# atomicarchitects/equiformer

Hardware: NVIDIA H100
Metric: edges/sec fwd+bwd, QM9 Lmax=2 batch (higher is better)
Workload: dtype f32

## Files before the change

### equiformer_b200/_lib.py

```python
from __future__ import annotations

import ctypes
import os
import shutil
import subprocess
import threading
from ctypes import POINTER, c_char_p, c_float, c_int32, c_int64, c_void_p
from pathlib import Path

PKG_DIR = Path(__file__).resolve().parent
CSRC_DIR = PKG_DIR / "csrc"
INCLUDE_DIR = PKG_DIR.parent / "include"
LIB_PATH = PKG_DIR / "libeqf_b200.so"
SOURCES = ("eqf_abi.cu", "eqf_dtp.cu", "eqf_dtp_vec.cu", "eqf_dtp_v3.cu", "eqf_attn.cu", "eqf_pointwise.cu", "eqf_gemm_tf32x3.cu", "eqf_graph.cu",
           "eqf_fused.cu", "eqf_edge.cu", "eqf_gemm_small.cu")

EQF_COLSUM_COUNTERS = 16384
EQF_MAX_BLOCKS = 8
EQF_MAX_HEADS = 16

NVCC_FLAGS = [
    "-gencode", "arch=compute_90a,code=sm_90a",
    "-lineinfo", "-O3", "-std=c++17", "--shared", "-Xcompiler", "-fPIC",
]


class EqfPathDesc(ctypes.Structure):
    _fields_ = [
        ("l1", c_int32), ("l2", c_int32), ("l3", c_int32), ("mul", c_int32),
        ("in1_block", c_int32), ("in2_off", c_int32), ("out_group", c_int32),
        ("out_chan_off", c_int32), ("w_off", c_int32), ("cg_off", c_int32),
    ]


class EqfEdgeOperands(ctypes.Structure):
    _fields_ = [
        ("x", c_void_p * EQF_MAX_BLOCKS),
        ("x2", c_void_p * EQF_MAX_BLOCKS),
        ("src", c_void_p),
        ("dst", c_void_p),
        ("y", c_void_p),
        ("w", c_void_p),
        ("w_shared", c_int32),
        ("g", c_void_p * EQF_MAX_BLOCKS),
        ("w_offset", c_void_p),
    ]


class EqfGateLayout(ctypes.Structure):
    _fields_ = [
        ("n_gated", c_int32),
        ("d", c_int32 * EQF_MAX_BLOCKS),
        ("C", c_int32 * EQF_MAX_BLOCKS),
        ("n_alpha", c_int32), ("n_scalars", c_int32), ("n_heads", c_int32),
        ("c_silu", c_float), ("c_sigmoid", c_float), ("c_slr", c_float), ("slr_slope", c_float),
    ]


class EqfNormLayout(ctypes.Structure):
    _fields_ = [
        ("n_entries", c_int32),
        ("mul", c_int32 * EQF_MAX_BLOCKS),
        ("d", c_int32 * EQF_MAX_BLOCKS),
        ("is_scalar", c_int32 * EQF_MAX_BLOCKS),
        ("eps", c_float),
    ]


class EqfHeadLayout(ctypes.Structure):
    _fields_ = [
        ("n_groups", c_int32),
        ("d", c_int32 * EQF_MAX_BLOCKS),
        ("C", c_int32 * EQF_MAX_BLOCKS),
        ("n_heads", c_int32),
    ]


EQF_GROUP_MAX = 8


class EqfGemmProblem(ctypes.Structure):
    _fields_ = [
        ("A", c_void_p), ("B", c_void_p), ("C", c_void_p),
        ("M", c_int64), ("N", c_int64), ("K", c_int64), ("lda", c_int64), ("ldb", c_int64), ("ldc", c_int64),
        ("mode", c_int32), ("accumulate", c_int32), ("alpha", c_float), ("pad", c_int32),
    ]


PtrArray = c_void_p * EQF_MAX_BLOCKS

SIGNATURES = {
    "eqf_version": (c_int32, []),
    "eqf_last_error": (c_char_p, []),
    "eqf_device_sm_count": (c_int32, []),
    "eqf_plan_create": (c_int32, [POINTER(EqfPathDesc), c_int32, POINTER(c_int32), POINTER(c_int32), c_int32,
                                  POINTER(c_int32), POINTER(c_int32), c_int32, c_int32, c_int32,
                                  POINTER(c_float), c_int32, POINTER(c_void_p)]),
    "eqf_plan_destroy": (None, [c_void_p]),
    "eqf_plan_info": (c_int32, [c_void_p, POINTER(c_int32), c_int32]),
    "eqf_plan_partial_rows": (c_int32, [c_void_p, c_int64]),
    "eqf_dtp_forward": (c_int32, [c_void_p, POINTER(EqfEdgeOperands), c_int64, POINTER(c_void_p), c_void_p]),
    "eqf_dtp_grad_x": (c_int32, [c_void_p, POINTER(EqfEdgeOperands), c_int64, POINTER(c_void_p), c_void_p]),
    "eqf_dtp_grad_w": (c_int32, [c_void_p, POINTER(EqfEdgeOperands), c_int64, c_void_p, c_void_p]),
    "eqf_dtp_grad_y": (c_int32, [c_void_p, POINTER(EqfEdgeOperands), c_int64, c_void_p, c_void_p]),
    "eqf_dtp_grad_xw": (c_int32, [c_void_p, POINTER(EqfEdgeOperands), c_int64, POINTER(c_void_p), c_void_p, c_void_p]),
    "eqf_seg_softmax": (c_int32, [c_void_p, c_void_p, c_int64, c_int32, c_void_p, c_void_p]),
    "eqf_seg_softmax_bwd": (c_int32, [c_void_p, c_void_p, c_void_p, c_void_p, c_int64, c_int32, c_void_p, c_void_p]),
    "eqf_attn_aggregate": (c_int32, [POINTER(EqfHeadLayout), c_void_p, POINTER(c_void_p), c_void_p, c_void_p, c_int64,
                                     POINTER(c_void_p), c_void_p]),
    "eqf_attn_softmax_aggregate": (c_int32, [POINTER(EqfHeadLayout), c_void_p, c_void_p, POINTER(c_void_p), c_void_p,
                                             c_int64, POINTER(c_void_p), c_void_p, c_void_p]),
    "eqf_attn_edge_dot": (c_int32, [POINTER(EqfHeadLayout), POINTER(c_void_p), POINTER(c_void_p), c_void_p, c_int64,
                                    c_void_p, c_void_p]),
    "eqf_attn_edge_scale": (c_int32, [POINTER(EqfHeadLayout), c_void_p, c_void_p, POINTER(c_void_p), c_void_p, c_int64,
                                      POINTER(c_void_p), c_void_p]),
    "eqf_pointwise_rows": (c_int32, [c_int64]),
    "eqf_ln_silu_fwd": (c_int32, [c_void_p, c_void_p, c_void_p, c_void_p, c_float, c_int64, c_int32, c_void_p, c_void_p,
                                  c_void_p, c_void_p]),
    "eqf_ln_silu_bwd": (c_int32, [c_void_p, c_void_p, c_void_p, c_void_p, c_void_p, c_void_p, c_void_p, c_int64, c_int32,
                                  c_void_p, c_void_p, c_void_p]),
    "eqf_gemm_tf32x3": (c_int32, [c_void_p, c_void_p, c_void_p, c_int64, c_int64, c_int64, c_int64, c_int64, c_int64, c_int32,
                                  c_void_p, c_void_p]),
    "eqf_gemm_tf32x3_wgrad_slices": (c_int64, [c_int64, c_int64, c_int64]),
    "eqf_gemm_tf32x3_wgrad": (c_int32, [c_void_p, c_void_p, c_void_p, c_int64, c_int64, c_int64, c_int64, c_int64, c_void_p]),
    "eqf_gemm_tf32x3_wgrad_accumulate": (c_int32, [c_void_p, c_void_p, c_void_p, c_int64, c_int64, c_int64, c_int64, c_int64,
                                                   c_void_p]),
    "eqf_dtp_linear_supported": (c_int32, [c_void_p, c_int32]),
    "eqf_fused_set_timeline": (None, [c_void_p]),
    "eqf_dtp_group_forward": (c_int32, [c_void_p, POINTER(EqfEdgeOperands), c_int64, c_int32, c_void_p, c_void_p]),
    "eqf_dtp_linear_fwd": (c_int32, [c_void_p, POINTER(EqfEdgeOperands), c_int64, c_int32, c_void_p, c_int64, c_int64, c_void_p,
                                     c_int64, c_void_p, c_void_p]),
    "eqf_radius_graph_count": (c_int32, [c_void_p, c_void_p, c_int64, c_float, c_int32, c_int64, c_void_p, c_void_p]),
    "eqf_radius_graph_fill": (c_int32, [c_void_p, c_void_p, c_int64, c_float, c_int32, c_int64, c_void_p, c_void_p, c_void_p,
                                        c_void_p]),
    "eqf_radius_graph_pbc_count": (c_int32, [c_void_p, c_void_p, c_void_p, c_void_p, c_int64, c_float, c_int32, c_int32, c_int32,
                                             c_void_p, c_void_p]),
    "eqf_radius_graph_pbc_fill": (c_int32, [c_void_p, c_void_p, c_void_p, c_void_p, c_int64, c_float, c_int32, c_int32, c_int32,
                                            c_void_p, c_void_p, c_void_p, c_void_p, c_void_p, c_void_p]),
    "eqf_edge_geom_fwd": (c_int32, [c_void_p, c_void_p, c_void_p, c_void_p, c_void_p, c_void_p, c_int64, c_int32, c_void_p,
                                    c_void_p, c_void_p, c_void_p]),
    "eqf_edge_geom_bwd": (c_int32, [c_void_p, c_void_p, c_void_p, c_int64, c_int32, c_void_p, c_void_p, c_void_p, c_void_p]),
    "eqf_expnorm_fwd": (c_int32, [c_void_p, c_void_p, c_void_p, c_float, c_float, c_int64, c_int32, c_void_p, c_void_p]),
    "eqf_expnorm_bwd": (c_int32, [c_void_p, c_void_p, c_void_p, c_float, c_float, c_int64, c_int32, c_void_p, c_void_p, c_void_p]),
    "eqf_rbf_fwd": (c_int32, [c_void_p, c_void_p, c_void_p, c_void_p, c_void_p, c_float, c_int64, c_void_p, c_void_p]),
    "eqf_rbf_bwd": (c_int32, [c_void_p, c_void_p, c_void_p, c_void_p, c_void_p, c_float, c_void_p, c_int64, c_void_p, c_void_p,
                              c_void_p]),
    "eqf_colsum_scratch_floats": (c_int64, [c_int64, c_int64]),
    "eqf_colsum": (c_int32, [c_void_p, c_int64, c_int64, c_int64, c_void_p, c_void_p, c_void_p, c_void_p]),
    "eqf_gemm_grouped": (c_int32, [ctypes.POINTER(EqfGemmProblem), c_int32, c_void_p]),
    "eqf_eln_rows": (c_int32, [POINTER(EqfNormLayout), c_int64]),
    "eqf_eln_fwd": (c_int32, [POINTER(EqfNormLayout), c_void_p, c_void_p, c_void_p, c_int64, c_void_p, c_void_p, c_void_p]),
    "eqf_eln_bwd": (c_int32, [POINTER(EqfNormLayout), c_void_p, c_void_p, c_void_p, c_void_p, c_int64, c_void_p, c_void_p,
                              c_void_p]),
    "eqf_eln_fwd_planar": (c_int32, [POINTER(EqfNormLayout), c_void_p, c_void_p, c_void_p, c_int64, c_void_p, c_void_p, c_void_p]),
    "eqf_eln_bwd_planar": (c_int32, [POINTER(EqfNormLayout), c_void_p, c_void_p, c_void_p, c_void_p, c_int64, c_void_p, c_void_p,
                                     c_void_p]),
    "eqf_gate_logits_fwd": (c_int32, [POINTER(EqfGateLayout), c_void_p, c_void_p, POINTER(c_void_p), c_void_p, c_int64,
                                      c_void_p, c_void_p, POINTER(c_void_p), c_void_p]),
    "eqf_gate_logits_bwd": (c_int32, [POINTER(EqfGateLayout), c_void_p, c_void_p, POINTER(c_void_p), c_void_p, c_void_p,
                                      c_void_p, POINTER(c_void_p), c_int64, c_void_p, POINTER(c_void_p), c_void_p,
                                      c_void_p]),
}


class EqfError(RuntimeError):
    pass


_lock = threading.Lock()
_lib = None


def sources():
    gen = sorted((CSRC_DIR / "gen").glob("dtp_gen_*.cu")) if (CSRC_DIR / "gen").exists() else []
    return [CSRC_DIR / s for s in SOURCES if (CSRC_DIR / s).exists()] + gen


def generate_sources():
    from . import codegen
    return codegen.write_all()


def needs_build() -> bool:
    if not LIB_PATH.exists():
        return True
    mtime = LIB_PATH.stat().st_mtime
    deps = sources() + list(CSRC_DIR.glob("*.cuh")) + [INCLUDE_DIR / "eqf_b200.h"]
    return any(p.stat().st_mtime > mtime for p in deps)


def build(force: bool = False, verbose: bool = False) -> Path:
    generate_sources()
    if not force and not needs_build():
        return LIB_PATH
    nvcc = shutil.which("nvcc") or "/usr/local/cuda/bin/nvcc"
    if not os.path.exists(nvcc):
        raise EqfError("nvcc not found: cannot build libeqf_b200.so")
    from concurrent.futures import ThreadPoolExecutor
    obj_dir = PKG_DIR / "build" / ("obj%d" % os.getpid())
    obj_dir.mkdir(parents=True, exist_ok=True)
    compile_flags = [f for f in NVCC_FLAGS if f != "--shared"]

    def compile_one(src: Path):
        obj = obj_dir / (src.stem + ".o")
        cmd = [nvcc, *compile_flags, "-I", str(INCLUDE_DIR), "-c", "-o", str(obj), str(src)]
        if verbose:
            cmd.insert(1, "-Xptxas=-v")
        return obj, subprocess.run(cmd, capture_output=True, text=True)

    try:
        with ThreadPoolExecutor(max_workers=min(8, os.cpu_count() or 1)) as pool:
            results = list(pool.map(compile_one, sources()))
        for _obj, proc in results:
            if proc.returncode != 0:
                raise EqfError("nvcc failed:\n" + proc.stdout + proc.stderr)
            if verbose:
                print(proc.stderr)
        tmp = LIB_PATH.with_suffix(".so.tmp%d" % os.getpid())
        link = subprocess.run([nvcc, "--shared", "-Xcompiler", "-fPIC", "-gencode", "arch=compute_90a,code=sm_90a",
                               "-o", str(tmp), *[str(o) for o, _ in results]], capture_output=True, text=True)
        if link.returncode != 0:
            raise EqfError("nvcc link failed:\n" + link.stdout + link.stderr)
        os.replace(tmp, LIB_PATH)
    finally:
        shutil.rmtree(obj_dir, ignore_errors=True)
    return LIB_PATH


def load():
    global _lib
    if _lib is not None:
        return _lib
    with _lock:
        if _lib is not None:
            return _lib
        if not LIB_PATH.exists():
            raise EqfError(
                f"{LIB_PATH} is missing: run `python -c 'import __graft_entry__ as g; g.build()'` "
                "(the sm_90a kernels are the only implementation of the edge path)")
        lib = ctypes.CDLL(str(LIB_PATH))
        for name, (restype, argtypes) in SIGNATURES.items():
            try:
                fn = getattr(lib, name)
            except AttributeError as exc:
                raise EqfError(f"libeqf_b200.so does not export {name}; rebuild it") from exc
            fn.restype = restype
            fn.argtypes = argtypes
        _lib = lib
    return _lib


def check(rc: int, what: str) -> None:
    if rc != 0:
        msg = load().eqf_last_error()
        raise EqfError(f"{what} failed (code {rc}): {msg.decode() if msg else '?'}")
```

### equiformer_b200/csrc/eqf_common.cuh

```cuda
#pragma once
#include <cuda_runtime.h>
#include <stdint.h>
#include <string>
#include <vector>

#include "../../include/eqf_b200.h"

struct EqfPlan;

namespace eqf {

constexpr int kThreads = 256;
constexpr int kWarps = kThreads / 32;
constexpr int kMaxD = 7;

struct PathDev {
  int d1, d2, d3;
  int mul;
  int xb;
  int y_off;
  int og;
  int koff;
  int w_off;
  int cg_off;
  int m_off;
  int pad;
};
static_assert(sizeof(PathDev) == 48, "PathDev layout");

struct PlanHdr {
  int n_paths, n_in1, n_out, d_y, w_numel, m_size, cg_len;
  int n_wtasks;
  int n_xtasks;
  int blob_words;
  int off_paths, off_cg, off_mdesc, off_wtasks, off_xtasks, off_xbstart, off_xbpaths;
  int te;
  int vec_ok, n_vwtasks, n_vxtasks, off_vwtasks, off_vxtasks;
  int in1_lpe[EQF_MAX_BLOCKS], in1_epw[EQF_MAX_BLOCKS];
  int in1_lpe_shift[EQF_MAX_BLOCKS];
  int in1_off[EQF_MAX_BLOCKS];
  int d_in;
  int in1_d[EQF_MAX_BLOCKS], in1_mul[EQF_MAX_BLOCKS];
  int out_d[EQF_MAX_BLOCKS], out_mul[EQF_MAX_BLOCKS];
};

struct EdgeArgs {
  const float* x[EQF_MAX_BLOCKS];
  const float* x2[EQF_MAX_BLOCKS];
  const long long* src;
  const long long* dst;
  const float* y;
  const float* w;
  const float* w_off;
  int w_shared;
  const float* g[EQF_MAX_BLOCKS];
  float* out[EQF_MAX_BLOCKS];
  float* gx[EQF_MAX_BLOCKS];
  float* gw;
  float* gy;
  long long E;
};

void set_error(const std::string& msg);
int check_cuda(cudaError_t err, const char* what);
int ensure_device(const EqfPlan* plan);
struct GeneratedKernels {
  unsigned long long signature;
  const char* tag;
  int (*forward)(const EqfPlan*, const EdgeArgs&, cudaStream_t);
  int (*backward)(const EqfPlan*, const EdgeArgs&, bool with_w, cudaStream_t);
  int (*grad_y)(const EqfPlan*, const EdgeArgs&, cudaStream_t);
  int (*partial_rows)(const EqfPlan*, long long);
};
int register_generated(const GeneratedKernels* k);
const GeneratedKernels* find_generated(unsigned long long signature);
int dtp_variant();
int launch_forward_vec(const EqfPlan* plan, const EdgeArgs& a, bool tma, cudaStream_t stream);
int launch_grad_x_vec(const EqfPlan* plan, const EdgeArgs& a, bool with_w, cudaStream_t stream);
int launch_forward_v3(const EqfPlan* plan, const EdgeArgs& a, cudaStream_t stream);
int launch_backward_v3(const EqfPlan* plan, const EdgeArgs& a, bool with_w, cudaStream_t stream);
int backward_v3_grid(const EqfPlan* plan, long long E);

}

struct EqfPlan {
  eqf::PlanHdr hdr;
  std::vector<uint32_t> blob;
  uint32_t* d_blob = nullptr;
  int device = -1;
  int sm_count = 132;
  size_t smem_bytes = 0;
  size_t smem_bytes_vec_fwd = 0;
  size_t smem_bytes_vec_bwd = 0;
  unsigned long long signature = 0;
  const eqf::GeneratedKernels* gen = nullptr;
};
```

### equiformer_b200/csrc/eqf_dtp.cu

```cuda
#include <mutex>
#include <unordered_map>

#include "eqf_common.cuh"

namespace eqf {

struct Smem {
  const PathDev* paths;
  const float* cg;
  const int* mdesc;
  const int2* wtasks;
  const int2* xtasks;
  const int* xbstart;
  const int* xbpaths;
  float* M;
  float* ysh;
  float* extra;
};

__device__ __forceinline__ Smem carve(const PlanHdr& h, const uint32_t* __restrict__ blob, uint32_t* smem) {
  for (int i = threadIdx.x; i < h.blob_words; i += blockDim.x) smem[i] = blob[i];
  Smem s;
  s.paths = reinterpret_cast<const PathDev*>(smem + h.off_paths);
  s.cg = reinterpret_cast<const float*>(smem + h.off_cg);
// ... 75 lines not shown
                                         long long e, int u) {
  float M[D1][D3];
  load_M<D1, D3>(Mp, M);
  if (u >= P.mul) return;
  float xi[D1];
  load_x<D1>(a, P.xb, P.mul, e, u, xi);
  const float wv = __ldg(a.w + (a.w_shared ? 0 : e * h.w_numel) + P.w_off + u);
  const int K = h.out_mul[P.og];
  float* o = a.out[P.og] + (e * D3) * K + P.koff + u;
#pragma unroll
  for (int k = 0; k < D3; ++k) {
    float acc = 0.f;
#pragma unroll
    for (int i = 0; i < D1; ++i) acc = fmaf(xi[i], M[i][k], acc);
    o[(long long)k * K] = wv * acc;
  }
}

__global__ void __launch_bounds__(kThreads) dtp_forward_kernel(PlanHdr h, const uint32_t* __restrict__ blob, EdgeArgs a) {
  extern __shared__ __align__(16) uint32_t smem_raw[];
  const Smem s = carve(h, blob, smem_raw);
  const int warp = threadIdx.x >> 5, lane = threadIdx.x & 31;
  const long long n_tiles = (a.E + h.te - 1) / h.te;
  for (long long tile = blockIdx.x; tile < n_tiles; tile += gridDim.x) {
    const long long e0 = tile * h.te;
    __syncthreads();
    stage_tile(h, s, a.y, e0, a.E);
    const int n_tasks = h.te * h.n_wtasks;
    for (int t = warp; t < n_tasks; t += kWarps) {
      const int te = t / h.n_wtasks;
      const long long e = e0 + te;
      if (e >= a.E) continue;
      const int2 wt = s.wtasks[t - te * h.n_wtasks];
      const PathDev& P = s.paths[wt.x];
      const float* Mp = s.M + te * h.m_size + P.m_off;
      const int u = wt.y + lane;
      EQF_DISPATCH_D(P.d1, D1, EQF_DISPATCH_D(P.d3, D3, (fwd_task<D1, D3>(h, a, P, Mp, e, u))));
    }
  }
}

template <int D1, int D3>
__device__ __forceinline__ float gw_value(const PlanHdr& h, const EdgeArgs& a, const PathDev& P, const float* Mp,
                                          long long e, int u) {
  float M[D1][D3];
  load_M<D1, D3>(Mp, M);
  if (u >= P.mul) return 0.f;
  float xi[D1];
  load_x<D1>(a, P.xb, P.mul, e, u, xi);
  const int K = h.out_mul[P.og];
  const float* gp = a.g[P.og] + (e * D3) * K + P.koff + u;
  float acc = 0.f;
#pragma unroll
  for (int k = 0; k < D3; ++k) {
    const float gk = __ldg(gp + (long long)k * K);
    float t = 0.f;
#pragma unroll
    for (int i = 0; i < D1; ++i) t = fmaf(xi[i], M[i][k], t);
    acc = fmaf(t, gk, acc);
  }
  return acc;
}

__global__ void __launch_bounds__(kThreads) dtp_grad_w_kernel(PlanHdr h, const uint32_t* __restrict__ blob, EdgeArgs a) {
  extern __shared__ __align__(16) uint32_t smem_raw[];
  const Smem s = carve(h, blob, smem_raw);
  float* wacc = s.extra;
  if (a.w_shared)
    for (int i = threadIdx.x; i < h.w_numel; i += blockDim.x) wacc[i] = 0.f;
  const int warp = threadIdx.x >> 5, lane = threadIdx.x & 31;
  const long long n_tiles = (a.E + h.te - 1) / h.te;
  for (long long tile = blockIdx.x; tile < n_tiles; tile += gridDim.x) {
    const long long e0 = tile * h.te;
    __syncthreads();
    stage_tile(h, s, a.y, e0, a.E);
    const int n_tasks = h.te * h.n_wtasks;
    for (int t = warp; t < n_tasks; t += kWarps) {
      const int te = t / h.n_wtasks;
      const long long e = e0 + te;
      if (e >= a.E) continue;
      const int2 wt = s.wtasks[t - te * h.n_wtasks];
      const PathDev& P = s.paths[wt.x];
      const float* Mp = s.M + te * h.m_size + P.m_off;
      const int u = wt.y + lane;
      float v = 0.f;
      EQF_DISPATCH_D(P.d1, D1, EQF_DISPATCH_D(P.d3, D3, (v = gw_value<D1, D3>(h, a, P, Mp, e, u))));
      if (u < P.mul) {
        if (a.w_shared) atomicAdd(wacc + P.w_off + u, v);
        else a.gw[e * h.w_numel + P.w_off + u] = v;
      }
    }
  }
  if (a.w_shared) {
    __syncthreads();
    for (int i = threadIdx.x; i < h.w_numel; i += blockDim.x) a.gw[(long long)blockIdx.x * h.w_numel + i] = wacc[i];
  }
}

template <int D1, int D3, bool WITH_W>
__device__ __forceinline__ void gx_path(const PlanHdr& h, const EdgeArgs& a, const PathDev& P, const float* Mp,
                                        long long e, int u, const float (&xi)[D1], float (&acc)[D1], float* wacc) {
  float M[D1][D3];
  load_M<D1, D3>(Mp, M);
  const int K = h.out_mul[P.og];
  const float* gp = a.g[P.og] + (e * D3) * K + P.koff + u;
  float gk[D3];
#pragma unroll
  for (int k = 0; k < D3; ++k) gk[k] = __ldg(gp + (long long)k * K);
  const float wv = __ldg(a.w + (a.w_shared ? 0 : e * h.w_numel) + P.w_off + u);
  float gwv = 0.f;
#pragma unroll
  for (int i = 0; i < D1; ++i) {
    float t = 0.f;
#pragma unroll
    for (int k = 0; k < D3; ++k) t = fmaf(gk[k], M[i][k], t);
    acc[i] = fmaf(wv, t, acc[i]);
    if (WITH_W) gwv = fmaf(xi[i], t, gwv);
  }
  if (WITH_W) {
    if (a.w_shared) atomicAdd(wacc + P.w_off + u, gwv);
    else a.gw[e * h.w_numel + P.w_off + u] = gwv;
  }
}

template <int D1, bool WITH_W>
__device__ __forceinline__ void gx_task(const PlanHdr& h, const EdgeArgs& a, const Smem& s, int te, long long e,
                                        int xb, int u, float* wacc) {
  const int mul = h.in1_mul[xb];
  if (u >= mul) return;
  float xi[D1];
  if (WITH_W) load_x<D1>(a, xb, mul, e, u, xi);
  float acc[D1];
#pragma unroll
  for (int i = 0; i < D1; ++i) acc[i] = 0.f;
  for (int q = s.xbstart[xb]; q < s.xbstart[xb + 1]; ++q) {
    const PathDev& P = s.paths[s.xbpaths[q]];
    const float* Mp = s.M + te * h.m_size + P.m_off;
    EQF_DISPATCH_D(P.d3, D3, (gx_path<D1, D3, WITH_W>(h, a, P, Mp, e, u, xi, acc, wacc)));
  }
  float* o = a.gx[xb] + (e * D1) * mul + u;
#pragma unroll
  for (int i = 0; i < D1; ++i) o[(long long)i * mul] = acc[i];
}

template <bool WITH_W>
__global__ void __launch_bounds__(kThreads) dtp_grad_x_kernel(PlanHdr h, const uint32_t* __restrict__ blob, EdgeArgs a) {
  extern __shared__ __align__(16) uint32_t smem_raw[];
  const Smem s = carve(h, blob, smem_raw);
  float* wacc = s.extra;
  if (WITH_W && a.w_shared)
    for (int i = threadIdx.x; i < h.w_numel; i += blockDim.x) wacc[i] = 0.f;
  const int warp = threadIdx.x >> 5, lane = threadIdx.x & 31;
  const long long n_tiles = (a.E + h.te - 1) / h.te;
  for (long long tile = blockIdx.x; tile < n_tiles; tile += gridDim.x) {
    const long long e0 = tile * h.te;
    __syncthreads();
    stage_tile(h, s, a.y, e0, a.E);
    const int n_tasks = h.te * h.n_xtasks;
    for (int t = warp; t < n_tasks; t += kWarps) {
      const int te = t / h.n_xtasks;
      const long long e = e0 + te;
      if (e >= a.E) continue;
      const int2 xt = s.xtasks[t - te * h.n_xtasks];
      const int u = xt.y + lane;
      EQF_DISPATCH_D(h.in1_d[xt.x], D1, (gx_task<D1, WITH_W>(h, a, s, te, e, xt.x, u, wacc)));
    }
  }
  if (WITH_W && a.w_shared) {
    __syncthreads();
    for (int i = threadIdx.x; i < h.w_numel; i += blockDim.x) a.gw[(long long)blockIdx.x * h.w_numel + i] = wacc[i];
  }
}

template <int D1, int D3>
__device__ __forceinline__ void gy_task(const PlanHdr& h, const EdgeArgs& a, const PathDev& P, float* Np,
                                        long long e, int u, int lane) {
  float xi[D1], gk[D3];
  float wv = 0.f;
#pragma unroll
  for (int i = 0; i < D1; ++i) xi[i] = 0.f;
#pragma unroll
  for (int k = 0; k < D3; ++k) gk[k] = 0.f;
  if (u < P.mul) {
    load_x<D1>(a, P.xb, P.mul, e, u, xi);
    const int K = h.out_mul[P.og];
    const float* gp = a.g[P.og] + (e * D3) * K + P.koff + u;
#pragma unroll
    for (int k = 0; k < D3; ++k) gk[k] = __ldg(gp + (long long)k * K);
    wv = __ldg(a.w + (a.w_shared ? 0 : e * h.w_numel) + P.w_off + u);
  }
#pragma unroll
  for (int i = 0; i < D1; ++i) {
    const float wx = wv * xi[i];
#pragma unroll
    for (int k = 0; k < D3; ++k) {
      const float r = warp_sum(wx * gk[k]);
      if (lane == 0) atomicAdd(Np + i * D3 + k, r);
    }
  }
}

__global__ void __launch_bounds__(kThreads) dtp_grad_y_kernel(PlanHdr h, const uint32_t* __restrict__ blob, EdgeArgs a) {
  extern __shared__ __align__(16) uint32_t smem_raw[];
  const Smem s = carve(h, blob, smem_raw);
  float* N = s.extra;
  const int warp = threadIdx.x >> 5, lane = threadIdx.x & 31;
  const long long n_tiles = (a.E + h.te - 1) / h.te;
  for (long long tile = blockIdx.x; tile < n_tiles; tile += gridDim.x) {
    const long long e0 = tile * h.te;
    __syncthreads();
    for (int i = threadIdx.x; i < h.te * h.m_size; i += blockDim.x) N[i] = 0.f;
    __syncthreads();
    const int n_tasks = h.te * h.n_wtasks;
    for (int t = warp; t < n_tasks; t += kWarps) {
      const int te = t / h.n_wtasks;
      const long long e = e0 + te;
      if (e >= a.E) continue;
      const int2 wt = s.wtasks[t - te * h.n_wtasks];
      const PathDev& P = s.paths[wt.x];
      float* Np = N + te * h.m_size + P.m_off;
      const int u = wt.y + lane;
      EQF_DISPATCH_D(P.d1, D1, EQF_DISPATCH_D(P.d3, D3, (gy_task<D1, D3>(h, a, P, Np, e, u, lane))));
    }
    __syncthreads();
    for (int idx = threadIdx.x; idx < h.te * h.d_y; idx += blockDim.x) {
      const int te = idx / h.d_y;
      const int jj = idx - te * h.d_y;
      const long long e = e0 + te;
      if (e >= a.E) continue;
      float acc = 0.f;
      for (int p = 0; p < h.n_paths; ++p) {
        const PathDev& P = s.paths[p];
        const int j = jj - P.y_off;
        if (j < 0 || j >= P.d2) continue;
        const float* c = s.cg + P.cg_off + j * P.d3;
        const float* Np = N + te * h.m_size + P.m_off;
        for (int i = 0; i < P.d1; ++i)
          for (int k = 0; k < P.d3; ++k) acc = fmaf(c[i * P.d2 * P.d3 + k], Np[i * P.d3 + k], acc);
      }
      a.gy[e * h.d_y + jj] = acc;
    }
  }
}

static int fill_args(const EqfPlan* plan, const EqfEdgeOperands* op, long long E, EdgeArgs& a, bool need_x,
                     bool need_g, bool need_w) {
  if (plan == nullptr || op == nullptr) { set_error("null plan/operands"); return EQF_ERR_INVALID; }
  if (E < 0) { set_error("negative edge count"); return EQF_ERR_INVALID; }
  const PlanHdr& h = plan->hdr;
  for (int b = 0; b < EQF_MAX_BLOCKS; ++b) {
    a.x[b] = op->x[b]; a.x2[b] = op->x2[b]; a.g[b] = op->g[b];
    a.out[b] = nullptr; a.gx[b] = nullptr;
  }
  a.src = reinterpret_cast<const long long*>(op->src);
  a.dst = reinterpret_cast<const long long*>(op->dst);
  a.y = op->y; a.w = op->w; a.w_off = op->w_offset; a.w_shared = op->w_shared; a.gw = nullptr; a.gy = nullptr; a.E = E;
  if (E == 0) return EQF_OK;
  if (a.w_off != nullptr && !(plan->gen != nullptr && dtp_variant() == 4)) {
    set_error("w_offset is only supported by the plan-specialised kernels");
    return EQF_ERR_UNSUPPORTED;
  }
  if (a.y == nullptr) { set_error("edge_attr (y) pointer is null"); return EQF_ERR_INVALID; }
  if (need_w && a.w == nullptr) { set_error("weight pointer is null"); return EQF_ERR_INVALID; }
  if (need_x) for (int b = 0; b < h.n_in1; ++b) {
    if (a.x[b] == nullptr) { set_error("in1 block pointer is null"); return EQF_ERR_INVALID; }
    if (a.x2[b] != nullptr && a.dst == nullptr) { set_error("x2 given without dst index"); return EQF_ERR_INVALID; }
  }
  if (need_g) for (int g = 0; g < h.n_out; ++g)
    if (a.g[g] == nullptr) { set_error("output-group pointer is null"); return EQF_ERR_INVALID; }
  return ensure_device(plan);
}

static int grid_for(const EqfPlan* plan, long long E) {
  const long long n_tiles = (E + plan->hdr.te - 1) / plan->hdr.te;
  const long long cap = (long long)plan->sm_count * 8;
  return (int)(n_tiles < cap ? (n_tiles > 0 ? n_tiles : 1) : cap);
}

template <typename K>
static int set_smem(K kernel, size_t bytes) {
  if (bytes <= 48 * 1024) return EQF_OK;
  static std::mutex mu;
  static std::unordered_map<const void*, size_t> configured;
  std::lock_guard<std::mutex> lock(mu);
  size_t& have = configured[reinterpret_cast<const void*>(kernel)];
  if (bytes > have) {
    int rc = check_cuda(cudaFuncSetAttribute(kernel, cudaFuncAttributeMaxDynamicSharedMemorySize, (int)bytes),
                        "cudaFuncSetAttribute(smem)");
    if (rc != EQF_OK) return rc;
    have = bytes;
  }
  return EQF_OK;
}

}

using namespace eqf;

extern "C" int eqf_plan_partial_rows(const EqfPlan* plan, int64_t n_edges) {
  if (plan == nullptr) return EQF_ERR_INVALID;
  int rows = grid_for(plan, n_edges);
  const int b = backward_v3_grid(plan, n_edges);
  if (b > rows) rows = b;
  if (plan->gen != nullptr) { const int c = plan->gen->partial_rows(plan, n_edges); if (c > rows) rows = c; }
  return rows;
}

extern "C" int eqf_dtp_forward(const EqfPlan* plan, const EqfEdgeOperands* op, int64_t n_edges,
                               float* const* out_groups, void* stream) {
  EdgeArgs a;
  int rc = fill_args(plan, op, n_edges, a, true, false, true);
  if (rc != EQF_OK || n_edges == 0) return rc;
  for (int g = 0; g < plan->hdr.n_out; ++g) {
    if (out_groups == nullptr || out_groups[g] == nullptr) { set_error("null output group"); return EQF_ERR_INVALID; }
    a.out[g] = out_groups[g];
  }
  if (plan->gen != nullptr && dtp_variant() == 4) return plan->gen->forward(plan, a, (cudaStream_t)stream);
  if (plan->hdr.vec_ok && dtp_variant() == 3) return launch_forward_v3(plan, a, (cudaStream_t)stream);
  if (plan->hdr.vec_ok && dtp_variant() > 0)
    return launch_forward_vec(plan, a, dtp_variant() == 2 && !a.w_shared, (cudaStream_t)stream);
  const size_t smem = plan->smem_bytes;
  if ((rc = set_smem(dtp_forward_kernel, smem)) != EQF_OK) return rc;
  dtp_forward_kernel<<<grid_for(plan, n_edges), kThreads, smem, (cudaStream_t)stream>>>(plan->hdr, plan->d_blob, a);
  return check_cuda(cudaGetLastError(), "dtp_forward_kernel launch");
}

extern "C" int eqf_dtp_grad_w(const EqfPlan* plan, const EqfEdgeOperands* op, int64_t n_edges, float* gw,
                              void* stream) {
  EdgeArgs a;
  int rc = fill_args(plan, op, n_edges, a, true, true, false);
  if (rc != EQF_OK || n_edges == 0) return rc;
  if (gw == nullptr) { set_error("null gw"); return EQF_ERR_INVALID; }
  a.gw = gw;
  const size_t smem = plan->smem_bytes;
  if ((rc = set_smem(dtp_grad_w_kernel, smem)) != EQF_OK) return rc;
  dtp_grad_w_kernel<<<grid_for(plan, n_edges), kThreads, smem, (cudaStream_t)stream>>>(plan->hdr, plan->d_blob, a);
  return check_cuda(cudaGetLastError(), "dtp_grad_w_kernel launch");
}

extern "C" int eqf_dtp_grad_x(const EqfPlan* plan, const EqfEdgeOperands* op, int64_t n_edges,
                              float* const* gx_blocks, void* stream) {
  EdgeArgs a;
  int rc = fill_args(plan, op, n_edges, a, false, true, true);
  if (rc != EQF_OK || n_edges == 0) return rc;
  for (int b = 0; b < plan->hdr.n_in1; ++b) {
    if (gx_blocks == nullptr || gx_blocks[b] == nullptr) { set_error("null gx block"); return EQF_ERR_INVALID; }
    a.gx[b] = gx_blocks[b];
  }
  if (plan->gen != nullptr && dtp_variant() == 4) return plan->gen->backward(plan, a, false, (cudaStream_t)stream);
  if (plan->hdr.vec_ok && dtp_variant() == 3) return launch_backward_v3(plan, a, false, (cudaStream_t)stream);
  if (plan->hdr.vec_ok && dtp_variant() > 0) return launch_grad_x_vec(plan, a, false, (cudaStream_t)stream);
  const size_t smem = plan->smem_bytes;
  if ((rc = set_smem(dtp_grad_x_kernel<false>, smem)) != EQF_OK) return rc;
  dtp_grad_x_kernel<false><<<grid_for(plan, n_edges), kThreads, smem, (cudaStream_t)stream>>>(plan->hdr, plan->d_blob, a);
  return check_cuda(cudaGetLastError(), "dtp_grad_x_kernel launch");
}

extern "C" int eqf_dtp_grad_xw(const EqfPlan* plan, const EqfEdgeOperands* op, int64_t n_edges,
                               float* const* gx_blocks, float* gw, void* stream) {
  EdgeArgs a;
  int rc = fill_args(plan, op, n_edges, a, true, true, true);
  if (rc != EQF_OK || n_edges == 0) return rc;
  if (gw == nullptr) { set_error("null gw"); return EQF_ERR_INVALID; }
  for (int b = 0; b < plan->hdr.n_in1; ++b) {
    if (gx_blocks == nullptr || gx_blocks[b] == nullptr) { set_error("null gx block"); return EQF_ERR_INVALID; }
    a.gx[b] = gx_blocks[b];
  }
  a.gw = gw;
  if (plan->gen != nullptr && dtp_variant() == 4) return plan->gen->backward(plan, a, true, (cudaStream_t)stream);
  if (plan->hdr.vec_ok && dtp_variant() == 3) return launch_backward_v3(plan, a, true, (cudaStream_t)stream);
  if (plan->hdr.vec_ok && dtp_variant() > 0) return launch_grad_x_vec(plan, a, true, (cudaStream_t)stream);
  const size_t smem = plan->smem_bytes;
  if ((rc = set_smem(dtp_grad_x_kernel<true>, smem)) != EQF_OK) return rc;
  dtp_grad_x_kernel<true><<<grid_for(plan, n_edges), kThreads, smem, (cudaStream_t)stream>>>(plan->hdr, plan->d_blob, a);
  return check_cuda(cudaGetLastError(), "dtp_grad_xw_kernel launch");
}

extern "C" int eqf_dtp_grad_y(const EqfPlan* plan, const EqfEdgeOperands* op, int64_t n_edges, float* gy,
                              void* stream) {
  EdgeArgs a;
  int rc = fill_args(plan, op, n_edges, a, true, true, true);
  if (rc != EQF_OK || n_edges == 0) return rc;
  if (gy == nullptr) { set_error("null gy"); return EQF_ERR_INVALID; }
  a.gy = gy;
  if (plan->gen != nullptr && dtp_variant() == 4) return plan->gen->grad_y(plan, a, (cudaStream_t)stream);
  const size_t smem = plan->smem_bytes;
  if ((rc = set_smem(dtp_grad_y_kernel, smem)) != EQF_OK) return rc;
  dtp_grad_y_kernel<<<grid_for(plan, n_edges), kThreads, smem, (cudaStream_t)stream>>>(plan->hdr, plan->d_blob, a);
  return check_cuda(cudaGetLastError(), "dtp_grad_y_kernel launch");
}
```

### equiformer_b200/csrc/eqf_tc.cuh

```cuda
#pragma once
#include <cuda.h>
#include <cuda_runtime.h>

#include <cstdint>
#include <string>

#include "eqf_common.cuh"

namespace eqf {
namespace tc {

__device__ __forceinline__ uint32_t smem_u32(const void* p) { return (uint32_t)__cvta_generic_to_shared(p); }

__device__ __forceinline__ void mbar_init(uint64_t* bar, uint32_t count) {
  asm volatile("mbarrier.init.shared::cta.b64 [%0], %1;" ::"r"(smem_u32(bar)), "r"(count));
}
__device__ __forceinline__ void mbar_arrive(uint64_t* bar) {
  asm volatile("mbarrier.arrive.shared::cta.b64 _, [%0];" ::"r"(smem_u32(bar)) : "memory");
}
__device__ __forceinline__ void mbar_expect_tx(uint64_t* bar, uint32_t bytes) {
  asm volatile("mbarrier.arrive.expect_tx.shared::cta.b64 _, [%0], %1;" ::"r"(smem_u32(bar)), "r"(bytes) : "memory");
}
__device__ __forceinline__ void mbar_wait(uint64_t* bar, uint32_t parity) {
  uint32_t done;
  do {
    asm volatile("{\n\t.reg .pred p;\n\tmbarrier.try_wait.parity.shared::cta.b64 p, [%1], %2;\n\tselp.u32 %0, 1, 0, p;\n\t}"
                 : "=r"(done) : "r"(smem_u32(bar)), "r"(parity) : "memory");
  } while (!done);
}
__device__ __forceinline__ void mbar_wait_hint(uint64_t* bar, uint32_t parity) {
  asm volatile(
      "{\n\t.reg .pred p;\n\t"
      "WAIT_%=:\n\t"
      "mbarrier.try_wait.parity.shared::cta.b64 p, [%0], %1, %2;\n\t"
      "@p bra DONE_%=;\n\t"
      "bra WAIT_%=;\n\t"
      "DONE_%=:\n\t}"
      ::"r"(smem_u32(bar)), "r"(parity), "r"(0x989680u) : "memory");
}
__device__ __forceinline__ void tma_load_2d(void* dst, const CUtensorMap* map, int c0, int c1, uint64_t* bar) {
  asm volatile("cp.async.bulk.tensor.2d.shared::cluster.global.mbarrier::complete_tx::bytes [%0], [%1, {%2, %3}], [%4];"
               ::"r"(smem_u32(dst)), "l"(reinterpret_cast<uint64_t>(map)), "r"(c0), "r"(c1), "r"(smem_u32(bar)) : "memory");
}
__device__ __forceinline__ void prefetch_map(const CUtensorMap* map) {
  asm volatile("prefetch.tensormap [%0];" ::"l"(reinterpret_cast<uint64_t>(map)) : "memory");
}
__device__ __forceinline__ void fence_async_smem() { asm volatile("fence.proxy.async.shared::cta;" ::: "memory"); }

__device__ __forceinline__ float tf32_rn(float x) {
  uint32_t r;
  asm("cvt.rna.tf32.f32 %0, %1;" : "=r"(r) : "f"(x));
  return __uint_as_float(r);
}
__device__ __forceinline__ float tf32_rn_fast(float x) {
  return __uint_as_float((__float_as_uint(x) + 0x1000u) & 0xffffe000u);
}

__device__ __forceinline__ float lds32(uint32_t addr) {
  float v;
  asm volatile("ld.shared.f32 %0, [%1];" : "=f"(v) : "r"(addr));
  return v;
}
__device__ __forceinline__ float4 lds128(uint32_t addr) {
  float4 v;
  asm volatile("ld.shared.v4.f32 {%0, %1, %2, %3}, [%4];" : "=f"(v.x), "=f"(v.y), "=f"(v.z), "=f"(v.w) : "r"(addr));
  return v;
}
__device__ __forceinline__ void sts128(uint32_t addr, const float4& v) {
  asm volatile("st.shared.v4.f32 [%0], {%1, %2, %3, %4};" ::"r"(addr), "f"(v.x), "f"(v.y), "f"(v.z), "f"(v.w) : "memory");
}

template <int N> __device__ __forceinline__ void reg_alloc() { asm volatile("setmaxnreg.inc.sync.aligned.u32 %0;" ::"n"(N)); }
template <int N> __device__ __forceinline__ void reg_dealloc() { asm volatile("setmaxnreg.dec.sync.aligned.u32 %0;" ::"n"(N)); }

__device__ __forceinline__ void named_barrier(int id, int threads) {
  asm volatile("bar.sync %0, %1;" ::"r"(id), "r"(threads) : "memory");
}

__device__ __forceinline__ uint64_t smem_desc_sw128(uint32_t addr) {
  return (uint64_t)((addr >> 4) & 0x3FFF) | (1ull << 16) | (64ull << 32) | (1ull << 62);
}
__device__ __forceinline__ void wgmma_fence() { asm volatile("wgmma.fence.sync.aligned;" ::: "memory"); }
__device__ __forceinline__ void wgmma_commit() { asm volatile("wgmma.commit_group.sync.aligned;" ::: "memory"); }
template <int N> __device__ __forceinline__ void wgmma_wait() { asm volatile("wgmma.wait_group.sync.aligned %0;" ::"n"(N) : "memory"); }

__device__ __forceinline__ void wgmma_rs_n32(float* d, const uint32_t* a, uint64_t b_desc) {
  asm volatile(
      "{\n\t.reg .pred p;\n\tsetp.ne.b32 p, 1, 0;\n\t"
      "wgmma.mma_async.sync.aligned.m64n32k8.f32.tf32.tf32 "
      "{%0, %1, %2, %3, %4, %5, %6, %7, %8, %9, %10, %11, %12, %13, %14, %15}, "
      "{%16, %17, %18, %19}, %20, p, 1, 1;\n\t}"
      : "+f"(d[0]), "+f"(d[1]), "+f"(d[2]), "+f"(d[3]), "+f"(d[4]), "+f"(d[5]), "+f"(d[6]), "+f"(d[7]),
        "+f"(d[8]), "+f"(d[9]), "+f"(d[10]), "+f"(d[11]), "+f"(d[12]), "+f"(d[13]), "+f"(d[14]), "+f"(d[15])
      : "r"(a[0]), "r"(a[1]), "r"(a[2]), "r"(a[3]), "l"(b_desc));
}
__device__ __forceinline__ void wgmma_rs_n64(float* d, const uint32_t* a, uint64_t b_desc) {
  asm volatile(
      "{\n\t.reg .pred p;\n\tsetp.ne.b32 p, 1, 0;\n\t"
      "wgmma.mma_async.sync.aligned.m64n64k8.f32.tf32.tf32 "
      "{%0, %1, %2, %3, %4, %5, %6, %7, %8, %9, %10, %11, %12, %13, %14, %15, "
      "%16, %17, %18, %19, %20, %21, %22, %23, %24, %25, %26, %27, %28, %29, %30, %31}, "
      "{%32, %33, %34, %35}, %36, p, 1, 1;\n\t}"
      : "+f"(d[0]), "+f"(d[1]), "+f"(d[2]), "+f"(d[3]), "+f"(d[4]), "+f"(d[5]), "+f"(d[6]), "+f"(d[7]),
        "+f"(d[8]), "+f"(d[9]), "+f"(d[10]), "+f"(d[11]), "+f"(d[12]), "+f"(d[13]), "+f"(d[14]), "+f"(d[15]),
        "+f"(d[16]), "+f"(d[17]), "+f"(d[18]), "+f"(d[19]), "+f"(d[20]), "+f"(d[21]), "+f"(d[22]), "+f"(d[23]),
        "+f"(d[24]), "+f"(d[25]), "+f"(d[26]), "+f"(d[27]), "+f"(d[28]), "+f"(d[29]), "+f"(d[30]), "+f"(d[31])
      : "r"(a[0]), "r"(a[1]), "r"(a[2]), "r"(a[3]), "l"(b_desc));
}

constexpr int kKTile = 32;

template <int N4>
__device__ __forceinline__ void load_a_split(uint32_t tile, int row0, int lane, uint32_t (&hi)[N4], uint32_t (&lo)[N4],
                                             int kb0 = 0) {
  static_assert(N4 % 4 == 0 && N4 <= 4 * (kKTile / 8), "whole 8-deep k-steps of one k-tile");
  const int g = row0 + (lane >> 2), t = lane & 3;
#pragma unroll
  for (int kb = 0; kb < N4 / 4; ++kb) {
#pragma unroll
    for (int q = 0; q < 4; ++q) {
      const int r = g + ((q & 1) ? 8 : 0);
      const int c = (kb0 + kb) * 8 + t + ((q & 2) ? 4 : 0);
      const float x = lds32(tile + (uint32_t)r * 128u + (uint32_t)((((c >> 2) ^ (r & 7)) << 4) + (c & 3) * 4));
      const float h = tf32_rn_fast(x);
      hi[kb * 4 + q] = __float_as_uint(h);
      lo[kb * 4 + q] = __float_as_uint(tf32_rn_fast(x - h));
    }
  }
}

template <int BN, int N4>
__device__ __forceinline__ void mma_ktile_3xtf32(float* acc, const uint32_t (&hi)[N4], const uint32_t (&lo)[N4], uint32_t b_hi,
                                                 uint32_t b_lo, int kb0 = 0) {
  static_assert(BN % 32 == 0 && BN >= 32 && BN <= 256, "BN must be a multiple of 32 up to 256");
  wgmma_fence();
#pragma unroll
  for (int kb = 0; kb < N4 / 4; ++kb) {
    const uint64_t adv = (uint64_t)(((kb0 + kb) * 32) >> 4);
#pragma unroll
    for (int j = 0; j < BN / 64; ++j) {
      const uint64_t dh = smem_desc_sw128(b_hi + (uint32_t)j * 8192u) + adv, dl = smem_desc_sw128(b_lo + (uint32_t)j * 8192u) + adv;
      wgmma_rs_n64(acc + 32 * j, &lo[kb * 4], dh);
      wgmma_rs_n64(acc + 32 * j, &hi[kb * 4], dl);
      wgmma_rs_n64(acc + 32 * j, &hi[kb * 4], dh);
    }
    if constexpr (BN % 64 == 32) {
      constexpr int j = BN / 64;
      const uint64_t dh = smem_desc_sw128(b_hi + (uint32_t)j * 8192u) + adv, dl = smem_desc_sw128(b_lo + (uint32_t)j * 8192u) + adv;
      wgmma_rs_n32(acc + 32 * j, &lo[kb * 4], dh);
      wgmma_rs_n32(acc + 32 * j, &hi[kb * 4], dl);
      wgmma_rs_n32(acc + 32 * j, &hi[kb * 4], dh);
    }
  }
  wgmma_commit();
}

__device__ __forceinline__ int acc_row(int i, int lane) { return (lane >> 2) + ((i >> 1) & 1) * 8; }
__device__ __forceinline__ int acc_col(int i, int lane) { return 8 * ((i & 31) >> 2) + 2 * (lane & 3) + (i & 1) + 64 * (i >> 5); }

template <int BN>
__device__ __forceinline__ void store_acc(const float* acc, float* C, long long ldc, long long row0, long long M, int col0, int N,
                                          int lane, bool add) {
#pragma unroll
  for (int i = 0; i < BN / 2; i += 2) {
    const long long r = row0 + acc_row(i, lane);
    const int c = col0 + acc_col(i, lane);
    if (r >= M || c >= N) continue;
    float* p = C + r * ldc + c;
    if (add) {
      atomicAdd(p, acc[i]);
      if (c + 1 < N) atomicAdd(p + 1, acc[i + 1]);
    } else if (c + 1 < N) {
      *reinterpret_cast<float2*>(p) = make_float2(acc[i], acc[i + 1]);
    } else {
      *p = acc[i];
    }
  }
}

typedef CUresult (*EncodeTiled)(CUtensorMap*, CUtensorMapDataType, cuuint32_t, void*, const cuuint64_t*, const cuuint64_t*,
                                const cuuint32_t*, const cuuint32_t*, CUtensorMapInterleave, CUtensorMapSwizzle,
                                CUtensorMapL2promotion, CUtensorMapFloatOOBfill);

static inline EncodeTiled encode_fn() {
  static EncodeTiled fn = [] {
    void* f = nullptr;
    cudaDriverEntryPointQueryResult q;
    if (cudaGetDriverEntryPoint("cuTensorMapEncodeTiled", &f, cudaEnableDefault, &q) != cudaSuccess) f = nullptr;
    return reinterpret_cast<EncodeTiled>(f);
  }();
  return fn;
}

enum class MapKind { kSwizzled, kLinear };

static inline int make_map_2d(CUtensorMap* map, const float* base, long long rows, long long cols, long long ld, int box_rows,
                              int box_cols, MapKind kind = MapKind::kSwizzled) {
  EncodeTiled enc = encode_fn();
  if (enc == nullptr) { set_error("cuTensorMapEncodeTiled is not available from the driver"); return EQF_ERR_CUDA; }
  cuuint64_t dims[2] = {(cuuint64_t)cols, (cuuint64_t)rows};
  cuuint64_t strides[1] = {(cuuint64_t)ld * sizeof(float)};
  cuuint32_t box[2] = {(cuuint32_t)box_cols, (cuuint32_t)box_rows};
  cuuint32_t estr[2] = {1, 1};
  const CUtensorMapSwizzle sw = kind == MapKind::kLinear ? CU_TENSOR_MAP_SWIZZLE_NONE : CU_TENSOR_MAP_SWIZZLE_128B;
  CUresult r = enc(map, CU_TENSOR_MAP_DATA_TYPE_FLOAT32, 2, const_cast<float*>(base), dims, strides, box, estr,
                   CU_TENSOR_MAP_INTERLEAVE_NONE, sw, CU_TENSOR_MAP_L2_PROMOTION_L2_128B, CU_TENSOR_MAP_FLOAT_OOB_FILL_NONE);
  if (r != CUDA_SUCCESS) { set_error("cuTensorMapEncodeTiled failed (code " + std::to_string((int)r) + ")"); return EQF_ERR_CUDA; }
  return EQF_OK;
}

static inline int device_sms() {
  int sms = 132, dev = 0;
  cudaGetDevice(&dev);
  cudaDeviceGetAttribute(&sms, cudaDevAttrMultiProcessorCount, dev);
  return sms;
}

}
}
```

### equiformer_b200/nets/graph_attention_transformer.py

```python
from __future__ import annotations

import math
from typing import List, Sequence

import torch

from .. import o3, ops
from ..graph import radius_graph, scatter_sum
from ..o3 import Irreps
from .drop import EquivariantDropout, GraphDropPath
from .fast_activation import Activation, Gate
from .gaussian_rbf import GaussianRadialBasisLayer
from .layer_norm import EquivariantLayerNormV2
from .radial_func import RadialProfile, clear_hoisted, hoist_first_layers
from .registry import register_model
from .tensor_product_rescale import (FullyConnectedTensorProductRescale,
                                     FullyConnectedTensorProductRescaleSwishGate, LinearRS, TensorProductRescale,
                                     irreps2gate, sort_irreps_even_first)

_RESCALE = True
_USE_BIAS = True

_MAX_ATOM_TYPE = 5
_AVG_NUM_NODES = 18.03065905448718
_AVG_DEGREE = 15.57930850982666


def get_norm_layer(norm_type):
    if norm_type == "layer":
        return EquivariantLayerNormV2
    if norm_type is None:
        return None
    if norm_type in ("graph", "instance", "fast_layer"):
        raise NotImplementedError(f"norm '{norm_type}' is not used by any shipped Equiformer config (out of scope)")
    raise ValueError(f"Norm type {norm_type} not supported.")


class SmoothLeakyReLU(torch.nn.Module):

    def __init__(self, negative_slope: float = 0.2):
        super().__init__()
        self.alpha = negative_slope

    def forward(self, x):
        return 0.5 * (1 + self.alpha) * x + 0.5 * (1 - self.alpha) * x * (2 * torch.sigmoid(x) - 1)

    def extra_repr(self) -> str:
        return f"negative_slope={self.alpha}"


def get_mul_0(irreps) -> int:
    return sum(mul for mul, ir in Irreps(irreps) if ir.l == 0 and ir.p == 1)


def DepthwiseTensorProduct(irreps_node_input, irreps_edge_attr, irreps_node_output, internal_weights=False, bias=True):
    irreps_node_input, irreps_edge_attr = Irreps(irreps_node_input), Irreps(irreps_edge_attr)
    irreps_node_output = Irreps(irreps_node_output)
    entries, raw = [], []
    scalar = o3.Irrep(0, 1)
    for i, (mul, ir_in) in enumerate(irreps_node_input):
        for j, (_, ir_edge) in enumerate(irreps_edge_attr):
            for ir_out in ir_in * ir_edge:
                if ir_out in irreps_node_output or ir_out == scalar:
                    raw.append((i, j, len(entries), "uvu", True))
                    entries.append((mul, ir_out))
    irreps_output, perm, _ = sort_irreps_even_first(Irreps(entries))
    instructions = [(i1, i2, perm[io], mode, train) for i1, i2, io, mode, train in raw]
    return TensorProductRescale(irreps_node_input, irreps_edge_attr, irreps_output, instructions,
                                internal_weights=internal_weights, shared_weights=internal_weights,
                                bias=bias, rescale=_RESCALE)


class SeparableFCTP(torch.nn.Module):

    def __init__(self, irreps_node_input, irreps_edge_attr, irreps_node_output, fc_neurons,
                 use_activation=False, norm_layer="graph", internal_weights=False):
        super().__init__()
        self.irreps_node_input = Irreps(irreps_node_input)
        self.irreps_edge_attr = Irreps(irreps_edge_attr)
        self.irreps_node_output = Irreps(irreps_node_output)
        norm = get_norm_layer(norm_layer)
        self.dtp = DepthwiseTensorProduct(self.irreps_node_input, self.irreps_edge_attr, self.irreps_node_output,
                                          bias=False, internal_weights=internal_weights)
        self.dtp_rad = None
        if fc_neurons is not None:
            self.dtp_rad = RadialProfile(fc_neurons + [self.dtp.tp.weight_numel])
            with torch.no_grad():
                for sl, k in self.dtp.slices_sqrt_k.values():
                    self.dtp_rad.net[-1].weight.data[sl, :] *= k
                    self.dtp_rad.offset.data[sl] *= k
        irreps_lin_output = self.irreps_node_output
        irreps_scalars, irreps_gates, irreps_gated = irreps2gate(self.irreps_node_output)
        if use_activation:
            irreps_lin_output = (irreps_scalars + irreps_gates + irreps_gated).simplify()
        self.lin = LinearRS(self.dtp.irreps_out.simplify(), irreps_lin_output)
        self.norm = norm(self.lin.irreps_out) if norm_layer is not None else None
        self.gate = None
        if use_activation:
            if irreps_gated.num_irreps == 0:
                self.gate = Activation(self.irreps_node_output, acts=[torch.nn.SiLU()])
            else:
                self.gate = Gate(irreps_scalars, [torch.nn.SiLU() for _ in irreps_scalars],
                                 irreps_gates, [torch.sigmoid for _ in irreps_gates], irreps_gated)

    def forward(self, node_input, edge_attr, edge_scalars, batch=None, **kwargs):
        weight = None
        if self.dtp_rad is not None and edge_scalars is not None:
            weight = self.dtp_rad(edge_scalars)
        out = self.lin(self.dtp(node_input, edge_attr, weight))
        if self.norm is not None:
            out = self.norm(out, batch=batch)
        if self.gate is not None:
            out = self.gate(out)
        return out

    def planar(self, xs: Sequence[torch.Tensor], edge_attr, edge_scalars):
        if self.norm is not None:
            raise NotImplementedError("planar SeparableFCTP with a norm layer is unused by the reference")
        weight = self.dtp_rad(edge_scalars) if (self.dtp_rad is not None and edge_scalars is not None) else None
        out = self.lin.planar(self.dtp.planar(xs, edge_attr, weight))
        if self.gate is not None:
            out = self.gate.planar(out) if isinstance(self.gate, Gate) else [self.gate(o) for o in out]
        return out


class Vec2AttnHeads(torch.nn.Module):

    def __init__(self, irreps_head, num_heads):
        super().__init__()
        self.num_heads = num_heads
        self.irreps_head = Irreps(irreps_head)
        self.irreps_mid_in = Irreps([(mul * num_heads, ir) for mul, ir in self.irreps_head])
        self.mid_in_indices = [(s.start, s.stop) for s in self.irreps_mid_in.slices()]

    def forward(self, x):
        n = x.shape[0]
        return torch.cat([x.narrow(1, a, b - a).reshape(n, self.num_heads, -1) for a, b in self.mid_in_indices], dim=2)

    def __repr__(self) -> str:
        return f"{self.__class__.__name__}(irreps_head={self.irreps_head}, num_heads={self.num_heads})"


class AttnHeads2Vec(torch.nn.Module):

    def __init__(self, irreps_head):
        super().__init__()
        self.irreps_head = Irreps(irreps_head)
        self.head_indices = [(s.start, s.stop) for s in self.irreps_head.slices()]

    def forward(self, x):
        n = x.shape[0]
        return torch.cat([x.narrow(2, a, b - a).reshape(n, -1) for a, b in self.head_indices], dim=1)

    def __repr__(self) -> str:
        return f"{self.__class__.__name__}(irreps_head={self.irreps_head})"


_GRAPH_CACHE = {}


def _graph_for(edge_src, edge_dst, n_nodes, kwargs) -> ops.Graph:
    g = kwargs.get("graph")
    if isinstance(g, ops.Graph) and g.n_nodes == n_nodes:
        return g
    key = (edge_src.data_ptr(), edge_dst.data_ptr(), edge_dst.numel(), n_nodes, edge_dst._version, edge_src._version)
    hit = _GRAPH_CACHE.get("last")
    if hit is not None and hit[0] == key:
        return hit[1]
    g = ops.Graph(edge_src, edge_dst, n_nodes)
    _GRAPH_CACHE["last"] = (key, g, edge_src, edge_dst)
    return g


def _is_sorted_simplified(irreps: Irreps) -> bool:
    keys = [(ir.l, -ir.p) for _, ir in irreps]
    return keys == sorted(keys) and len(set(keys)) == len(keys)


def _entries_from_groups(groups: Sequence[torch.Tensor], plan) -> List[torch.Tensor]:
    return [groups[plan.group_of_entry[io]].narrow(2, plan.chan_off_of_entry[io], mul)
            for io, (mul, _ir) in enumerate(plan.irreps_out)]


def _reblock(blocks: Sequence[torch.Tensor], irreps_from: Irreps, irreps_to: Irreps) -> List[torch.Tensor]:
    if list(irreps_from) == list(irreps_to):
        return list(blocks)
    if irreps_from.dim != irreps_to.dim:
        raise ValueError(f"cannot reinterpret {irreps_from} as {irreps_to}")
    return ops.to_planar(ops.from_planar(blocks), irreps_to)


def _group_weight_matrices(lin, n_groups: int):
    try:
        ins = [(i.i_in1, i.i_in2, i.i_out) for i in lin.tp.instructions]
        if ins != [(g, 0, g) for g in range(n_groups)] or len(lin.irreps_out) != n_groups:
            return None
        blocks = lin.tp.linear_weight_blocks()
        if any(c != 1.0 for *_i, _W, c in blocks):
            return None
        return [W.reshape(W.shape[0], W.shape[2]) for _i1, _i2, _io, W, _c in blocks]
    except (AttributeError, NotImplementedError):
        return None


def _fused_linear_possible(lin, dtp) -> bool:
    return _group_weight_matrices(lin, len(dtp.tp.plan.out_groups)) is not None


class GraphAttention(torch.nn.Module):

    def __init__(self, irreps_node_input, irreps_node_attr, irreps_edge_attr, irreps_node_output, fc_neurons,
                 irreps_head, num_heads, irreps_pre_attn=None, rescale_degree=False, nonlinear_message=False,
                 alpha_drop=0.1, proj_drop=0.1):
        super().__init__()
        self.irreps_node_input = Irreps(irreps_node_input)
        self.irreps_node_attr = Irreps(irreps_node_attr)
        self.irreps_edge_attr = Irreps(irreps_edge_attr)
        self.irreps_node_output = Irreps(irreps_node_output)
        self.irreps_pre_attn = self.irreps_node_input if irreps_pre_attn is None else Irreps(irreps_pre_attn)
        self.irreps_head = Irreps(irreps_head)
        self.num_heads = num_heads
        self.rescale_degree = rescale_degree
        self.nonlinear_message = nonlinear_message

        self.merge_src = LinearRS(self.irreps_node_input, self.irreps_pre_attn, bias=True)
        self.merge_dst = LinearRS(self.irreps_node_input, self.irreps_pre_attn, bias=False)

        irreps_attn_heads = self.irreps_head * num_heads
        irreps_attn_heads, _, _ = sort_irreps_even_first(irreps_attn_heads)
        irreps_attn_heads = irreps_attn_heads.simplify()
        mul_alpha = get_mul_0(irreps_attn_heads)
        mul_alpha_head = mul_alpha // num_heads
        irreps_alpha = Irreps(f"{mul_alpha}x0e")
        irreps_attn_all = (irreps_alpha + irreps_attn_heads).simplify()
        self.irreps_attn_heads = irreps_attn_heads

        self.sep_act = None
        if self.nonlinear_message:
            self.sep_act = SeparableFCTP(self.irreps_pre_attn, self.irreps_edge_attr, self.irreps_pre_attn, fc_neurons,
                                         use_activation=True, norm_layer=None, internal_weights=False)
            self.sep_alpha = LinearRS(self.sep_act.dtp.irreps_out, irreps_alpha)
            self.sep_value = SeparableFCTP(self.irreps_pre_attn, self.irreps_edge_attr, irreps_attn_heads,
                                           fc_neurons=None, use_activation=False, norm_layer=None,
                                           internal_weights=True)
            self.vec2heads_alpha = Vec2AttnHeads(Irreps(f"{mul_alpha_head}x0e"), num_heads)
            self.vec2heads_value = Vec2AttnHeads(self.irreps_head, num_heads)
        else:
            self.sep = SeparableFCTP(self.irreps_pre_attn, self.irreps_edge_attr, irreps_attn_all, fc_neurons,
                                     use_activation=False, norm_layer=None)
            self.vec2heads = Vec2AttnHeads((Irreps(f"{mul_alpha_head}x0e") + self.irreps_head).simplify(), num_heads)

        self.alpha_act = Activation(Irreps(f"{mul_alpha_head}x0e"), [SmoothLeakyReLU(0.2)])
        self.heads2vec = AttnHeads2Vec(self.irreps_head)
        self.mul_alpha_head = mul_alpha_head
        self.alpha_dot = torch.nn.Parameter(torch.randn(1, num_heads, mul_alpha_head))
        bound = math.sqrt(6.0 / (num_heads + mul_alpha_head))
        with torch.no_grad():
            self.alpha_dot.uniform_(-bound, bound)
        self.alpha_dropout = torch.nn.Dropout(alpha_drop) if alpha_drop != 0.0 else None
        self.proj = LinearRS(irreps_attn_heads, self.irreps_node_output)
        self.proj_drop = EquivariantDropout(self.irreps_node_input, drop_prob=proj_drop) if proj_drop != 0.0 else None

        self._alpha_single_gemm = False
        if self.nonlinear_message:
            plan_out = self.sep_act.dtp.irreps_out
            n0 = sum(1 for _, ir in plan_out if ir.is_scalar())
            ins = [(i.i_in1, i.i_in2, i.i_out) for i in self.sep_alpha.tp.instructions]
            if (n0 > 0 and all(ir.is_scalar() for _, ir in plan_out[:n0]) and ins == [(i, 0, 0) for i in range(n0)]
                    and all(c == 1.0 for *_i, _W, c in self.sep_alpha.tp.linear_weight_blocks())):
                self._alpha_single_gemm = True

        self._gate_layout = None
        if self.nonlinear_message and self._alpha_single_gemm and isinstance(self.sep_act.gate, Gate):
            gate, lin = self.sep_act.gate, self.sep_act.lin
            ins = [(i.i_in1, i.i_out) for i in lin.tp.instructions]
            n_out = len(lin.irreps_out)
            canonical = (len(gate.irreps_scalars) == 1 and ins == [(i, i) for i in range(n_out)]
                         and lin.irreps_out[0].ir.is_scalar()
                         and lin.irreps_out[0].mul == gate.irreps_scalars.dim + gate.irreps_gates.dim
                         and [m for m, _ in lin.irreps_out[1:]] == [m for m, _ in gate.irreps_gated]
                         and len(lin.bias) == 1 and len(self.sep_alpha.bias) == 1 and mul_alpha_head <= 32
                         and all(c == 1.0 for *_i, _W, c in lin.tp.linear_weight_blocks())
                         and all(c == 1.0 for *_i, _W, c in self.sep_alpha.tp.linear_weight_blocks()))
            if canonical:
                self._gate_layout = ops.GateLayout(
                    mul_alpha, gate.irreps_scalars.dim, num_heads, [ir.dim for _, ir in gate.irreps_gated],
                    [m for m, _ in gate.irreps_gated], gate.act_scalars.acts[0].cst, gate.act_gates.acts[0].cst,
                    self.alpha_act.acts[0].cst, 0.2)

        if not _is_sorted_simplified(self.irreps_head):
            raise NotImplementedError("irreps_head must be sorted (l ascending, even first) with one entry per irrep")
        self._head_layout = ops.HeadLayout([ir.dim for _, ir in irreps_attn_heads],
                                           [mul for mul, _ in irreps_attn_heads], num_heads)
        self._fuse_act = (self._gate_layout is not None and _fused_linear_possible(self.sep_act.lin, self.sep_act.dtp))
        self._fuse_value = (self.nonlinear_message and _fused_linear_possible(self.sep_value.lin, self.sep_value.dtp))

    @property
    def supports_planar(self) -> bool:
        return self.proj_drop is None or not self.training or getattr(self.proj_drop, "drop_prob", 1.0) == 0.0

    def forward(self, node_input, node_attr, edge_src, edge_dst, edge_attr, edge_scalars, batch, **kwargs):
        xs = ops.to_planar(node_input, self.irreps_node_input)
        node = self.forward_planar(xs, node_attr, edge_src, edge_dst, edge_attr, edge_scalars, batch, **kwargs)
        node_output = ops.from_planar(node)
        if self.proj_drop is not None:
            node_output = self.proj_drop(node_output)
        return node_output

    def forward_planar(self, xs, node_attr, edge_src, edge_dst, edge_attr, edge_scalars, batch, **kwargs):
        n_nodes = xs[0].shape[0]
        graph = _graph_for(edge_src, edge_dst, n_nodes, kwargs)
        edge_attr = graph.sort_edges(edge_attr).contiguous()
        edge_scalars = graph.sort_edges(edge_scalars)
        E, H, A = graph.n_edges, self.num_heads, self.mul_alpha_head

        m_src = self.merge_src.planar(xs)
        m_dst = self.merge_dst.planar(xs)

        if self.nonlinear_message:
            sa = self.sep_act
            weight = sa.dtp_rad(edge_scalars, add_offset=False)
            plan1 = sa.dtp.tp.plan
            fuse1 = self._fuse_act and ops.dtp_linear_ok(plan1, edge_attr, weight)
            f = None
            if not fuse1:
                f = sa.dtp.tp.planar_depthwise_gathered(graph, m_src, m_dst, edge_attr, weight,
                                                        sa.dtp_rad.offset)
            logits = None
            if self._gate_layout is not None and (fuse1 or ops.fused_ok(f[0])):
                lay = self._gate_layout
                blocks = {io: (W, c) for _i1, _i2, io, W, c in sa.lin.tp.linear_weight_blocks()}
                k0 = plan1.out_groups[0][2]
                w_cat = torch.cat([self.sep_alpha.tp.weight.view(k0, -1), blocks[0][0].reshape(k0, -1)], dim=1)
                bias = torch.cat([self.sep_alpha.bias[0], sa.lin.bias[0]])
                if fuse1:
                    Ws = [w_cat] + [blocks[g][0].reshape(blocks[g][0].shape[0], -1) for g in range(1, len(plan1.out_groups))]
                    outs = ops.dtp_linear(plan1, graph, m_src, m_dst, edge_attr, weight, sa.dtp_rad.offset, Ws)
                    t0, gated = outs[0].reshape(E, -1), outs[1:]
                else:
                    t0 = ops.matmul_f32(f[0].reshape(E, k0), w_cat)
                    gated = [ops.matmul_f32(f[g].reshape(E * f[g].shape[1], f[g].shape[2]), blocks[g][0].reshape(f[g].shape[2], -1))
                             .view(E, f[g].shape[1], -1) for g in range(1, len(f))]
                logits, v0, *vs = ops.GateLogits.apply(lay, t0, bias, self.alpha_dot.view(H, A), *gated)
                value = _reblock([v0.view(E, 1, -1), *vs], sa.gate.irreps_out, self.sep_value.irreps_node_input)
                value = self._value_linear(value, edge_attr)
                alpha = None
            elif self._alpha_single_gemm:
                k0 = f[0].shape[2]
                w_alpha = self.sep_alpha.tp.weight.view(k0, -1)
                alpha = ops.matmul_f32(f[0].reshape(E, k0), w_alpha)
                if len(self.sep_alpha.bias) > 0:
                    alpha = alpha + self.sep_alpha.bias[0]
            else:
                alpha = self.sep_alpha.planar(_entries_from_groups(f, sa.dtp.tp.plan))[0]
            if logits is None:
                value = sa.lin.planar(f)
                value = sa.gate.planar(value) if isinstance(sa.gate, Gate) else [sa.gate(v) for v in value]
                value = _reblock(value, sa.gate.irreps_out, self.sep_value.irreps_node_input)
                value = self._value_linear(value, edge_attr)
                alpha = alpha.reshape(E, H, A)
        else:
            weight = self.sep.dtp_rad(edge_scalars, add_offset=False)
            logits = None
            out = self.sep.lin.planar(self.sep.dtp.tp.planar_depthwise_gathered(
                graph, m_src, m_dst, edge_attr, weight, self.sep.dtp_rad.offset))
            first = out[0]
            if first.shape[1] != 1:
                raise NotImplementedError("attention logits need a leading 0e entry")
            per_head = first.reshape(E, H, -1)
            alpha = per_head.narrow(2, 0, A)
            rest = per_head.shape[2] - A
            value = ([per_head.narrow(2, A, rest).reshape(E, 1, H * rest)] if rest > 0 else []) + list(out[1:])

        z = logits if logits is not None else (self.alpha_act(alpha) * self.alpha_dot).sum(dim=-1)
        no_drop = self.alpha_dropout is None or not self.training or self.alpha_dropout.p == 0.0
        if ops.softmax_aggregate_ok(self._head_layout, z):
            vs = [v.contiguous() for v in value]
            if no_drop:
                node = list(ops.SoftmaxAggregate.apply(self._head_layout, graph, z.contiguous(), *vs))
            else:
                keep = torch.nn.functional.dropout(torch.ones_like(z), self.alpha_dropout.p, True)
                node = list(ops.MaskedSoftmaxAggregate.apply(self._head_layout, graph, z.contiguous(), keep, *vs))
        else:
            attn = ops.segment_softmax(z.contiguous(), graph)
            if self.alpha_dropout is not None:
                attn = self.alpha_dropout(attn)
            node = ops.attention_aggregate(self._head_layout, graph, attn.contiguous(), [v.contiguous() for v in value])

        if self.rescale_degree:
            degree = (graph.row_ptr[1:] - graph.row_ptr[:-1]).to(node[0].dtype).view(-1, 1, 1)
            node = [t * degree for t in node]
        return self.proj.planar(node)

    def _value_linear(self, value, edge_attr):
        sv = self.sep_value
        plan2 = sv.dtp.tp.plan
        w2 = sv.dtp.tp.weight
        if self._fuse_value and ops.dtp_linear_ok(plan2, edge_attr, w2):
            Ws = _group_weight_matrices(sv.lin, len(plan2.out_groups))
            return sv.lin._planar_bias(ops.dtp_linear(plan2, None, [v.contiguous() for v in value], None, edge_attr, w2,
                                                      None, Ws))
        return sv.lin.planar(sv.dtp.planar(value, edge_attr, None))

    def extra_repr(self) -> str:
        return f"rescale_degree={self.rescale_degree}, "


class FeedForwardNetwork(torch.nn.Module):

    def __init__(self, irreps_node_input, irreps_node_attr, irreps_node_output, irreps_mlp_mid=None, proj_drop=0.1):
        super().__init__()
        self.irreps_node_input = Irreps(irreps_node_input)
        self.irreps_node_attr = Irreps(irreps_node_attr)
        self.irreps_mlp_mid = Irreps(irreps_mlp_mid) if irreps_mlp_mid is not None else self.irreps_node_input
        self.irreps_node_output = Irreps(irreps_node_output)
        self.fctp_1 = FullyConnectedTensorProductRescaleSwishGate(
            self.irreps_node_input, self.irreps_node_attr, self.irreps_mlp_mid, bias=True, rescale=_RESCALE)
        self.fctp_2 = FullyConnectedTensorProductRescale(
            self.irreps_mlp_mid, self.irreps_node_attr, self.irreps_node_output, bias=True, rescale=_RESCALE)
        self.proj_drop = EquivariantDropout(self.irreps_node_output, drop_prob=proj_drop) if proj_drop != 0.0 else None
        self._gate_layout = None
        gate, f1 = self.fctp_1.gate, self.fctp_1
        ins = [(i.i_in1, i.i_out) for i in f1.tp.instructions]
        if (isinstance(gate, Gate) and ins == [(i, i) for i in range(len(f1.irreps_out))] and len(f1.bias) == 1
                and self.irreps_node_attr.dim == 1):
            lay = ops.gate_only_layout(gate, f1.irreps_out)
            self._gate_layout = lay if (lay is not None and f1.bias[0].numel() == lay.width) else None

    @property
    def supports_planar(self) -> bool:
        return self.proj_drop is None or not self.training or getattr(self.proj_drop, "drop_prob", 1.0) == 0.0

    def forward(self, node_input, node_attr, **kwargs):
        node_output = ops.from_planar(self.forward_planar(ops.to_planar(node_input, self.irreps_node_input), node_attr))
        if self.proj_drop is not None:
            node_output = self.proj_drop(node_output)
        return node_output

    def forward_planar(self, xs, node_attr, **kwargs):
        y = None if (getattr(node_attr, "_eqf_all_ones", False) and self.irreps_node_attr.dim == 1) else node_attr
        gate = self.fctp_1.gate
        if self._gate_layout is not None and y is None and ops.fused_ok(xs[0]):
            pre = self.fctp_1.tp.planar_linear(xs, None, None)
            N = pre[0].shape[0]
            h = ops.gate_fused(self._gate_layout, pre[0].reshape(N, -1), self.fctp_1.bias[0], pre[1:])
            h = _reblock([h[0].view(N, 1, -1), *h[1:]], gate.irreps_out, self.fctp_2.irreps_in1)
        else:
            h = self.fctp_1.planar(xs, y)
            if isinstance(gate, Gate):
                h = _reblock(gate.planar(h), gate.irreps_out, self.fctp_2.irreps_in1)
            else:
                h = [gate(t) for t in h]
        return self.fctp_2.planar(h, y)


class TransBlock(torch.nn.Module):

    def __init__(self, irreps_node_input, irreps_node_attr, irreps_edge_attr, irreps_node_output, fc_neurons,
                 irreps_head, num_heads, irreps_pre_attn=None, rescale_degree=False, nonlinear_message=False,
                 alpha_drop=0.1, proj_drop=0.1, drop_path_rate=0.0, irreps_mlp_mid=None, norm_layer="layer"):
        super().__init__()
        self.irreps_node_input = Irreps(irreps_node_input)
        self.irreps_node_attr = Irreps(irreps_node_attr)
        self.irreps_edge_attr = Irreps(irreps_edge_attr)
        self.irreps_node_output = Irreps(irreps_node_output)
        self.irreps_pre_attn = self.irreps_node_input if irreps_pre_attn is None else Irreps(irreps_pre_attn)
        self.irreps_head = Irreps(irreps_head)
        self.num_heads = num_heads
        self.rescale_degree = rescale_degree
        self.nonlinear_message = nonlinear_message
        self.irreps_mlp_mid = Irreps(irreps_mlp_mid) if irreps_mlp_mid is not None else self.irreps_node_input

        self.norm_1 = get_norm_layer(norm_layer)(self.irreps_node_input)
        setattr(self, self._attn_name, self._make_attention(fc_neurons, alpha_drop, proj_drop))
        self.drop_path = GraphDropPath(drop_path_rate) if drop_path_rate > 0.0 else None
        self.norm_2 = get_norm_layer(norm_layer)(self.irreps_node_input)
        self.ffn = FeedForwardNetwork(irreps_node_input=self.irreps_node_input, irreps_node_attr=self.irreps_node_attr,
                                      irreps_node_output=self.irreps_node_output, irreps_mlp_mid=self.irreps_mlp_mid,
                                      proj_drop=proj_drop)
        self.ffn_shortcut = None
        if self.irreps_node_input != self.irreps_node_output:
            self.ffn_shortcut = FullyConnectedTensorProductRescale(
                self.irreps_node_input, self.irreps_node_attr, self.irreps_node_output, bias=True, rescale=_RESCALE)

    _attn_name = "ga"

    def _make_attention(self, fc_neurons, alpha_drop, proj_drop):
        return GraphAttention(irreps_node_input=self.irreps_node_input, irreps_node_attr=self.irreps_node_attr,
                              irreps_edge_attr=self.irreps_edge_attr, irreps_node_output=self.irreps_node_input,
                              fc_neurons=fc_neurons, irreps_head=self.irreps_head, num_heads=self.num_heads,
                              irreps_pre_attn=self.irreps_pre_attn, rescale_degree=self.rescale_degree,
                              nonlinear_message=self.nonlinear_message, alpha_drop=alpha_drop, proj_drop=proj_drop)

    @property
    def attention(self):
        return getattr(self, self._attn_name)

    def forward(self, node_input, node_attr, edge_src, edge_dst, edge_attr, edge_scalars, batch, **kwargs):
        features = self.norm_1(node_input, batch=batch)
        features = self.attention(node_input=features, node_attr=node_attr, edge_src=edge_src, edge_dst=edge_dst,
                                  edge_attr=edge_attr, edge_scalars=edge_scalars, batch=batch, **kwargs)
        n_graphs = kwargs.get("n_graphs")
        if self.drop_path is not None:
            features = self._drop_path(features, batch, n_graphs)
        node_output = node_input + features

        features = self.ffn(self.norm_2(node_output, batch=batch), node_attr)
        if self.ffn_shortcut is not None:
            node_output = self.ffn_shortcut(node_output, node_attr)
        if self.drop_path is not None:
            features = self._drop_path(features, batch, n_graphs)
        return node_output + features

    def _drop_path(self, features, batch, n_graphs):
        return self.drop_path(features, batch) if n_graphs is None else self.drop_path(features, batch, n_graphs=n_graphs)

    @property
    def supports_planar(self) -> bool:
        return (getattr(self.norm_1, "supports_planar", False) and getattr(self.norm_2, "supports_planar", False)
                and self.ffn_shortcut is None
                and (self.drop_path is None or not self.training or type(self.drop_path) is GraphDropPath)
                and self.attention.supports_planar and self.ffn.supports_planar
                and self.irreps_node_input == self.irreps_node_output)

    def forward_planar(self, xs, node_attr, edge_src, edge_dst, edge_attr, edge_scalars, batch, **kwargs):
        f = self.attention.forward_planar(self.norm_1.planar(xs), node_attr, edge_src, edge_dst, edge_attr, edge_scalars,
                                          batch, **kwargs)
        xs = self._residual(xs, f, batch, kwargs.get("n_graphs"))
        f = self.ffn.forward_planar(self.norm_2.planar(xs), node_attr)
        return self._residual(xs, f, batch, kwargs.get("n_graphs"))

    def _residual(self, xs, f, batch, n_graphs):
        if self.drop_path is None or not self.training:
            return [a + b for a, b in zip(xs, f)]
        s = self.drop_path.node_scale(f[0], batch, n_graphs)
        return [torch.addcmul(a, b, s) for a, b in zip(xs, f)]


class NodeEmbeddingNetwork(torch.nn.Module):
    def __init__(self, irreps_node_embedding, max_atom_type=_MAX_ATOM_TYPE, bias=True):
        super().__init__()
        self.max_atom_type = max_atom_type
        self.irreps_node_embedding = Irreps(irreps_node_embedding)
        self.atom_type_lin = LinearRS(Irreps(f"{self.max_atom_type}x0e"), self.irreps_node_embedding, bias=bias)
        self.atom_type_lin.tp.weight.data.mul_(self.max_atom_type ** 0.5)

    def forward(self, node_atom):
        classes = torch.arange(self.max_atom_type, device=node_atom.device)
        onehot = (node_atom.unsqueeze(-1) == classes).to(self.atom_type_lin.tp.weight.dtype)
        return self.atom_type_lin(onehot), onehot, onehot


class ScaledScatter(torch.nn.Module):
    def __init__(self, avg_aggregate_num):
        super().__init__()
        self.avg_aggregate_num = avg_aggregate_num + 0.0

    def forward(self, x, index, **kwargs):
        return scatter_sum(x, index, **kwargs).div(self.avg_aggregate_num ** 0.5)

    def extra_repr(self) -> str:
        return f"avg_aggregate_num={self.avg_aggregate_num}"


class EdgeDegreeEmbeddingNetwork(torch.nn.Module):

    def __init__(self, irreps_node_embedding, irreps_edge_attr, fc_neurons, avg_aggregate_num):
        super().__init__()
        irreps_node_embedding = Irreps(irreps_node_embedding)
        self.exp = LinearRS(Irreps("1x0e"), irreps_node_embedding, bias=_USE_BIAS, rescale=_RESCALE)
        self.dw = DepthwiseTensorProduct(irreps_node_embedding, irreps_edge_attr, irreps_node_embedding,
                                         internal_weights=False, bias=False)
        self.rad = RadialProfile(fc_neurons + [self.dw.tp.weight_numel])
        with torch.no_grad():
            for sl, k in self.dw.slices_sqrt_k.values():
                self.rad.net[-1].weight.data[sl, :] *= k
                self.rad.offset.data[sl] *= k
        self.proj = LinearRS(self.dw.irreps_out.simplify(), irreps_node_embedding)
        self.scale_scatter = ScaledScatter(avg_aggregate_num)
        self._sum_layout = ops.HeadLayout([ir.dim for _, ir in self.proj.irreps_out],
                                          [mul for mul, _ in self.proj.irreps_out], 1)
        self._fuse_proj = _fused_linear_possible(self.proj, self.dw)

    def forward(self, node_input, edge_attr, edge_scalars, edge_src, edge_dst, batch, **kwargs):
        n_nodes = node_input.shape[0]
        graph = _graph_for(edge_src, edge_dst, n_nodes, kwargs)
        edge_attr = graph.sort_edges(edge_attr).contiguous()
        edge_scalars = graph.sort_edges(edge_scalars)
        ones = torch.ones((n_nodes, 1, 1), dtype=node_input.dtype, device=node_input.device)
        node_feats = self.exp.planar([ones])
        weight = self.rad(edge_scalars, add_offset=False)
        plan = self.dw.tp.plan
        if self._fuse_proj and ops.dtp_linear_ok(plan, edge_attr, weight):
            Ws = _group_weight_matrices(self.proj, len(plan.out_groups))
            edge_feats = self.proj._planar_bias(ops.dtp_linear(plan, graph, node_feats, None, edge_attr, weight,
                                                               self.rad.offset, Ws))
        else:
            edge_feats = self.dw.tp.planar_depthwise_gathered(graph, node_feats, None, edge_attr, weight, self.rad.offset)
            edge_feats = self.proj.planar(edge_feats)
        summed = ops.attention_aggregate(self._sum_layout, graph, None, [t.contiguous() for t in edge_feats])
        return ops.from_planar(summed).div(self.scale_scatter.avg_aggregate_num ** 0.5)


class GraphAttentionTransformer(torch.nn.Module):

    def __init__(self, irreps_in="5x0e", irreps_node_embedding="128x0e+64x1e+32x2e", num_layers=6,
                 irreps_node_attr="1x0e", irreps_sh="1x0e+1x1e+1x2e", max_radius=5.0, number_of_basis=128,
                 basis_type="gaussian", fc_neurons=[64, 64], irreps_feature="512x0e",
                 irreps_head="32x0e+16x1o+8x2e", num_heads=4, irreps_pre_attn=None, rescale_degree=False,
                 nonlinear_message=False, irreps_mlp_mid="128x0e+64x1e+32x2e", norm_layer="layer",
                 alpha_drop=0.2, proj_drop=0.0, out_drop=0.0, drop_path_rate=0.0,
                 mean=None, std=None, scale=None, atomref=None):
        super().__init__()
        self.max_radius = max_radius
        self.number_of_basis = number_of_basis
        self.alpha_drop, self.proj_drop, self.out_drop = alpha_drop, proj_drop, out_drop
        self.drop_path_rate = drop_path_rate
        self.norm_layer = norm_layer
        self.task_mean, self.task_std, self.scale = mean, std, scale
        self.register_buffer("atomref", atomref)

        self.irreps_node_attr = Irreps(irreps_node_attr)
        self.irreps_node_input = Irreps(irreps_in)
        self.irreps_node_embedding = Irreps(irreps_node_embedding)
        self.lmax = self.irreps_node_embedding.lmax
        self.irreps_feature = Irreps(irreps_feature)
        self.num_layers = num_layers
        self.irreps_edge_attr = Irreps(irreps_sh) if irreps_sh is not None else Irreps.spherical_harmonics(self.lmax)
        self.fc_neurons = [self.number_of_basis] + list(fc_neurons)
        self.irreps_head = Irreps(irreps_head)
        self.num_heads = num_heads
        self.irreps_pre_attn = irreps_pre_attn
        self.rescale_degree = rescale_degree
        self.nonlinear_message = nonlinear_message
        self.irreps_mlp_mid = Irreps(irreps_mlp_mid)

        self.atom_embed = NodeEmbeddingNetwork(self.irreps_node_embedding, _MAX_ATOM_TYPE)
        self.basis_type = basis_type
        if basis_type == "gaussian":
            self.rbf = GaussianRadialBasisLayer(self.number_of_basis, cutoff=self.max_radius)
        elif basis_type == "bessel":
            raise NotImplementedError("Bessel basis comes from ocpmodels (absent dependency; out of scope, SURVEY.md 2#5)")
        else:
            raise ValueError(basis_type)
        self.edge_deg_embed = EdgeDegreeEmbeddingNetwork(self.irreps_node_embedding, self.irreps_edge_attr,
                                                         self.fc_neurons, _AVG_DEGREE)
        self.blocks = torch.nn.ModuleList()
        self.build_blocks()
        self.norm = get_norm_layer(self.norm_layer)(self.irreps_feature)
        self.out_dropout = EquivariantDropout(self.irreps_feature, self.out_drop) if self.out_drop != 0.0 else None
        self.head = torch.nn.Sequential(
            LinearRS(self.irreps_feature, self.irreps_feature, rescale=_RESCALE),
            Activation(self.irreps_feature, acts=[torch.nn.SiLU()]),
            LinearRS(self.irreps_feature, Irreps("1x0e"), rescale=_RESCALE))
        self.scale_scatter = ScaledScatter(_AVG_NUM_NODES)
        self.register_buffer("_atom_remap", torch.tensor([-1, 0, -1, -1, -1, -1, 1, 2, 3, 4]), persistent=False)
        self.apply(self._init_weights)

    _block_cls = TransBlock

    def build_blocks(self):
        for i in range(self.num_layers):
            out = self.irreps_node_embedding if i != self.num_layers - 1 else self.irreps_feature
            self.blocks.append(self._block_cls(
                irreps_node_input=self.irreps_node_embedding, irreps_node_attr=self.irreps_node_attr,
                irreps_edge_attr=self.irreps_edge_attr, irreps_node_output=out, fc_neurons=self.fc_neurons,
                irreps_head=self.irreps_head, num_heads=self.num_heads, irreps_pre_attn=self.irreps_pre_attn,
                rescale_degree=self.rescale_degree, nonlinear_message=self.nonlinear_message,
                alpha_drop=self.alpha_drop, proj_drop=self.proj_drop, drop_path_rate=self.drop_path_rate,
                irreps_mlp_mid=self.irreps_mlp_mid, norm_layer=self.norm_layer))

    def _init_weights(self, m):
        if isinstance(m, torch.nn.Linear):
            if m.bias is not None:
                torch.nn.init.constant_(m.bias, 0)
        elif isinstance(m, torch.nn.LayerNorm):
            torch.nn.init.constant_(m.bias, 0)
            torch.nn.init.constant_(m.weight, 1.0)

    @torch.jit.ignore
    def no_weight_decay(self):
        skip = set()
        names = {n for n, _ in self.named_parameters()}
        for mod_name, mod in self.named_modules():
            if isinstance(mod, (torch.nn.Linear, torch.nn.LayerNorm, EquivariantLayerNormV2, GaussianRadialBasisLayer)):
                for p_name, _ in mod.named_parameters():
                    if isinstance(mod, torch.nn.Linear) and "weight" in p_name:
                        continue
                    full = f"{mod_name}.{p_name}"
                    assert full in names
                    skip.add(full)
        return skip

    def forward(self, f_in, pos, batch, node_atom, **kwargs) -> torch.Tensor:
        edge_src, edge_dst = radius_graph(pos, r=self.max_radius, batch=batch, max_num_neighbors=1000)
        return self.forward_edges(pos, batch, node_atom, edge_src, edge_dst, n_graphs=kwargs.get("n_graphs"),
                                  edges_sorted=True)

    def forward_edges(self, pos, batch, node_atom, edge_src, edge_dst, graph=None, n_graphs=None,
                      edges_sorted: bool = False, edge_vec=None) -> torch.Tensor:
        if edge_vec is not None and not (edges_sorted or graph is not None):
            raise ValueError("edge_vec needs a destination-sorted edge list (edges_sorted=True or a graph)")
        if graph is None:
            graph = ops.Graph(edge_src, edge_dst, pos.shape[0], check_sorted=not edges_sorted)
            if graph.perm is not None:
                edge_src, edge_dst = graph.src, graph.dst
                graph.perm = None
        edge_vec, edge_length, edge_sh = edge_features(self.irreps_edge_attr, pos, graph, edge_vec)
        atom_embedding, _attr, _onehot = self.atom_embed(self._atom_remap[node_atom])
        edge_length_embedding = self.rbf(edge_length)
        served = hoist_radial(self, edge_length_embedding)
        try:
            edge_degree_embedding = self.edge_deg_embed(atom_embedding, edge_sh, edge_length_embedding, edge_src, edge_dst,
                                                        batch, graph=graph)
            node_features = atom_embedding + edge_degree_embedding
            node_attr = torch.ones_like(node_features.narrow(1, 0, 1))
            node_attr._eqf_all_ones = True
            node_features = _run_blocks(self.blocks, node_features, self.irreps_node_embedding, node_attr, edge_src, edge_dst,
                                        edge_sh, edge_length_embedding, batch, graph, n_graphs)
        finally:
            clear_hoisted(served)
        node_features = self.norm(node_features, batch=batch)
        if self.out_dropout is not None:
            node_features = self.out_dropout(node_features)
        outputs = self.head(node_features)
        outputs = self.scale_scatter(outputs, batch, dim=0, dim_size=n_graphs)
        if self.scale is not None:
            outputs = self.scale * outputs
        return outputs


def edge_features(irreps_edge_attr, pos, graph, edge_vec=None):
    ls = [ir.l for mul, ir in irreps_edge_attr for _ in range(mul)]
    if (edge_vec is None and ls == list(range(len(ls))) and 1 <= len(ls) <= 4 and pos.is_cuda and pos.dtype == torch.float32
            and graph.perm is None and graph.n_edges > 0):
        return ops.edge_geometry(pos, graph, len(ls) - 1)
    if edge_vec is None:
        edge_vec = pos.index_select(0, graph.src) - pos.index_select(0, graph.dst)
    edge_sh = o3.spherical_harmonics(l=irreps_edge_attr, x=edge_vec, normalize=True, normalization="component")
    return edge_vec, edge_vec.norm(dim=1), edge_sh


def hoist_radial(model, edge_scalars):
    mods = model.__dict__.get("_rad_modules")
    if mods is None:
        mods = [m for m in model.modules() if isinstance(m, RadialProfile)]
        model.__dict__["_rad_modules"] = mods
    return hoist_first_layers(mods, edge_scalars)


def _run_blocks(blocks, node_features, irreps, node_attr, edge_src, edge_dst, edge_sh, edge_scalars, batch, graph,
                n_graphs=None):
    planar = None
    for blk in blocks:
        kw = dict(node_attr=node_attr, edge_src=edge_src, edge_dst=edge_dst, edge_attr=edge_sh, edge_scalars=edge_scalars,
                  batch=batch, graph=graph, n_graphs=n_graphs)
        if getattr(blk, "supports_planar", False) and ops.fused_ok(node_features if planar is None else planar[0]):
            if planar is None:
                planar = ops.to_planar(node_features, Irreps(irreps))
            planar = blk.forward_planar(planar, **kw)
        else:
            if planar is not None:
                node_features, planar = ops.from_planar(planar), None
            node_features = blk(node_input=node_features, **kw)
    return ops.from_planar(planar) if planar is not None else node_features


def _qm9(irreps_in, radius, num_basis, atomref, task_mean, task_std, **over):
    cfg = dict(irreps_in=irreps_in, irreps_node_embedding="128x0e+64x1e+32x2e", num_layers=6,
               irreps_node_attr="1x0e", irreps_sh="1x0e+1x1e+1x2e", max_radius=radius, number_of_basis=num_basis,
               fc_neurons=[64, 64], irreps_feature="512x0e", irreps_head="32x0e+16x1e+8x2e", num_heads=4,
               irreps_pre_attn=None, rescale_degree=False, nonlinear_message=False,
               irreps_mlp_mid="384x0e+192x1e+96x2e", norm_layer="layer", alpha_drop=0.2, proj_drop=0.0,
               out_drop=0.0, drop_path_rate=0.0, mean=task_mean, std=task_std, scale=None, atomref=atomref)
    cfg.update(over)
    return GraphAttentionTransformer(**cfg)


@register_model
def graph_attention_transformer_l2(irreps_in, radius, num_basis=128, atomref=None, task_mean=None, task_std=None, **kwargs):
    return _qm9(irreps_in, radius, num_basis, atomref, task_mean, task_std)


@register_model
def graph_attention_transformer_nonlinear_l2(irreps_in, radius, num_basis=128, atomref=None, task_mean=None,
                                             task_std=None, **kwargs):
    return _qm9(irreps_in, radius, num_basis, atomref, task_mean, task_std, nonlinear_message=True)


@register_model
def graph_attention_transformer_nonlinear_l2_e3(irreps_in, radius, num_basis=128, atomref=None, task_mean=None,
                                                task_std=None, **kwargs):
    return _qm9(irreps_in, radius, num_basis, atomref, task_mean, task_std, nonlinear_message=True,
                irreps_node_embedding="128x0e+32x0o+32x1e+32x1o+16x2e+16x2o", irreps_sh="1x0e+1x1o+1x2e",
                irreps_head="32x0e+8x0o+8x1e+8x1o+4x2e+4x2o", irreps_mlp_mid="384x0e+96x0o+96x1e+96x1o+48x2e+48x2o")


@register_model
def graph_attention_transformer_nonlinear_bessel_l2(irreps_in, radius, num_basis=128, atomref=None, task_mean=None,
                                                    task_std=None, **kwargs):
    return _qm9(irreps_in, radius, num_basis, atomref, task_mean, task_std, nonlinear_message=True, basis_type="bessel")


@register_model
def graph_attention_transformer_nonlinear_bessel_l2_drop01(irreps_in, radius, num_basis=128, atomref=None,
                                                           task_mean=None, task_std=None, **kwargs):
    return _qm9(irreps_in, radius, num_basis, atomref, task_mean, task_std, nonlinear_message=True,
                basis_type="bessel", alpha_drop=0.1)


@register_model
def graph_attention_transformer_nonlinear_bessel_l2_drop00(irreps_in, radius, num_basis=128, atomref=None,
                                                           task_mean=None, task_std=None, **kwargs):
    return _qm9(irreps_in, radius, num_basis, atomref, task_mean, task_std, nonlinear_message=True,
                basis_type="bessel", alpha_drop=0.0)
```

### equiformer_b200/ops.py

```python
from __future__ import annotations

import contextlib
import ctypes
import os
from typing import List, Optional, Sequence, Tuple

import torch

from . import _lib
from .plan import DtpPlan



def _require_cuda(t: torch.Tensor, name: str) -> torch.Tensor:
    if not t.is_cuda:
        raise _lib.EqfError(
            f"{name} lives on {t.device}: the equiformer_b200 edge kernels are CUDA-only (sm_90a); "
            "there is no CPU fallback on the product path")
    if t.dtype != torch.float32:
        raise _lib.EqfError(f"{name} must be float32 (the reference trains in fp32), got {t.dtype}")
    return t.contiguous()


def _require_index(t: torch.Tensor, name: str) -> torch.Tensor:
    if not t.is_cuda:
        raise _lib.EqfError(f"{name} lives on {t.device}: CUDA index tensor required")
    if t.dtype != torch.int64:
        t = t.to(torch.int64)
    return t.contiguous()


def _stream() -> ctypes.c_void_p:
    return ctypes.c_void_p(torch.cuda.current_stream().cuda_stream)


def _ptr_array(ts: Sequence[torch.Tensor]):
    arr = (ctypes.c_void_p * _lib.EQF_MAX_BLOCKS)()
    for i, t in enumerate(ts):
        arr[i] = t.data_ptr()
    return arr


def _operands(plan: DtpPlan, xs, y, w, gs, w_shared: bool, gather=None, w_offset=None) -> _lib.EqfEdgeOperands:
    op = _lib.EqfEdgeOperands()
    if w_offset is not None:
        w_offset = _require_cuda(w_offset, "w_offset")
        if w_shared or tuple(w_offset.shape) != (plan.weight_numel,):
            raise ValueError("w_offset must be [weight_numel] and needs per-edge weights")
        op.w_offset = w_offset.data_ptr()
    if xs is not None:
        for i, t in enumerate(xs):
            op.x[i] = t.data_ptr()
    if gather is not None:
        src, dst, x2s = gather
        op.src = src.data_ptr()
        if x2s is not None:
            op.dst = dst.data_ptr()
            for i, t in enumerate(x2s):
                op.x2[i] = t.data_ptr()
    if gs is not None:
        for i, t in enumerate(gs):
            op.g[i] = t.data_ptr()
    op.y = y.data_ptr()
    op.w = w.data_ptr() if w is not None else None
    op.w_shared = 1 if w_shared else 0
    return op


def _check_blocks(plan: DtpPlan, xs, E: int, what: str):
    if len(xs) != len(plan.in1_blocks):
        raise ValueError(f"{what}: expected {len(plan.in1_blocks)} in1 blocks, got {len(xs)}")
    out = []
    for t, (l, mul) in zip(xs, plan.in1_blocks):
        t = _require_cuda(t, what)
        if tuple(t.shape) != (E, 2 * l + 1, mul):
            raise ValueError(f"{what}: block shape {tuple(t.shape)} != {(E, 2 * l + 1, mul)}")
        out.append(t)
    return out


def _check_groups(plan: DtpPlan, gs, E: int, what: str):
    if len(gs) != len(plan.out_groups):
        raise ValueError(f"{what}: expected {len(plan.out_groups)} output groups, got {len(gs)}")
    out = []
    for t, (l, _p, mul) in zip(gs, plan.out_groups):
        t = _require_cuda(t, what)
        if tuple(t.shape) != (E, 2 * l + 1, mul):
            raise ValueError(f"{what}: group shape {tuple(t.shape)} != {(E, 2 * l + 1, mul)}")
        out.append(t)
    return out


def _check_yw(plan: DtpPlan, y, w, E: Optional[int] = None):
    y = _require_cuda(y, "edge_attr")
    if y.dim() != 2 or y.shape[1] != plan.d_y:
        raise ValueError(f"edge_attr must be [E, {plan.d_y}], got {tuple(y.shape)}")
    E = y.shape[0]
    shared = None
    if w is not None:
        w = _require_cuda(w, "weight")
        if w.dim() == 1:
            shared = True
            if w.shape[0] != plan.weight_numel:
                raise ValueError(f"shared weight must be [{plan.weight_numel}], got {tuple(w.shape)}")
        else:
            shared = False
            if tuple(w.shape) != (E, plan.weight_numel):
                raise ValueError(f"per-edge weight must be [{E}, {plan.weight_numel}], got {tuple(w.shape)}")
    return y, w, E, shared




class KernelProfile:

    def __init__(self, time_events: bool = True, presleep_cycles: int = 0):
        self.time_events = time_events
        self.presleep_cycles = presleep_cycles
        self.launches = 0
        self.records = []

    def summary(self):
        out = {}
        for name, nbytes, s, e, flops in self.records:
            ms = s.elapsed_time(e)
            d = out.setdefault(name, {"launches": 0, "ms": 0.0, "bytes": 0, "flops": 0})
            d["launches"] += 1
            d["ms"] += ms
            d["bytes"] += nbytes
            d["flops"] += flops
        return out


PROFILE: Optional[KernelProfile] = None


@contextlib.contextmanager
def _kernel(name: str, nbytes: int, flops: int = 0):
    prof = PROFILE
    if prof is None:
        yield
        return
    prof.launches += 1
    if not prof.time_events:
        yield
        return
    s = torch.cuda.Event(enable_timing=True)
    e = torch.cuda.Event(enable_timing=True)
    if prof.presleep_cycles:
        torch.cuda._sleep(prof.presleep_cycles)
    s.record()
    yield
    e.record()
    prof.records.append((name, nbytes, s, e, flops))


def _dtp_bytes(plan: DtpPlan, E: int, shared: bool, kind: str) -> int:
    d_in, d_out, w = plan.irreps_in1.dim, plan.irreps_out.dim, (0 if shared else plan.weight_numel)
    per_edge = {"forward": d_in + plan.d_y + w + d_out,
                "grad_x": d_out + plan.d_y + w + d_in,
                "grad_w": d_out + plan.d_y + d_in + w,
                "grad_y": d_out + d_in + w + 2 * plan.d_y,
                "grad_xw": d_out + d_in + plan.d_y + w + d_in + w}[kind]
    return 4 * per_edge * E


def _attn_bytes(lay: "HeadLayout", rows_edge: int, rows_node: int, kind: str) -> int:
    dv = sum(d * c for d, c in zip(lay.ds, lay.Cs))
    h = lay.n_heads
    per = {"aggregate": rows_edge * (dv + h) + rows_node * dv,
           "edge_dot": rows_edge * (2 * dv + h),
           "edge_scale": rows_edge * (2 * dv + h)}[kind]
    return 4 * per




def _check_gather(plan: DtpPlan, xs, gather, E: int, what: str):
    if gather is None:
        return _check_blocks(plan, xs, E, what), None
    src, dst, x2s = gather
    n_rows = xs[0].shape[0]
    xs = _check_blocks(plan, xs, n_rows, what)
    src = _require_index(src, "edge_src")
    if src.numel() != E:
        raise ValueError(f"{what}: gather index has {src.numel()} entries for {E} edges")
    if x2s is not None:
        x2s = _check_blocks(plan, x2s, x2s[0].shape[0], what)
        dst = _require_index(dst, "edge_dst")
    return xs, (src, dst, x2s)


def dtp_forward_raw(plan: DtpPlan, xs, y, w, gather=None, w_offset=None) -> List[torch.Tensor]:
    y, w, E, shared = _check_yw(plan, y, w)
    xs, gather = _check_gather(plan, xs, gather, E, "dtp_forward x")
    outs = [torch.empty((E, 2 * l + 1, mul), device=y.device, dtype=torch.float32) for l, _p, mul in plan.out_groups]
    op = _operands(plan, xs, y, w, None, shared, gather, w_offset)
    with torch.cuda.device(y.device), _kernel("dtp_forward", _dtp_bytes(plan, E, shared, "forward")):
        rc = _lib.load().eqf_dtp_forward(plan.handle, ctypes.byref(op), E, _ptr_array(outs), _stream())
    _lib.check(rc, "eqf_dtp_forward")
    return outs


def dtp_grad_x_raw(plan: DtpPlan, gs, y, w) -> List[torch.Tensor]:
    y, w, E, shared = _check_yw(plan, y, w)
    gs = _check_groups(plan, gs, E, "dtp_grad_x g")
    gxs = [torch.empty((E, 2 * l + 1, mul), device=y.device, dtype=torch.float32) for l, mul in plan.in1_blocks]
    op = _operands(plan, None, y, w, gs, shared)
    with torch.cuda.device(y.device), _kernel("dtp_grad_x", _dtp_bytes(plan, E, shared, "grad_x")):
        rc = _lib.load().eqf_dtp_grad_x(plan.handle, ctypes.byref(op), E, _ptr_array(gxs), _stream())
    _lib.check(rc, "eqf_dtp_grad_x")
    return gxs


def _gw_buffer(plan: DtpPlan, E: int, shared: bool, device) -> torch.Tensor:
    if shared:
        rows = _lib.load().eqf_plan_partial_rows(plan.handle, E)
        return torch.zeros((max(rows, 1), plan.weight_numel), device=device, dtype=torch.float32)
    return torch.empty((E, plan.weight_numel), device=device, dtype=torch.float32)


def dtp_grad_w_raw(plan: DtpPlan, xs, y, gs, shared: bool) -> torch.Tensor:
    y, _, E, _ = _check_yw(plan, y, None)
    xs = _check_blocks(plan, xs, E, "dtp_grad_w x")
    gs = _check_groups(plan, gs, E, "dtp_grad_w g")
    if E == 0:
        return torch.zeros((plan.weight_numel,) if shared else (0, plan.weight_numel), device=y.device)
    gw = _gw_buffer(plan, E, shared, y.device)
    op = _operands(plan, xs, y, None, gs, shared)
    with torch.cuda.device(y.device), _kernel("dtp_grad_w", _dtp_bytes(plan, E, shared, "grad_w")):
        rc = _lib.load().eqf_dtp_grad_w(plan.handle, ctypes.byref(op), E, ctypes.c_void_p(gw.data_ptr()), _stream())
    _lib.check(rc, "eqf_dtp_grad_w")
    return _colsum(gw) if shared else gw


def dtp_grad_y_raw(plan: DtpPlan, xs, w, gs, y_like) -> torch.Tensor:
    y, w, E, shared = _check_yw(plan, y_like, w)
    xs = _check_blocks(plan, xs, E, "dtp_grad_y x")
    gs = _check_groups(plan, gs, E, "dtp_grad_y g")
    gy = torch.empty((E, plan.d_y), device=y.device, dtype=torch.float32)
    op = _operands(plan, xs, y, w, gs, shared)
    with torch.cuda.device(y.device), _kernel("dtp_grad_y", _dtp_bytes(plan, E, shared, "grad_y")):
        rc = _lib.load().eqf_dtp_grad_y(plan.handle, ctypes.byref(op), E, ctypes.c_void_p(gy.data_ptr()), _stream())
    _lib.check(rc, "eqf_dtp_grad_y")
    return gy


def dtp_grad_xw_raw(plan: DtpPlan, xs, y, w, gs, gather=None, w_offset=None) -> Tuple[List[torch.Tensor], torch.Tensor]:
    y, w, E, shared = _check_yw(plan, y, w)
    xs, gather = _check_gather(plan, xs, gather, E, "dtp_grad_xw x")
    gs = _check_groups(plan, gs, E, "dtp_grad_xw g")
    gxs = [torch.empty((E, 2 * l + 1, mul), device=y.device, dtype=torch.float32) for l, mul in plan.in1_blocks]
    if E == 0:
        return gxs, torch.zeros_like(w)
    gw = _gw_buffer(plan, E, shared, y.device)
    op = _operands(plan, xs, y, w, gs, shared, gather, w_offset)
    with torch.cuda.device(y.device), _kernel("dtp_grad_xw", _dtp_bytes(plan, E, shared, "grad_xw")):
        rc = _lib.load().eqf_dtp_grad_xw(plan.handle, ctypes.byref(op), E, _ptr_array(gxs),
                                         ctypes.c_void_p(gw.data_ptr()), _stream())
    _lib.check(rc, "eqf_dtp_grad_xw")
    return gxs, (_colsum(gw) if shared else gw)




def _fill(gs, likes):
    return [g if g is not None else torch.zeros_like(t) for g, t in zip(gs, likes)]


class DtpOut(torch.autograd.Function):

    @staticmethod
    def forward(ctx, plan: DtpPlan, y, w, *xs):
        ctx.plan = plan
        outs = dtp_forward_raw(plan, xs, y, w)
        ctx.save_for_backward(y, w, *xs)
        return tuple(outs)

    @staticmethod
    def backward(ctx, *gs):
        plan = ctx.plan
        y, w, *xs = ctx.saved_tensors
        nb = len(xs)
        E = y.shape[0]
        gs = [g if g is not None else torch.zeros((E, 2 * l + 1, m), device=y.device)
              for g, (l, _p, m) in zip(gs, plan.out_groups)]
        need_y, need_w = ctx.needs_input_grad[1], ctx.needs_input_grad[2]
        need_x = any(ctx.needs_input_grad[3:3 + nb])
        gy = gw = None
        gxs = [None] * nb
        if torch.is_grad_enabled():
            if need_x:
                gxs = list(DtpGradX.apply(plan, y, w, *gs))
            if need_w:
                gw = DtpGradW.apply(plan, y, w.dim() == 1, *xs, *gs)
            if need_y:
                gy = DtpGradY.apply(plan, y, w, *xs, *gs)
        else:
            gs = [g.contiguous() for g in gs]
            if need_x and need_w:
                gxs, gw = dtp_grad_xw_raw(plan, xs, y, w, gs)
            elif need_x:
                gxs = dtp_grad_x_raw(plan, gs, y, w)
            elif need_w:
                gw = dtp_grad_w_raw(plan, xs, y, gs, w.dim() == 1)
            if need_y:
                gy = dtp_grad_y_raw(plan, xs, w, gs, y)
        return (None, gy, gw, *gxs)


class DtpGradX(torch.autograd.Function):

    @staticmethod
    def forward(ctx, plan: DtpPlan, y, w, *gs):
        ctx.plan = plan
        outs = dtp_grad_x_raw(plan, gs, y, w)
        ctx.save_for_backward(y, w, *gs)
        return tuple(outs)

    @staticmethod
    def backward(ctx, *cxs):
        plan = ctx.plan
        y, w, *gs = ctx.saved_tensors
        E = y.shape[0]
        cxs = [c if c is not None else torch.zeros((E, 2 * l + 1, m), device=y.device)
               for c, (l, m) in zip(cxs, plan.in1_blocks)]
        need_y, need_w = ctx.needs_input_grad[1], ctx.needs_input_grad[2]
        need_g = any(ctx.needs_input_grad[3:])
        gy = gw = None
        ggs = [None] * len(gs)
        if need_g:
            ggs = list(DtpOut.apply(plan, y, w, *cxs))
        if need_w:
            gw = DtpGradW.apply(plan, y, w.dim() == 1, *cxs, *gs)
        if need_y:
            gy = DtpGradY.apply(plan, y, w, *cxs, *gs)
        return (None, gy, gw, *ggs)


class DtpGradW(torch.autograd.Function):

    @staticmethod
    def forward(ctx, plan: DtpPlan, y, shared: bool, *xg):
        nb = len(plan.in1_blocks)
        xs, gs = xg[:nb], xg[nb:]
        ctx.plan, ctx.shared = plan, shared
        out = dtp_grad_w_raw(plan, xs, y, gs, shared)
        ctx.save_for_backward(y, *xg)
        return out

    @staticmethod
    def backward(ctx, cw):
        plan = ctx.plan
        y, *xg = ctx.saved_tensors
        nb = len(plan.in1_blocks)
        xs, gs = xg[:nb], xg[nb:]
        need_y = ctx.needs_input_grad[1]
        need_x = any(ctx.needs_input_grad[3:3 + nb])
        need_g = any(ctx.needs_input_grad[3 + nb:])
        cw = cw.contiguous()
        gy = None
        gxs = [None] * nb
        ggs = [None] * len(gs)
        if need_x:
            gxs = list(DtpGradX.apply(plan, y, cw, *gs))
        if need_g:
            ggs = list(DtpOut.apply(plan, y, cw, *xs))
        if need_y:
            gy = DtpGradY.apply(plan, y, cw, *xs, *gs)
        return (None, gy, None, *gxs, *ggs)


class DtpGradY(torch.autograd.Function):

    @staticmethod
    def forward(ctx, plan: DtpPlan, y_like, w, *xg):
        nb = len(plan.in1_blocks)
        xs, gs = xg[:nb], xg[nb:]
        ctx.plan = plan
        out = dtp_grad_y_raw(plan, xs, w, gs, y_like)
        ctx.save_for_backward(w, *xg)
        return out

    @staticmethod
    def backward(ctx, cy):
        plan = ctx.plan
        w, *xg = ctx.saved_tensors
        nb = len(plan.in1_blocks)
        xs, gs = xg[:nb], xg[nb:]
        need_w = ctx.needs_input_grad[2]
        need_x = any(ctx.needs_input_grad[3:3 + nb])
        need_g = any(ctx.needs_input_grad[3 + nb:])
        cy = cy.contiguous()
        gw = None
        gxs = [None] * nb
        ggs = [None] * len(gs)
        if need_x:
            gxs = list(DtpGradX.apply(plan, cy, w, *gs))
        if need_g:
            ggs = list(DtpOut.apply(plan, cy, w, *xs))
        if need_w:
            gw = DtpGradW.apply(plan, cy, w.dim() == 1, *xs, *gs)
        return (None, None, gw, *gxs, *ggs)


class DtpOutGathered(torch.autograd.Function):

    @staticmethod
    def forward(ctx, plan: DtpPlan, graph: "Graph", n_b: int, y, w, *AB):
        nb = len(plan.in1_blocks)
        As, Bs = AB[:nb], (AB[nb:] if n_b else None)
        ctx.plan, ctx.graph, ctx.n_b = plan, graph, n_b
        outs = dtp_forward_raw(plan, As, y, w, gather=(graph.src, graph.dst, Bs))
        ctx.save_for_backward(y, w, *AB)
        return tuple(outs)

    @staticmethod
    def backward(ctx, *gs):
        plan, graph, n_b = ctx.plan, ctx.graph, ctx.n_b
        y, w, *AB = ctx.saved_tensors
        nb = len(plan.in1_blocks)
        As, Bs = AB[:nb], (AB[nb:] if n_b else None)
        E = y.shape[0]
        gs = [g if g is not None else torch.zeros((E, 2 * l + 1, m), device=y.device)
              for g, (l, _p, m) in zip(gs, plan.out_groups)]
        need_y, need_w = ctx.needs_input_grad[3], ctx.needs_input_grad[4]
        need_x = any(ctx.needs_input_grad[5:])
        if torch.is_grad_enabled():
            xs = [a.index_select(0, graph.src) for a in As]
            if Bs is not None:
                xs = [x + b.index_select(0, graph.dst) for x, b in zip(xs, Bs)]
            gy = DtpGradY.apply(plan, y, w, *xs, *gs) if need_y else None
            gw = DtpGradW.apply(plan, y, w.dim() == 1, *xs, *gs) if need_w else None
            gA = [None] * nb
            gB = [None] * nb
            if need_x:
                gxs = DtpGradX.apply(plan, y, w, *gs)
                gA = [torch.zeros_like(a).index_add(0, graph.src, g) for a, g in zip(As, gxs)]
                if Bs is not None:
                    gB = [torch.zeros_like(b).index_add(0, graph.dst, g) for b, g in zip(Bs, gxs)]
            return (None, None, None, gy, gw, *gA, *(gB if Bs is not None else []))
        gs = [g.contiguous() for g in gs]
        gather = (graph.src, graph.dst, Bs)
        gy = gw = None
        gA = [None] * nb
        gB = [None] * nb
        if need_x or need_w:
            gxs, gw_full = dtp_grad_xw_raw(plan, As, y, w, gs, gather=gather)
            gw = gw_full if need_w else None
            if need_x:
                lay = HeadLayout([2 * l + 1 for l, _ in plan.in1_blocks], [m for _, m in plan.in1_blocks], 1)
                gA = attn_aggregate_raw(lay, None, gxs, graph, by_src=True)
                if Bs is not None:
                    gB = attn_aggregate_raw(lay, None, gxs, graph)
        if need_y:
            xs = [a.index_select(0, graph.src) for a in As]
            if Bs is not None:
                xs = [x + b.index_select(0, graph.dst) for x, b in zip(xs, Bs)]
            gy = dtp_grad_y_raw(plan, xs, w, gs, y)
        return (None, None, None, gy, gw, *gA, *(gB if Bs is not None else []))


class DtpOutGatheredOffset(torch.autograd.Function):

    @staticmethod
    def forward(ctx, plan: DtpPlan, graph: "Graph", n_b: int, y, w, offset, *AB):
        nb = len(plan.in1_blocks)
        As, Bs = AB[:nb], (AB[nb:] if n_b else None)
        ctx.plan, ctx.graph, ctx.n_b = plan, graph, n_b
        outs = dtp_forward_raw(plan, As, y, w, gather=(graph.src, graph.dst, Bs), w_offset=offset)
        ctx.save_for_backward(y, w, offset, *AB)
        return tuple(outs)

    @staticmethod
    def backward(ctx, *gs):
        plan, graph, n_b = ctx.plan, ctx.graph, ctx.n_b
        y, w, offset, *AB = ctx.saved_tensors
        nb = len(plan.in1_blocks)
        As, Bs = AB[:nb], (AB[nb:] if n_b else None)
        E = y.shape[0]
        gs = [g if g is not None else torch.zeros((E, 2 * l + 1, m), device=y.device)
              for g, (l, _p, m) in zip(gs, plan.out_groups)]
        need_y, need_w, need_off = ctx.needs_input_grad[3:6]
        need_x = any(ctx.needs_input_grad[6:])
        if torch.is_grad_enabled() or need_y:
            fn = lambda yy, ww, oo, *ab: DtpOutGathered.apply(plan, graph, n_b, yy, ww + oo, *ab)
            grads = _higher_order_grads(fn, (y, w, offset, *AB), gs)
            return (None, None, None, *grads)
        gs = [g.contiguous() for g in gs]
        gw = goff = None
        gA = [None] * nb
        gB = [None] * nb
        if need_x or need_w or need_off:
            gxs, gw = dtp_grad_xw_raw(plan, As, y, w, gs, gather=(graph.src, graph.dst, Bs), w_offset=offset)
            if need_off:
                goff = colsum_raw(gw)
            if need_x:
                lay = HeadLayout([2 * l + 1 for l, _ in plan.in1_blocks], [m for _, m in plan.in1_blocks], 1)
                gA = attn_aggregate_raw(lay, None, gxs, graph, by_src=True)
                if Bs is not None:
                    gB = attn_aggregate_raw(lay, None, gxs, graph)
        return (None, None, None, None, gw if need_w else None, goff, *gA, *(gB if Bs is not None else []))


def depthwise_tensor_product_gathered(plan: DtpPlan, graph: "Graph", As, Bs, y, w, w_offset=None):
    AB = (*As, *(Bs if Bs is not None else ()))
    n_b = 0 if Bs is None else len(Bs)
    if w_offset is not None:
        if plan.generated and w.dim() == 2 and fused_ok(y):
            return list(DtpOutGatheredOffset.apply(plan, graph, n_b, y, w, w_offset, *AB))
        w = w + w_offset
    return list(DtpOutGathered.apply(plan, graph, n_b, y, w, *AB))



_FUSED_MODE = os.environ.get("EQF_FUSED", "auto")
_FUSED = _FUSED_MODE != "0"
_FUSED_MIN_EDGES = int(os.environ.get("EQF_FUSED_MIN_EDGES", "200000"))
_FUSED_SPLIT = {}


def dtp_linear_supported(plan: DtpPlan) -> bool:
    ok = getattr(plan, "_fused_ok", None)
    if ok is None:
        lib = _lib.load()
        ok = all(lib.eqf_dtp_linear_supported(plan.handle, g) == 1 for g in range(len(plan.out_groups)))
        plan._fused_ok = ok
    return ok


def dtp_linear_ok(plan: DtpPlan, y: torch.Tensor, w: torch.Tensor) -> bool:
    if not _FUSED or (_FUSED_MODE == "auto" and y.shape[0] < _FUSED_MIN_EDGES and not FUSED_ON_ANY_DEVICE):
        return False
    return (fused_ok(y) and not (torch.is_grad_enabled() and y.requires_grad)
            and y.shape[0] > 0 and dtp_linear_supported(plan))


def dtp_linear_fwd_raw(plan: DtpPlan, group: int, xs, y, w, Wt: torch.Tensor, gather=None, w_offset=None) -> torch.Tensor:
    y, w, E, shared = _check_yw(plan, y, w)
    xs, gather = _check_gather(plan, xs, gather, E, "dtp_linear x")
    l3, _p, K = plan.out_groups[group]
    Wt = _require_cuda(Wt, "dtp_linear weight")
    if Wt.dim() != 2 or Wt.shape[0] != K:
        raise ValueError(f"dtp_linear: weight must be [{K}, N], got {tuple(Wt.shape)}")
    N = Wt.shape[1]
    d3 = 2 * l3 + 1
    C = torch.empty((E, d3, N), device=y.device, dtype=torch.float32)
    need = 2 * N * K
    split = _FUSED_SPLIT.get(y.device)
    if split is None or split.numel() < need:
        split = torch.empty(max(need, 1 << 20), device=y.device, dtype=torch.float32)
        _FUSED_SPLIT[y.device] = split
    op = _operands(plan, xs, y, w, None, shared, gather, w_offset)
    d_in = sum((2 * l + 1) * m for l, m in plan.in1_blocks)
    nbytes = 4 * (E * (d_in + plan.d_y + (0 if shared else K) + d3 * N) + K * N)
    with torch.cuda.device(y.device), _kernel("dtp_linear_fwd", nbytes, 2 * E * d3 * K * N):
        rc = _lib.load().eqf_dtp_linear_fwd(plan.handle, ctypes.byref(op), E, group, Wt.data_ptr(), N, Wt.stride(0),
                                            C.data_ptr(), N, split.data_ptr(), _stream())
    _lib.check(rc, "eqf_dtp_linear_fwd")
    return C


_FUSED_MAX_N = int(os.environ.get("EQF_FUSED_MAX_N", "64"))


def dtp_group_forward_raw(plan: DtpPlan, group: int, xs, y, w, gather=None, w_offset=None) -> torch.Tensor:
    y, w, E, shared = _check_yw(plan, y, w)
    xs, gather = _check_gather(plan, xs, gather, E, "dtp_group_forward x")
    l3, _p, K = plan.out_groups[group]
    out = torch.empty((E, 2 * l3 + 1, K), device=y.device, dtype=torch.float32)
    op = _operands(plan, xs, y, w, None, shared, gather, w_offset)
    d_in = sum((2 * l + 1) * m for l, m in plan.in1_blocks)
    nbytes = 4 * E * (d_in + plan.d_y + (0 if shared else K) + (2 * l3 + 1) * K)
    with torch.cuda.device(y.device), _kernel("dtp_group_forward", nbytes):
        rc = _lib.load().eqf_dtp_group_forward(plan.handle, ctypes.byref(op), E, group, out.data_ptr(), _stream())
    _lib.check(rc, "eqf_dtp_group_forward")
    return out


def _dtp_linear_unfused(plan: DtpPlan, graph, n_b: int, y, w, offset, AB, Ws):
    nb = len(plan.in1_blocks)
    As, Bs = AB[:nb], (AB[nb:] if n_b else None)
    if graph is not None:
        f = depthwise_tensor_product_gathered(plan, graph, As, Bs, y, w, offset)
    else:
        f = depthwise_tensor_product(plan, As, y, w if offset is None else w + offset)
    E = y.shape[0]
    return [matmul_f32(fg.reshape(E * fg.shape[1], fg.shape[2]), W).view(E, fg.shape[1], -1) for fg, W in zip(f, Ws)]


class DtpLinear(torch.autograd.Function):

    @staticmethod
    def forward(ctx, plan: DtpPlan, graph, n_b: int, y, w, offset, *rest):
        nb, ng = len(plan.in1_blocks), len(plan.out_groups)
        n_ab = nb + (nb if n_b else 0)
        AB, Ws = rest[:n_ab], rest[n_ab:]
        if len(Ws) != ng:
            raise ValueError(f"DtpLinear: expected {ng} weight matrices, got {len(Ws)}")
        As, Bs = AB[:nb], (AB[nb:] if n_b else None)
        gather = (graph.src, graph.dst, Bs) if graph is not None else None
        outs = []
        for g in range(ng):
            if Ws[g].shape[1] <= _FUSED_MAX_N:
                outs.append(dtp_linear_fwd_raw(plan, g, As, y, w, Ws[g], gather=gather, w_offset=offset))
            else:
                fg = dtp_group_forward_raw(plan, g, As, y, w, gather=gather, w_offset=offset)
                E, d = fg.shape[0], fg.shape[1]
                outs.append(gemm_raw(0, fg.reshape(E * d, fg.shape[2]), Ws[g].contiguous()).view(E, d, -1))
        ctx.plan, ctx.graph, ctx.n_b, ctx.n_ab, ctx.has_off = plan, graph, n_b, n_ab, offset is not None
        ctx.save_for_backward(y, w, *([offset] if offset is not None else []), *rest)
        return tuple(outs)

    @staticmethod
    def backward(ctx, *dCs):
        plan, graph, n_b, n_ab = ctx.plan, ctx.graph, ctx.n_b, ctx.n_ab
        y, w, *saved = ctx.saved_tensors
        offset = saved.pop(0) if ctx.has_off else None
        AB, Ws = saved[:n_ab], saved[n_ab:]
        nb, ng = len(plan.in1_blocks), len(plan.out_groups)
        As, Bs = AB[:nb], (AB[nb:] if n_b else None)
        E = y.shape[0]
        dCs = [g if g is not None else torch.zeros((E, 2 * l + 1, W.shape[1]), device=y.device)
               for g, (l, _p, _k), W in zip(dCs, plan.out_groups, Ws)]
        need = ctx.needs_input_grad
        need_y, need_w, need_off = need[3], need[4], need[5]
        need_x = any(need[6:6 + n_ab])
        need_W = need[6 + n_ab:]
        if torch.is_grad_enabled() or need_y:
            fn = lambda yy, ww, oo, *r: tuple(_dtp_linear_unfused(plan, graph, n_b, yy, ww, oo, r[:n_ab], r[n_ab:]))
            grads = _higher_order_grads(fn, (y, w, offset, *AB, *Ws), dCs)
            return (None, None, None, *grads)
        gather = (graph.src, graph.dst, Bs) if graph is not None else None
        shared = w.dim() == 1
        f = dtp_forward_raw(plan, As, y, w, gather=gather, w_offset=offset)
        gWs, dfs = [], []
        for g in range(ng):
            d, K = f[g].shape[1], f[g].shape[2]
            dC2 = dCs[g].contiguous().reshape(E * d, -1)
            gWs.append(gemm_raw(2, f[g].reshape(E * d, K), dC2) if need_W[g] else None)
            dfs.append(gemm_raw(1, dC2, Ws[g]).view(E, d, K) if (need_x or need_w or need_off) else None)
        del f
        gw = goff = None
        gA = [None] * nb
        gB = [None] * nb
        if need_x or need_w or need_off:
            gxs, gw_full = dtp_grad_xw_raw(plan, As, y, w, dfs, gather=gather, w_offset=offset)
            gw = gw_full if need_w else None
            if need_off:
                goff = colsum_raw(gw_full)
            if need_x:
                if graph is None:
                    gA = gxs
                else:
                    lay = HeadLayout([2 * l + 1 for l, _ in plan.in1_blocks], [m for _, m in plan.in1_blocks], 1)
                    gA = attn_aggregate_raw(lay, None, gxs, graph, by_src=True)
                    if Bs is not None:
                        gB = attn_aggregate_raw(lay, None, gxs, graph)
        return (None, None, None, None, gw, goff, *gA, *(gB if Bs is not None else []), *gWs)


def dtp_linear(plan: DtpPlan, graph, As, Bs, y, w, w_offset, Ws):
    AB = (*As, *(Bs if Bs is not None else ()))
    n_b = 0 if Bs is None else len(Bs)
    return list(DtpLinear.apply(plan, graph, n_b, y, w, w_offset, *AB, *Ws))


def depthwise_tensor_product(plan: DtpPlan, xs: Sequence[torch.Tensor], y: torch.Tensor, w: torch.Tensor):
    return list(DtpOut.apply(plan, y, w, *xs))




class HeadLayout:

    def __init__(self, ds: Sequence[int], Cs: Sequence[int], n_heads: int):
        if len(ds) != len(Cs) or not ds:
            raise ValueError("bad head layout")
        if len(ds) > _lib.EQF_MAX_BLOCKS or n_heads > _lib.EQF_MAX_HEADS:
            raise NotImplementedError("head layout exceeds kernel limits")
        for c in Cs:
            if c % n_heads:
                raise ValueError("channels per group must be divisible by the number of heads")
        self.ds, self.Cs, self.n_heads = tuple(ds), tuple(Cs), int(n_heads)
        c = _lib.EqfHeadLayout()
        c.n_groups = len(ds)
        c.n_heads = n_heads
        for i, (d, C) in enumerate(zip(ds, Cs)):
            c.d[i], c.C[i] = d, C
        self.c = c

    def check(self, ts, rows: int, what: str):
        if len(ts) != len(self.ds):
            raise ValueError(f"{what}: expected {len(self.ds)} groups")
        out = []
        for t, d, C in zip(ts, self.ds, self.Cs):
            t = _require_cuda(t, what)
            if tuple(t.shape) != (rows, d, C):
                raise ValueError(f"{what}: group shape {tuple(t.shape)} != {(rows, d, C)}")
            out.append(t)
        return out


class Graph:

    def __init__(self, edge_src: torch.Tensor, edge_dst: torch.Tensor, n_nodes: int, check_sorted: bool = True):
        self.n_nodes = int(n_nodes)
        self.perm = None
        edge_src = _require_index(edge_src, "edge_src")
        edge_dst = _require_index(edge_dst, "edge_dst")
        if check_sorted and edge_dst.numel() > 1 and bool((edge_dst[1:] < edge_dst[:-1]).any()):
            self.perm = torch.sort(edge_dst, stable=True).indices
            edge_src, edge_dst = edge_src[self.perm], edge_dst[self.perm]
        self.src, self.dst = edge_src, edge_dst
        self.n_edges = int(edge_dst.numel())
        counts = torch.bincount(edge_dst, minlength=self.n_nodes)
        self.row_ptr = torch.zeros(self.n_nodes + 1, dtype=torch.int64, device=edge_dst.device)
        torch.cumsum(counts, 0, out=self.row_ptr[1:])

    def sort_edges(self, t: torch.Tensor) -> torch.Tensor:
        return t if self.perm is None else t.index_select(0, self.perm)

    def build_csc(self) -> None:
        self._src_perm = torch.sort(self.src, stable=True).indices
        counts = torch.zeros(self.n_nodes, dtype=torch.int64, device=self.src.device)
        counts.index_add_(0, self.src, torch.ones_like(self.src))
        self._src_row_ptr = torch.zeros(self.n_nodes + 1, dtype=torch.int64, device=self.src.device)
        torch.cumsum(counts, 0, out=self._src_row_ptr[1:])

    @property
    def src_perm(self) -> torch.Tensor:
        if getattr(self, "_src_perm", None) is None:
            self.build_csc()
        return self._src_perm

    @property
    def src_row_ptr(self) -> torch.Tensor:
        if getattr(self, "_src_row_ptr", None) is None:
            self.build_csc()
        return self._src_row_ptr


def seg_softmax_raw(z: torch.Tensor, graph: Graph) -> torch.Tensor:
    z = _require_cuda(z, "attention logits")
    if z.dim() != 2 or z.shape[0] != graph.n_edges:
        raise ValueError("logits must be [E, H]")
    alpha = torch.empty_like(z)
    with torch.cuda.device(z.device), _kernel("seg_softmax", 8 * z.numel()):
        rc = _lib.load().eqf_seg_softmax(z.data_ptr(), graph.row_ptr.data_ptr(), graph.n_nodes, z.shape[1],
                                         alpha.data_ptr(), _stream())
    _lib.check(rc, "eqf_seg_softmax")
    return alpha


def _keep_ptr(keep: Optional[torch.Tensor], like: torch.Tensor):
    if keep is None:
        return None
    keep = _require_cuda(keep, "dropout mask")
    if keep.shape != like.shape or keep.dtype != like.dtype:
        raise ValueError("the dropout mask must match the attention weights [E, H]")
    return keep.data_ptr()


def seg_softmax_bwd_raw(alpha: torch.Tensor, ga: torch.Tensor, graph: Graph, keep=None) -> torch.Tensor:
    ga = _require_cuda(ga, "softmax cotangent").contiguous()
    gz = torch.empty_like(alpha)
    nbytes = (12 + (4 if keep is not None else 0)) * alpha.numel()
    with torch.cuda.device(alpha.device), _kernel("seg_softmax_bwd", nbytes):
        rc = _lib.load().eqf_seg_softmax_bwd(alpha.data_ptr(), ga.data_ptr(), _keep_ptr(keep, alpha), graph.row_ptr.data_ptr(),
                                             graph.n_nodes, alpha.shape[1], gz.data_ptr(), _stream())
    _lib.check(rc, "eqf_seg_softmax_bwd")
    return gz


def attn_aggregate_raw(lay: HeadLayout, alpha, Vs, graph: Graph, by_src: bool = False) -> List[torch.Tensor]:
    Vs = lay.check(Vs, graph.n_edges, "aggregate V")
    if alpha is not None:
        alpha = _require_cuda(alpha, "alpha")
        if tuple(alpha.shape) != (graph.n_edges, lay.n_heads):
            raise ValueError("alpha must be [E, H]")
    dev = Vs[0].device
    outs = [torch.empty((graph.n_nodes, d, C), device=dev, dtype=torch.float32) for d, C in zip(lay.ds, lay.Cs)]
    if by_src:
        row_ptr, perm = graph.src_row_ptr, graph.src_perm
    else:
        row_ptr, perm = graph.row_ptr, None
    with torch.cuda.device(dev), _kernel("attn_aggregate", _attn_bytes(lay, graph.n_edges, graph.n_nodes, "aggregate")):
        rc = _lib.load().eqf_attn_aggregate(ctypes.byref(lay.c), alpha.data_ptr() if alpha is not None else None,
                                            _ptr_array(Vs), row_ptr.data_ptr(),
                                            perm.data_ptr() if perm is not None else None, graph.n_nodes,
                                            _ptr_array(outs), _stream())
    _lib.check(rc, "eqf_attn_aggregate")
    return outs


def attn_edge_dot_raw(lay: HeadLayout, Vs, Gs, graph: Graph) -> torch.Tensor:
    Vs = lay.check(Vs, graph.n_edges, "edge_dot V")
    Gs = lay.check(Gs, graph.n_nodes, "edge_dot G")
    out = torch.empty((graph.n_edges, lay.n_heads), device=Vs[0].device, dtype=torch.float32)
    with torch.cuda.device(out.device), _kernel("attn_edge_dot", _attn_bytes(lay, graph.n_edges, graph.n_nodes, "edge_dot")):
        rc = _lib.load().eqf_attn_edge_dot(ctypes.byref(lay.c), _ptr_array(Vs), _ptr_array(Gs),
                                           graph.dst.data_ptr(), graph.n_edges, out.data_ptr(), _stream())
    _lib.check(rc, "eqf_attn_edge_dot")
    return out


def attn_edge_scale_raw(lay: HeadLayout, alpha, Gs, graph: Graph, keep=None) -> List[torch.Tensor]:
    Gs = lay.check(Gs, graph.n_nodes, "edge_scale G")
    if alpha is not None:
        alpha = _require_cuda(alpha, "alpha")
    elif keep is not None:
        raise ValueError("edge_scale: a dropout mask needs alpha")
    dev = Gs[0].device
    outs = [torch.empty((graph.n_edges, d, C), device=dev, dtype=torch.float32) for d, C in zip(lay.ds, lay.Cs)]
    with torch.cuda.device(dev), _kernel("attn_edge_scale", _attn_bytes(lay, graph.n_edges, graph.n_nodes, "edge_scale")):
        rc = _lib.load().eqf_attn_edge_scale(ctypes.byref(lay.c), alpha.data_ptr() if alpha is not None else None,
                                             _keep_ptr(keep, alpha), _ptr_array(Gs), graph.dst.data_ptr(), graph.n_edges,
                                             _ptr_array(outs), _stream())
    _lib.check(rc, "eqf_attn_edge_scale")
    return outs


class SegSoftmax(torch.autograd.Function):

    @staticmethod
    def forward(ctx, z, graph: Graph):
        alpha = seg_softmax_raw(z, graph)
        ctx.graph = graph
        ctx.save_for_backward(alpha)
        return alpha

    @staticmethod
    def backward(ctx, ga):
        (alpha,) = ctx.saved_tensors
        g = ctx.graph
        if not torch.is_grad_enabled() and fused_ok(alpha):
            return seg_softmax_bwd_raw(alpha, ga, g), None
        t = alpha * ga
        s = torch.zeros((g.n_nodes, alpha.shape[1]), device=alpha.device, dtype=alpha.dtype).index_add(0, g.dst, t)
        return t - alpha * s.index_select(0, g.dst), None


class AttnAggregate(torch.autograd.Function):

    @staticmethod
    def forward(ctx, lay: HeadLayout, graph: Graph, alpha, *Vs):
        ctx.lay, ctx.graph = lay, graph
        ctx.has_alpha = alpha is not None
        outs = attn_aggregate_raw(lay, alpha, Vs, graph)
        if ctx.has_alpha:
            ctx.save_for_backward(alpha, *Vs)
        else:
            ctx.save_for_backward(*Vs)
        return tuple(outs)

    @staticmethod
    def backward(ctx, *Gs):
        lay, graph = ctx.lay, ctx.graph
        saved = ctx.saved_tensors
        alpha, Vs = (saved[0], saved[1:]) if ctx.has_alpha else (None, saved)
        Gs = [G.contiguous() if G is not None else torch.zeros((graph.n_nodes, d, C), device=Vs[0].device)
              for G, d, C in zip(Gs, lay.ds, lay.Cs)]
        ga = None
        gVs = [None] * len(Vs)
        if ctx.has_alpha and ctx.needs_input_grad[2]:
            ga = EdgeDot.apply(lay, graph, *Vs, *Gs)
        if any(ctx.needs_input_grad[3:]):
            gVs = list(EdgeScale.apply(lay, graph, alpha, *Gs))
        return (None, None, ga, *gVs)


class EdgeDot(torch.autograd.Function):

    @staticmethod
    def forward(ctx, lay: HeadLayout, graph: Graph, *VG):
        n = len(lay.ds)
        ctx.lay, ctx.graph = lay, graph
        out = attn_edge_dot_raw(lay, VG[:n], VG[n:], graph)
        ctx.save_for_backward(*VG)
        return out

    @staticmethod
    def backward(ctx, ca):
        lay, graph = ctx.lay, ctx.graph
        n = len(lay.ds)
        VG = ctx.saved_tensors
        Vs, Gs = VG[:n], VG[n:]
        ca = ca.contiguous()
        gVs = [None] * n
        gGs = [None] * n
        if any(ctx.needs_input_grad[2:2 + n]):
            gVs = list(EdgeScale.apply(lay, graph, ca, *Gs))
        if any(ctx.needs_input_grad[2 + n:]):
            gGs = list(AttnAggregate.apply(lay, graph, ca, *Vs))
        return (None, None, *gVs, *gGs)


class EdgeScale(torch.autograd.Function):

    @staticmethod
    def forward(ctx, lay: HeadLayout, graph: Graph, alpha, *Gs):
        ctx.lay, ctx.graph = lay, graph
        ctx.has_alpha = alpha is not None
        outs = attn_edge_scale_raw(lay, alpha, Gs, graph)
        if ctx.has_alpha:
            ctx.save_for_backward(alpha, *Gs)
        else:
            ctx.save_for_backward(*Gs)
        return tuple(outs)

    @staticmethod
    def backward(ctx, *cVs):
        lay, graph = ctx.lay, ctx.graph
        saved = ctx.saved_tensors
        alpha, Gs = (saved[0], saved[1:]) if ctx.has_alpha else (None, saved)
        cVs = [c.contiguous() if c is not None else torch.zeros((graph.n_edges, d, C), device=Gs[0].device)
               for c, d, C in zip(cVs, lay.ds, lay.Cs)]
        ga = None
        gGs = [None] * len(Gs)
        if ctx.has_alpha and ctx.needs_input_grad[2]:
            ga = EdgeDot.apply(lay, graph, *cVs, *Gs)
        if any(ctx.needs_input_grad[3:]):
            gGs = list(AttnAggregate.apply(lay, graph, alpha, *cVs))
        return (None, None, ga, *gGs)


def softmax_aggregate_raw(lay: HeadLayout, z: torch.Tensor, Vs, graph: Graph, keep=None):
    Vs = lay.check(Vs, graph.n_edges, "softmax_aggregate V")
    z = _require_cuda(z, "attention logits")
    if tuple(z.shape) != (graph.n_edges, lay.n_heads):
        raise ValueError("logits must be [E, H]")
    dev = z.device
    outs = [torch.empty((graph.n_nodes, d, C), device=dev, dtype=torch.float32) for d, C in zip(lay.ds, lay.Cs)]
    alpha = torch.empty_like(z)
    nbytes = _attn_bytes(lay, graph.n_edges, graph.n_nodes, "aggregate") + (4 if keep is None else 8) * z.numel()
    with torch.cuda.device(dev), _kernel("softmax_aggregate", nbytes):
        rc = _lib.load().eqf_attn_softmax_aggregate(ctypes.byref(lay.c), z.data_ptr(), _keep_ptr(keep, z), _ptr_array(Vs),
                                                    graph.row_ptr.data_ptr(), graph.n_nodes, _ptr_array(outs),
                                                    alpha.data_ptr(), _stream())
    _lib.check(rc, "eqf_attn_softmax_aggregate")
    return outs, alpha


def softmax_aggregate_ok(lay: HeadLayout, z: torch.Tensor) -> bool:
    return (fused_ok(z) and lay.ds[0] == 1 and all((c // lay.n_heads) % 4 == 0 for c in lay.Cs) and z.shape[0] > 0)


def _softmax_aggregate_forward(ctx, lay: HeadLayout, graph: Graph, z, keep, Vs):
    extra = () if keep is None else (keep,)
    outs, alpha = softmax_aggregate_raw(lay, z, Vs, graph, *extra)
# ... 1096 lines not shown
```

### include/eqf_b200.h

```cpp
#ifndef EQF_B200_H_
#define EQF_B200_H_

#include <stdint.h>

#ifdef __cplusplus
extern "C" {
#endif

#define EQF_MAX_BLOCKS 8
#define EQF_MAX_HEADS 16

#define EQF_OK 0
#define EQF_ERR_INVALID (-1)
#define EQF_ERR_CUDA (-2)
#define EQF_ERR_UNSUPPORTED (-3)

typedef struct EqfPlan EqfPlan;

typedef struct {
  int32_t l1, l2, l3;
  int32_t mul;
  int32_t in1_block;
  int32_t in2_off;
  int32_t out_group;
  int32_t out_chan_off;
  int32_t w_off;
  int32_t cg_off;
} EqfPathDesc;

typedef struct {
  const float* x[EQF_MAX_BLOCKS];
  const float* x2[EQF_MAX_BLOCKS];
  const int64_t* src;
  const int64_t* dst;
  const float* y;
  const float* w;
  int32_t w_shared;
  const float* g[EQF_MAX_BLOCKS];
  const float* w_offset;
} EqfEdgeOperands;

int eqf_version(void);
const char* eqf_last_error(void);
int eqf_device_sm_count(void);

int eqf_plan_create(const EqfPathDesc* paths, int32_t n_paths,
                    const int32_t* in1_l, const int32_t* in1_mul, int32_t n_in1,
                    const int32_t* out_l, const int32_t* out_mul, int32_t n_out,
                    int32_t d_y, int32_t weight_numel,
                    const float* cg, int32_t cg_len, EqfPlan** plan_out);
void eqf_plan_destroy(EqfPlan* plan);
int eqf_plan_info(const EqfPlan* plan, int32_t* out, int32_t n);
int eqf_plan_partial_rows(const EqfPlan* plan, int64_t n_edges);

int eqf_dtp_forward(const EqfPlan* plan, const EqfEdgeOperands* op, int64_t n_edges,
                    float* const* out_groups , void* stream);

int eqf_dtp_grad_x(const EqfPlan* plan, const EqfEdgeOperands* op, int64_t n_edges,
                   float* const* gx_blocks , void* stream);

int eqf_dtp_grad_w(const EqfPlan* plan, const EqfEdgeOperands* op, int64_t n_edges,
                   float* gw, void* stream);

int eqf_dtp_grad_y(const EqfPlan* plan, const EqfEdgeOperands* op, int64_t n_edges,
                   float* gy, void* stream);

int eqf_dtp_grad_xw(const EqfPlan* plan, const EqfEdgeOperands* op, int64_t n_edges,
                    float* const* gx_blocks, float* gw, void* stream);

typedef struct {
  int32_t n_groups;
  int32_t d[EQF_MAX_BLOCKS];
  int32_t C[EQF_MAX_BLOCKS];
  int32_t n_heads;
} EqfHeadLayout;

int eqf_seg_softmax(const float* z, const int64_t* row_ptr, int64_t n_nodes, int32_t n_heads,
                    float* alpha, void* stream);
int eqf_seg_softmax_bwd(const float* alpha, const float* ga, const float* keep, const int64_t* row_ptr, int64_t n_nodes,
                        int32_t n_heads, float* gz, void* stream);

int eqf_attn_aggregate(const EqfHeadLayout* lay, const float* alpha, const float* const* V,
                       const int64_t* row_ptr, const int64_t* perm, int64_t n_nodes, float* const* out, void* stream);
int eqf_attn_softmax_aggregate(const EqfHeadLayout* lay, const float* z, const float* keep, const float* const* V,
                               const int64_t* row_ptr, int64_t n_nodes, float* const* out, float* alpha, void* stream);

int eqf_attn_edge_dot(const EqfHeadLayout* lay, const float* const* V, const float* const* G,
                      const int64_t* dst, int64_t n_edges, float* galpha, void* stream);

int eqf_attn_edge_scale(const EqfHeadLayout* lay, const float* alpha, const float* keep, const float* const* G,
                        const int64_t* dst, int64_t n_edges, float* const* out, void* stream);

int eqf_pointwise_rows(int64_t rows);
int eqf_ln_silu_fwd(const float* x, const float* bias, const float* gamma, const float* beta, float eps, int64_t R,
                    int32_t C, float* y, float* mean, float* rstd, void* stream);
int eqf_ln_silu_bwd(const float* x, const float* bias, const float* gamma, const float* beta, const float* mean,
                    const float* rstd, const float* gy, int64_t R, int32_t C, float* gx, float* part, void* stream);

int eqf_gemm_tf32x3(const float* A, const float* Bt, float* C, int64_t M, int64_t N, int64_t K, int64_t lda,
                    int64_t ldb, int64_t ldc, int32_t b_is_kn, float* split, void* stream);
int64_t eqf_gemm_tf32x3_wgrad_slices(int64_t R, int64_t K1, int64_t N);
int eqf_gemm_tf32x3_wgrad(const float* A, const float* G, float* partial, int64_t R, int64_t K1, int64_t N, int64_t lda,
                          int64_t ldg, void* stream);
int eqf_gemm_tf32x3_wgrad_accumulate(const float* A, const float* G, float* W, int64_t R, int64_t K1, int64_t N,
                                     int64_t lda, int64_t ldg, void* stream);

int eqf_dtp_linear_supported(const EqfPlan* plan, int32_t group);
void eqf_fused_set_timeline(long long* device_buffer);
int eqf_dtp_group_forward(const EqfPlan* plan, const EqfEdgeOperands* op, int64_t n_edges, int32_t group, float* out,
                          void* stream);
int eqf_dtp_linear_fwd(const EqfPlan* plan, const EqfEdgeOperands* op, int64_t n_edges, int32_t group,
                       const float* Wt, int64_t N, int64_t ldw, float* C, int64_t ldc, float* split, void* stream);

int eqf_edge_geom_fwd(const float* pos, const int64_t* src, const int64_t* dst, const float* offsets, const float* a1,
                      const float* a2, int64_t E, int32_t lmax, float* vec, float* len, float* sh, void* stream);
int eqf_edge_geom_bwd(const float* vec, const float* a1, const float* a2, int64_t E, int32_t lmax, const float* g_sh,
                      const float* g_len, float* g_vec, void* stream);
int eqf_expnorm_fwd(const float* dist, const float* means, const float* betas, float alpha, float cutoff_upper, int64_t E,
                    int32_t B, float* out, void* stream);
int eqf_expnorm_bwd(const float* dist, const float* means, const float* betas, float alpha, float cutoff_upper, int64_t E,
                    int32_t B, const float* g, float* g_dist, void* stream);

int eqf_radius_graph_count(const float* pos, const int64_t* batch, int64_t n, float r_squared, int32_t loop,
                           int64_t max_neighbors, int64_t* deg, void* stream);
int eqf_radius_graph_fill(const float* pos, const int64_t* batch, int64_t n, float r_squared, int32_t loop,
                          int64_t max_neighbors, const int64_t* row_ptr, int64_t* src, int64_t* dst, void* stream);

int eqf_radius_graph_pbc_count(const float* pos, const int64_t* batch, const int64_t* frame_ptr, const float* cell,
                               int64_t n, float r_squared, int32_t rep_a, int32_t rep_b, int32_t rep_c, int64_t* deg,
                               void* stream);
int eqf_radius_graph_pbc_fill(const float* pos, const int64_t* batch, const int64_t* frame_ptr, const float* cell,
                              int64_t n, float r_squared, int32_t rep_a, int32_t rep_b, int32_t rep_c,
                              const int64_t* row_ptr, int64_t* src, int64_t* dst, int32_t* cell_offsets, float* dist2,
                              void* stream);

int eqf_rbf_fwd(const float* dist, const float* mean, const float* std, const float* weight, const float* bias,
                float cutoff, int64_t n_edges, float* out, void* stream);
int eqf_rbf_bwd(const float* dist, const float* mean, const float* std, const float* weight, const float* bias,
                float cutoff, const float* g, int64_t n_edges, float* g_dist, float* part, void* stream);

#define EQF_COLSUM_COUNTERS 16384
int64_t eqf_colsum_scratch_floats(int64_t rows, int64_t cols);
int eqf_colsum(const float* x, int64_t rows, int64_t cols, int64_t ld, float* out, float* part, uint32_t* counters,
               void* stream);

#define EQF_GROUP_MAX 8
typedef struct {
  const float* A;
  const float* B;
  float* C;
  int64_t M, N, K, lda, ldb, ldc;
  int32_t mode;
  int32_t accumulate;
  float alpha;
  int32_t pad;
} EqfGemmProblem;
int eqf_gemm_grouped(const EqfGemmProblem* problems, int32_t n, void* stream);

typedef struct {
  int32_t n_entries;
  int32_t mul[EQF_MAX_BLOCKS];
  int32_t d[EQF_MAX_BLOCKS];
  int32_t is_scalar[EQF_MAX_BLOCKS];
  float eps;
} EqfNormLayout;
int eqf_eln_rows(const EqfNormLayout* lay, int64_t rows);
int eqf_eln_fwd(const EqfNormLayout* lay, const float* x, const float* w, const float* b, int64_t N, float* y,
                float* rstd, void* stream);
int eqf_eln_bwd(const EqfNormLayout* lay, const float* x, const float* w, const float* rstd, const float* gy,
                int64_t N, float* gx, float* part, void* stream);

int eqf_eln_fwd_planar(const EqfNormLayout* lay, const float* const* x_blocks, const float* w, const float* b, int64_t N,
                       float* const* y_blocks, float* rstd, void* stream);
int eqf_eln_bwd_planar(const EqfNormLayout* lay, const float* const* x_blocks, const float* w, const float* rstd,
                       const float* const* gy_blocks, int64_t N, float* const* gx_blocks, float* part, void* stream);

typedef struct {
  int32_t n_gated;
  int32_t d[EQF_MAX_BLOCKS];
  int32_t C[EQF_MAX_BLOCKS];
  int32_t n_alpha, n_scalars, n_heads;
  float c_silu, c_sigmoid, c_slr, slr_slope;
} EqfGateLayout;
int eqf_gate_logits_fwd(const EqfGateLayout* lay, const float* t0, const float* bias, const float* const* gated,
                        const float* alpha_dot, int64_t n_edges, float* z, float* v0, float* const* vout, void* stream);
int eqf_gate_logits_bwd(const EqfGateLayout* lay, const float* t0, const float* bias, const float* const* gated,
                        const float* alpha_dot, const float* gz, const float* gv0, const float* const* gvout,
                        int64_t n_edges, float* gt0, float* const* ggated, float* gdot_part, void* stream);

#ifdef __cplusplus
}
#endif
#endif
```

Baseline: 1.383 million.

## Add fused DTP-linear backward kernel and save forward DTP output for backward

```diff
diff --git a/equiformer_b200/_lib.py b/equiformer_b200/_lib.py
--- a/equiformer_b200/_lib.py
+++ b/equiformer_b200/_lib.py
@@ -13,7 +13,7 @@
 INCLUDE_DIR = PKG_DIR.parent / "include"
 LIB_PATH = PKG_DIR / "libeqf_b200.so"
 SOURCES = ("eqf_abi.cu", "eqf_dtp.cu", "eqf_dtp_vec.cu", "eqf_dtp_v3.cu", "eqf_attn.cu", "eqf_pointwise.cu", "eqf_gemm_tf32x3.cu", "eqf_graph.cu",
-           "eqf_fused.cu", "eqf_edge.cu", "eqf_gemm_small.cu")
+           "eqf_fused.cu", "eqf_fused_bwd.cu", "eqf_edge.cu", "eqf_gemm_small.cu")
 
 EQF_COLSUM_COUNTERS = 16384
 EQF_MAX_BLOCKS = 8
@@ -130,6 +130,8 @@
     "eqf_dtp_group_forward": (c_int32, [c_void_p, POINTER(EqfEdgeOperands), c_int64, c_int32, c_void_p, c_void_p]),
     "eqf_dtp_linear_fwd": (c_int32, [c_void_p, POINTER(EqfEdgeOperands), c_int64, c_int32, c_void_p, c_int64, c_int64, c_void_p,
                                      c_int64, c_void_p, c_void_p]),
+    "eqf_dtp_linear_bwd": (c_int32, [c_void_p, POINTER(EqfEdgeOperands), c_int64, POINTER(c_int32), POINTER(c_void_p),
+                                     POINTER(c_void_p), c_void_p, c_void_p, c_void_p]),
     "eqf_radius_graph_count": (c_int32, [c_void_p, c_void_p, c_int64, c_float, c_int32, c_int64, c_void_p, c_void_p]),
     "eqf_radius_graph_fill": (c_int32, [c_void_p, c_void_p, c_int64, c_float, c_int32, c_int64, c_void_p, c_void_p, c_void_p,
                                         c_void_p]),
diff --git a/equiformer_b200/csrc/eqf_common.cuh b/equiformer_b200/csrc/eqf_common.cuh
--- a/equiformer_b200/csrc/eqf_common.cuh
+++ b/equiformer_b200/csrc/eqf_common.cuh
@@ -80,6 +80,7 @@
 int launch_forward_v3(const EqfPlan* plan, const EdgeArgs& a, cudaStream_t stream);
 int launch_backward_v3(const EqfPlan* plan, const EdgeArgs& a, bool with_w, cudaStream_t stream);
 int backward_v3_grid(const EqfPlan* plan, long long E);
+int dtp_linear_bwd_grid(long long E);
 
 }
 
diff --git a/equiformer_b200/csrc/eqf_dtp.cu b/equiformer_b200/csrc/eqf_dtp.cu
--- a/equiformer_b200/csrc/eqf_dtp.cu
+++ b/equiformer_b200/csrc/eqf_dtp.cu
@@ -401,6 +401,8 @@
   int rows = grid_for(plan, n_edges);
   const int b = backward_v3_grid(plan, n_edges);
   if (b > rows) rows = b;
+  const int f = dtp_linear_bwd_grid(n_edges);
+  if (f > rows) rows = f;
   if (plan->gen != nullptr) { const int c = plan->gen->partial_rows(plan, n_edges); if (c > rows) rows = c; }
   return rows;
 }
diff --git a/equiformer_b200/csrc/eqf_fused_bwd.cu b/equiformer_b200/csrc/eqf_fused_bwd.cu
--- /dev/null
+++ b/equiformer_b200/csrc/eqf_fused_bwd.cu
@@ -0,0 +1,440 @@
+#include <cuda_runtime.h>
+
+#include <cstdint>
+#include <mutex>
+#include <string>
+
+#include "eqf_common.cuh"
+#include "eqf_tc.cuh"
+
+namespace eqf {
+namespace fused_bwd {
+
+using namespace tc;
+
+constexpr int kThreads = 256;
+constexpr int TE = 24;
+constexpr int kDtpThreads = TE * 8;
+constexpr int kMaxPaths = 32;
+constexpr int kMaxSlices = 96;
+constexpr int kTileBytes = 32 * 128;
+constexpr int kSliceBytes = 2 * 2 * kTileBytes;
+constexpr int kMaxDeg = 5;
+constexpr int kDfBytes = TE * kMaxDeg * 128;
+constexpr int kXBytes = kMaxDeg * kDtpThreads * 16;
+constexpr int kMaxMRowBytes = 48 * 1024;
+
+struct BPath {
+  int d1, d2, d3, og, xb, mul, koff, w_off, y_off, cg_off, m_off;
+};
+
+struct BArgs {
+  const float* x[EQF_MAX_BLOCKS];
+  const float* x2[EQF_MAX_BLOCKS];
+  const long long* src;
+  const long long* dst;
+  const float* y;
+  const float* w;
+  const float* w_offset;
+  const float* cg;
+  const float* g[EQF_MAX_BLOCKS];
+  const float* whi[EQF_MAX_BLOCKS];
+  const float* wlo[EQF_MAX_BLOCKS];
+  float* gx[EQF_MAX_BLOCKS];
+  float* gw;
+  long long E;
+  int w_shared, W, d_y, m_row, n_in1, n_paths, n_slices;
+  int gn[EQF_MAX_BLOCKS];
+  int gk[EQF_MAX_BLOCKS];
+  int gd[EQF_MAX_BLOCKS];
+  int n_out;
+  int in1_d[EQF_MAX_BLOCKS], in1_mul[EQF_MAX_BLOCKS];
+  int xb_first[EQF_MAX_BLOCKS + 1];
+  int m_bytes;
+  int a_off[EQF_MAX_BLOCKS];
+  int a_bytes;
+  unsigned char slice_og[kMaxSlices];
+  unsigned short slice_ch[kMaxSlices];
+  BPath paths[kMaxPaths];
+};
+
+__device__ __forceinline__ float4 ld4(const float* p) { return __ldg(reinterpret_cast<const float4*>(p)); }
+__device__ __forceinline__ void st4(float* p, const float4& v) { *reinterpret_cast<float4*>(p) = v; }
+__device__ __forceinline__ void addv(float4& a, const float4& b) { a.x += b.x; a.y += b.y; a.z += b.z; a.w += b.w; }
+__device__ __forceinline__ void fs(float4& a, const float4& x, float m) {
+  a.x = fmaf(x.x, m, a.x); a.y = fmaf(x.y, m, a.y); a.z = fmaf(x.z, m, a.z); a.w = fmaf(x.w, m, a.w);
+}
+__device__ __forceinline__ void fv(float4& a, const float4& x, const float4& y) {
+  a.x = fmaf(x.x, y.x, a.x); a.y = fmaf(x.y, y.y, a.y); a.z = fmaf(x.z, y.z, a.z); a.w = fmaf(x.w, y.w, a.w);
+}
+__device__ __forceinline__ void sts64(uint32_t addr, float a, float b) {
+  asm volatile("st.shared.v2.f32 [%0], {%1, %2};" ::"r"(addr), "f"(a), "f"(b) : "memory");
+}
+__device__ __forceinline__ void cp_async16(uint32_t dst, const void* src) {
+  asm volatile("cp.async.cg.shared.global [%0], [%1], 16;" ::"r"(dst), "l"(src) : "memory");
+}
+__device__ __forceinline__ void cp_async_commit() { asm volatile("cp.async.commit_group;" ::: "memory"); }
+__device__ __forceinline__ void cp_async_wait_all() { asm volatile("cp.async.wait_all;" ::: "memory"); }
+
+__device__ __forceinline__ void prefetch_slice(const BArgs& a, int s, uint32_t buf) {
+  const int og = a.slice_og[s], ch0 = a.slice_ch[s], N = a.gn[og], n_kt = N / 32;
+  const int chunks = 2 * n_kt * 32 * 8;
+  for (int q = threadIdx.x; q < chunks; q += kThreads) {
+    const int c = q & 7, r = (q >> 3) & 31, pk = q >> 8;
+    const int plane = pk / n_kt, kt = pk - plane * n_kt;
+    const float* src = (plane ? a.wlo[og] : a.whi[og]) + (long long)(ch0 + r) * N + kt * 32 + c * 4;
+    cp_async16(buf + (uint32_t)(pk * kTileBytes + r * 128 + ((c ^ (r & 7)) << 4)), src);
+  }
+  cp_async_commit();
+}
+
+__device__ __forceinline__ void load_dc_tile(const BArgs& a, long long e0, int n_e, uint32_t a_addr, int n_out) {
+  for (int g = 0; g < n_out; ++g) {
+    const int N = a.gn[g];
+    if (N == 0) continue;
+    const int d3 = a.gd[g], rows = n_e * d3, cpr = N / 4;
+    const float* src = a.g[g] + e0 * d3 * (long long)N;
+    const uint32_t base = a_addr + (uint32_t)a.a_off[g];
+    for (int q = threadIdx.x; q < rows * cpr; q += kThreads) {
+      const int r = q / cpr, c = q - r * cpr, kt = c >> 3, c8 = c & 7;
+      cp_async16(base + (uint32_t)(kt * TE * d3 * 128 + r * 128 + ((c8 ^ (r & 7)) << 4)), src + (long long)r * N + c * 4);
+    }
+  }
+  cp_async_commit();
+}
+
+template <int D3>
+__device__ __noinline__ void mma_slice(const BArgs& a, int og, int n_e, uint32_t a_addr, uint32_t bbuf, uint32_t df_addr) {
+  constexpr int kBlocks = (TE * D3 + 63) / 64;
+  const int warp = threadIdx.x >> 5, lane = threadIdx.x & 31, wg = warp >> 2, r_w = (warp & 3) * 16;
+  const int n_kt = a.gn[og] / 32;
+  const int rows = n_e * D3;
+  const uint32_t a_tile = a_addr + (uint32_t)a.a_off[og];
+#pragma unroll 1
+  for (int mb = wg; mb < kBlocks; mb += 2) {
+    if (mb * 64 >= rows) break;
+#pragma unroll 1
+    for (int kt = 0; kt < n_kt; ++kt) {
+      float part[16];
+#pragma unroll
+      for (int i = 0; i < 16; ++i) part[i] = 0.f;
+#pragma unroll
+      for (int half = 0; half < 2; ++half) {
+        uint32_t hi[8], lo[8];
+        load_a_split(a_tile + (uint32_t)(kt * TE * D3 * 128), mb * 64 + r_w, lane, hi, lo, 2 * half);
+        mma_ktile_3xtf32<32>(part, hi, lo, bbuf + (uint32_t)(kt * kTileBytes), bbuf + (uint32_t)((n_kt + kt) * kTileBytes),
+                             2 * half);
+        wgmma_wait<0>();
+      }
+#pragma unroll
+      for (int i = 0; i < 16; i += 2) {
+        const int r = mb * 64 + r_w + acc_row(i, lane);
+        const int c = acc_col(i, lane);
+        const uint32_t addr = df_addr + (uint32_t)(r * 128 + (((c >> 2) ^ (r & 7)) << 4) + (c & 3) * 4);
+        if (r >= rows) continue;
+        if (kt == 0) {
+          sts64(addr, part[i], part[i + 1]);
+        } else {
+          sts64(addr, lds32(addr) + part[i], lds32(addr + 4u) + part[i + 1]);
+        }
+      }
+    }
+  }
+}
+
+struct SliceRing {
+  int s;
+};
+
+template <int D1, int D3>
+__device__ __forceinline__ void path_bwd(const BArgs& a, const BPath& p, int u, int el, long long e0, int n_e,
+                                         uint32_t x_addr, float4 (&gx)[D1], uint32_t m_addr, uint32_t a_addr, uint32_t b_addr,
+                                         uint32_t df_addr, float* gacc, SliceRing& ring) {
+  const bool active = el < n_e;
+  const int es = active ? el : 0;
+  const long long e = e0 + es;
+  float4 wv = ld4(a.w + (a.w_shared ? 0 : e * a.W) + p.w_off + u);
+  if (a.w_offset != nullptr) addv(wv, ld4(a.w_offset + p.w_off + u));
+  float4 df[D3];
+  if (a.gn[p.og] != 0) {
+    cp_async_wait_all();
+    fence_async_smem();
+    __syncthreads();
+    mma_slice<D3>(a, p.og, n_e, a_addr, b_addr, df_addr);
+    __syncthreads();
+    ring.s = ring.s + 1 == a.n_slices ? 0 : ring.s + 1;
+    prefetch_slice(a, ring.s, b_addr);
+    const int c8 = (u >> 2) & 7;
+#pragma unroll
+    for (int k = 0; k < D3; ++k) {
+      const int r = es * D3 + k;
+      df[k] = lds128(df_addr + (uint32_t)(r * 128 + ((c8 ^ (r & 7)) << 4)));
+    }
+  } else {
+    const float* dp = a.g[p.og] + e * D3 * (long long)a.gk[p.og] + p.koff + u;
+#pragma unroll
+    for (int k = 0; k < D3; ++k) df[k] = ld4(dp + (long long)k * a.gk[p.og]);
+  }
+  const uint32_t ma = m_addr + (uint32_t)(es * a.m_row + p.m_off) * 4u;
+  float4 gwv = make_float4(0.f, 0.f, 0.f, 0.f);
+#pragma unroll
+  for (int i = 0; i < D1; ++i) {
+    float4 t = make_float4(0.f, 0.f, 0.f, 0.f);
+#pragma unroll
+    for (int k = 0; k < D3; ++k) fs(t, df[k], lds32(ma + (uint32_t)(i * D3 + k) * 4u));
+    fv(gx[i], wv, t);
+    fv(gwv, lds128(x_addr + (uint32_t)(i * kDtpThreads * 16)), t);
+  }
+  if (!a.w_shared) {
+    if (active) st4(a.gw + e * a.W + p.w_off + u, gwv);
+  } else {
+    if (!active) gwv = make_float4(0.f, 0.f, 0.f, 0.f);
+#pragma unroll
+    for (int o = 8; o < 32; o <<= 1) {
+      gwv.x += __shfl_xor_sync(0xffffffffu, gwv.x, o);
+      gwv.y += __shfl_xor_sync(0xffffffffu, gwv.y, o);
+      gwv.z += __shfl_xor_sync(0xffffffffu, gwv.z, o);
+      gwv.w += __shfl_xor_sync(0xffffffffu, gwv.w, o);
+    }
+    if ((threadIdx.x & 31) < 8) {
+      float* ga = gacc + p.w_off + u;
+      atomicAdd(ga, gwv.x); atomicAdd(ga + 1, gwv.y); atomicAdd(ga + 2, gwv.z); atomicAdd(ga + 3, gwv.w);
+    }
+  }
+}
+
+template <int D1>
+__device__ __forceinline__ void block_chunk(const BArgs& a, int b, int u, int el, long long e0, int n_e, uint32_t x_base,
+                                            uint32_t m_addr, uint32_t a_addr, uint32_t b_addr, uint32_t df_addr, float* gacc,
+                                            SliceRing& ring) {
+  const bool active = el < n_e;
+  const long long e = e0 + (active ? el : 0);
+  const int mul = a.in1_mul[b];
+  const long long row_floats = (long long)D1 * mul;
+  const long long rs = a.src != nullptr ? a.src[e] : e;
+  float4 x[D1], gx[D1];
+#pragma unroll
+  for (int i = 0; i < D1; ++i) {
+    x[i] = ld4(a.x[b] + rs * row_floats + i * mul + u);
+    gx[i] = make_float4(0.f, 0.f, 0.f, 0.f);
+  }
+  if (a.x2[b] != nullptr) {
+    const float* xq = a.x2[b] + a.dst[e] * row_floats + u;
+#pragma unroll
+    for (int i = 0; i < D1; ++i) addv(x[i], ld4(xq + i * mul));
+  }
+  const uint32_t x_addr = x_base + (uint32_t)(threadIdx.x < kDtpThreads ? threadIdx.x : 0) * 16u;
+  if (threadIdx.x < kDtpThreads) {
+#pragma unroll
+    for (int i = 0; i < D1; ++i) sts128(x_addr + (uint32_t)(i * kDtpThreads * 16), x[i]);
+  }
+  for (int pi = a.xb_first[b]; pi < a.xb_first[b + 1]; ++pi) {
+    const BPath& p = a.paths[pi];
+    switch (p.d3) {
+      case 1: path_bwd<D1, 1>(a, p, u, el, e0, n_e, x_addr, gx, m_addr, a_addr, b_addr, df_addr, gacc, ring); break;
+      case 3: path_bwd<D1, 3>(a, p, u, el, e0, n_e, x_addr, gx, m_addr, a_addr, b_addr, df_addr, gacc, ring); break;
+      default: path_bwd<D1, 5>(a, p, u, el, e0, n_e, x_addr, gx, m_addr, a_addr, b_addr, df_addr, gacc, ring); break;
+    }
+  }
+  if (active) {
+    float* go = a.gx[b] + e * row_floats + u;
+#pragma unroll
+    for (int i = 0; i < D1; ++i) st4(go + i * mul, gx[i]);
+  }
+}
+
+__global__ void __launch_bounds__(kThreads, 2) dtp_linear_bwd_kernel(const __grid_constant__ BArgs a) {
+  extern __shared__ uint8_t smem_raw[];
+  uint8_t* smem = reinterpret_cast<uint8_t*>((reinterpret_cast<uintptr_t>(smem_raw) + 1023) & ~uintptr_t(1023));
+  const uint32_t b_addr = smem_u32(smem);
+  const uint32_t a_addr = b_addr + kSliceBytes;
+  const uint32_t df_addr = a_addr + (uint32_t)a.a_bytes;
+  const uint32_t x_base = df_addr + kDfBytes;
+  float* mw = reinterpret_cast<float*>(smem + kSliceBytes + a.a_bytes + kDfBytes + kXBytes);
+  int4* mdesc = reinterpret_cast<int4*>(reinterpret_cast<uint8_t*>(mw) + a.m_bytes);
+  float* gacc = reinterpret_cast<float*>(mdesc + a.m_row);
+  const uint32_t m_addr = smem_u32(mw);
+  const int t = threadIdx.x, el = t >> 3, c8 = t & 7;
+
+  for (int q = t; q < a.m_row; q += kThreads) {
+    int pi = 0;
+    for (int j = 1; j < a.n_paths; ++j) if (a.paths[j].m_off <= q) pi = j;
+    const BPath& p = a.paths[pi];
+    const int r = q - p.m_off, i = r / p.d3, k = r - i * p.d3;
+    mdesc[q] = i < p.d1 ? make_int4(p.cg_off + i * p.d2 * p.d3 + k, p.y_off, p.d2, p.d3) : make_int4(0, 0, 0, 1);
+  }
+  if (a.w_shared) for (int i = t; i < a.W; i += kThreads) gacc[i] = 0.f;
+  SliceRing ring{0};
+  prefetch_slice(a, 0, b_addr);
+
+  const long long n_tiles = (a.E + TE - 1) / TE;
+  for (long long tile = blockIdx.x; tile < n_tiles; tile += gridDim.x) {
+    const long long e0 = tile * TE;
+    const int n_e = (int)((a.E - e0) < TE ? (a.E - e0) : TE);
+    __syncthreads();
+    load_dc_tile(a, e0, n_e, a_addr, a.n_out);
+    for (int q = t; q < n_e * a.m_row; q += kThreads) {
+      const int ee = q / a.m_row, r = q - ee * a.m_row;
+      const int4 d = mdesc[r];
+      const float* yv = a.y + (e0 + ee) * a.d_y + d.y;
+      float m = 0.f;
+      for (int j = 0; j < d.z; ++j) m = fmaf(__ldg(a.cg + d.x + j * d.w), __ldg(yv + j), m);
+      mw[ee * a.m_row + r] = m;
+    }
+    __syncthreads();
+    for (int b = 0; b < a.n_in1; ++b) {
+      for (int c0 = 0; c0 < a.in1_mul[b]; c0 += 32) {
+        const int u = c0 + c8 * 4;
+        switch (a.in1_d[b]) {
+          case 1: block_chunk<1>(a, b, u, el, e0, n_e, x_base, m_addr, a_addr, b_addr, df_addr, gacc, ring); break;
+          case 3: block_chunk<3>(a, b, u, el, e0, n_e, x_base, m_addr, a_addr, b_addr, df_addr, gacc, ring); break;
+          default: block_chunk<5>(a, b, u, el, e0, n_e, x_base, m_addr, a_addr, b_addr, df_addr, gacc, ring); break;
+        }
+      }
+    }
+  }
+  cp_async_wait_all();
+  if (a.w_shared) {
+    __syncthreads();
+    for (int i = t; i < a.W; i += kThreads) a.gw[(long long)blockIdx.x * a.W + i] = gacc[i];
+  }
+}
+
+__global__ void split_kernel(const float* __restrict__ w, long long ldw, float* __restrict__ hi, float* __restrict__ lo, long long K,
+                             long long N) {
+  for (long long i = (long long)blockIdx.x * blockDim.x + threadIdx.x; i < K * N; i += (long long)gridDim.x * blockDim.x) {
+    const long long k = i / N, n = i - k * N;
+    const float v = w[k * ldw + n];
+    const float h = tf32_rn(v);
+    hi[i] = h;
+    lo[i] = tf32_rn(v - h);
+  }
+}
+
+}
+
+int dtp_linear_bwd_grid(long long n_edges) {
+  const long long tiles = (n_edges + fused_bwd::TE - 1) / fused_bwd::TE;
+  const long long cap = 2LL * tc::device_sms();
+  return (int)(tiles < cap ? (tiles > 0 ? tiles : 1) : cap);
+}
+
+}
+
+using namespace eqf;
+
+extern "C" int eqf_dtp_linear_bwd(const EqfPlan* plan, const EqfEdgeOperands* op, int64_t n_edges, const int32_t* group_n,
+                                  const float* const* Wts, float* const* gx_blocks, float* gw, float* split, void* stream) {
+  using namespace eqf::fused_bwd;
+  if (plan == nullptr || op == nullptr || group_n == nullptr || Wts == nullptr || gx_blocks == nullptr || gw == nullptr ||
+      split == nullptr) {
+    set_error("eqf_dtp_linear_bwd: null argument");
+    return EQF_ERR_INVALID;
+  }
+  if (n_edges <= 0) return EQF_OK;
+  int rc = ensure_device(plan);
+  if (rc != EQF_OK) return rc;
+  const PlanHdr& h = plan->hdr;
+  BArgs a;
+  auto misaligned = [](const void* p) { return ((uintptr_t)p & 15) != 0; };
+  if (!op->y || !op->w || misaligned(op->w) || misaligned(op->w_offset) || misaligned(gw) || (h.w_numel & 3)) {
+    set_error("eqf_dtp_linear_bwd: y / w missing, or weights not 16-byte aligned / weight_numel % 4 != 0");
+    return EQF_ERR_INVALID;
+  }
+  if (h.n_paths > kMaxPaths || h.n_in1 > EQF_MAX_BLOCKS || h.n_out > EQF_MAX_BLOCKS) {
+    set_error("eqf_dtp_linear_bwd: plan too large");
+    return EQF_ERR_UNSUPPORTED;
+  }
+  for (int b = 0; b < EQF_MAX_BLOCKS; ++b) {
+    a.x[b] = a.x2[b] = nullptr; a.gx[b] = nullptr; a.g[b] = nullptr; a.whi[b] = a.wlo[b] = nullptr; a.gn[b] = a.gk[b] = 0;
+    a.gd[b] = 1; a.a_off[b] = 0;
+    a.in1_d[b] = a.in1_mul[b] = 0;
+  }
+  for (int b = 0; b < h.n_in1; ++b) {
+    if (!op->x[b] || !gx_blocks[b] || misaligned(op->x[b]) || misaligned(op->x2[b]) || misaligned(gx_blocks[b]) ||
+        h.in1_mul[b] % 32 != 0 || h.in1_d[b] > kMaxDeg) {
+      set_error("eqf_dtp_linear_bwd: in1 blocks must be present, 16-byte aligned, l <= 2, multiplicities % 32 == 0");
+      return EQF_ERR_INVALID;
+    }
+    a.x[b] = op->x[b]; a.x2[b] = op->x2[b]; a.gx[b] = gx_blocks[b];
+    a.in1_d[b] = h.in1_d[b]; a.in1_mul[b] = h.in1_mul[b];
+  }
+  a.src = reinterpret_cast<const long long*>(op->src);
+  a.dst = reinterpret_cast<const long long*>(op->dst);
+  if (a.x2[0] != nullptr && (a.src == nullptr || a.dst == nullptr)) { set_error("eqf_dtp_linear_bwd: x2 needs src and dst"); return EQF_ERR_INVALID; }
+  a.y = op->y; a.w = op->w; a.w_offset = op->w_offset; a.w_shared = op->w_shared;
+  if (a.w_shared && a.w_offset != nullptr) { set_error("eqf_dtp_linear_bwd: w_offset needs per-edge weights"); return EQF_ERR_INVALID; }
+  a.cg = reinterpret_cast<const float*>(plan->d_blob + h.off_cg);
+  a.gw = gw; a.E = n_edges; a.W = h.w_numel; a.d_y = h.d_y; a.n_in1 = h.n_in1; a.n_paths = h.n_paths;
+  long long split_off = 0;
+  bool any_narrow = false;
+  cudaStream_t s = (cudaStream_t)stream;
+  for (int g = 0; g < h.n_out; ++g) {
+    const int N = group_n[g];
+    if (!op->g[g] || misaligned(op->g[g]) || (N != 0 && N != 32 && N != 64) || h.out_d[g] > kMaxDeg) {
+      set_error("eqf_dtp_linear_bwd: group gradient missing / misaligned, l > 2, or N_g not in {0, 32, 64}");
+      return EQF_ERR_INVALID;
+    }
+    a.g[g] = op->g[g]; a.gn[g] = N; a.gk[g] = h.out_mul[g]; a.gd[g] = h.out_d[g];
+    if (N == 0) continue;
+    any_narrow = true;
+    if (Wts[g] == nullptr) { set_error("eqf_dtp_linear_bwd: null weight of a narrow group"); return EQF_ERR_INVALID; }
+    const long long n = (long long)h.out_mul[g] * N;
+    float* hi = split + split_off;
+    float* lo = hi + n;
+    split_off += 2 * n;
+    const unsigned blocks = (unsigned)((n + 255) / 256 < 1056 ? (n + 255) / 256 : 1056);
+    split_kernel<<<blocks, 256, 0, s>>>(Wts[g], N, hi, lo, h.out_mul[g], N);
+    if ((rc = check_cuda(cudaGetLastError(), "eqf_dtp_linear_bwd split launch")) != EQF_OK) return rc;
+    a.whi[g] = hi; a.wlo[g] = lo;
+  }
+  a.n_out = h.n_out;
+  a.a_bytes = 0;
+  for (int g = 0; g < h.n_out; ++g)
+    if (a.gn[g] != 0) { a.a_off[g] = a.a_bytes; a.a_bytes += (a.gn[g] / 32) * TE * a.gd[g] * 128; }
+  if (!any_narrow) { set_error("eqf_dtp_linear_bwd: no narrow group (use eqf_dtp_grad_xw)"); return EQF_ERR_INVALID; }
+  const PathDev* pd = reinterpret_cast<const PathDev*>(plan->blob.data() + h.off_paths);
+  int n = 0, m_off = 0;
+  a.n_slices = 0;
+  for (int b = 0; b < h.n_in1; ++b) {
+    a.xb_first[b] = n;
+    for (int p = 0; p < h.n_paths; ++p) {
+      if (pd[p].xb != b) continue;
+      BPath& q = a.paths[n++];
+      q.d1 = pd[p].d1; q.d2 = pd[p].d2; q.d3 = pd[p].d3; q.og = pd[p].og; q.xb = b; q.mul = pd[p].mul; q.koff = pd[p].koff;
+      q.w_off = pd[p].w_off; q.y_off = pd[p].y_off; q.cg_off = pd[p].cg_off; q.m_off = m_off;
+      m_off += (q.d1 * q.d3 + 3) & ~3;
+      if (q.mul != h.in1_mul[b] || q.koff % 32 != 0) {
+        set_error("eqf_dtp_linear_bwd: depth-wise paths with 32-channel aligned group offsets required");
+        return EQF_ERR_UNSUPPORTED;
+      }
+    }
+  }
+  a.xb_first[h.n_in1] = n;
+  for (int b = 0; b < h.n_in1; ++b)
+    for (int c0 = 0; c0 < h.in1_mul[b]; c0 += 32)
+      for (int pi = a.xb_first[b]; pi < a.xb_first[b + 1]; ++pi) {
+        if (a.gn[a.paths[pi].og] == 0) continue;
+        if (a.n_slices >= kMaxSlices) { set_error("eqf_dtp_linear_bwd: too many narrow slices"); return EQF_ERR_UNSUPPORTED; }
+        a.slice_og[a.n_slices] = (unsigned char)a.paths[pi].og;
+        a.slice_ch[a.n_slices] = (unsigned short)(a.paths[pi].koff + c0);
+        ++a.n_slices;
+      }
+  a.m_row = m_off;
+  a.m_bytes = (TE * m_off * 4 + 127) & ~127;
+  if (a.m_bytes > kMaxMRowBytes) { set_error("eqf_dtp_linear_bwd: coupling blocks of a tile exceed shared memory"); return EQF_ERR_UNSUPPORTED; }
+  const int smem = 1024 + kSliceBytes + a.a_bytes + kDfBytes + kXBytes + a.m_bytes + a.m_row * 16 + (a.w_shared ? a.W * 4 : 0);
+  if (smem > 227 * 1024) { set_error("eqf_dtp_linear_bwd: shared memory"); return EQF_ERR_UNSUPPORTED; }
+  {
+    static std::mutex mtx;
+    static int attr_bytes = 0;
+    std::lock_guard<std::mutex> lock(mtx);
+    if (smem > attr_bytes) {
+      cudaError_t e = cudaFuncSetAttribute(dtp_linear_bwd_kernel, cudaFuncAttributeMaxDynamicSharedMemorySize, smem);
+      if (e != cudaSuccess) return check_cuda(e, "dtp_linear_bwd smem attribute");
+      attr_bytes = smem;
+    }
+  }
+  dtp_linear_bwd_kernel<<<dtp_linear_bwd_grid(n_edges), fused_bwd::kThreads, smem, s>>>(a);
+  return check_cuda(cudaGetLastError(), "dtp_linear_bwd_kernel launch");
+}
diff --git a/equiformer_b200/csrc/eqf_tc.cuh b/equiformer_b200/csrc/eqf_tc.cuh
--- a/equiformer_b200/csrc/eqf_tc.cuh
+++ b/equiformer_b200/csrc/eqf_tc.cuh
@@ -198,6 +198,13 @@
                               int box_cols, MapKind kind = MapKind::kSwizzled) {
   EncodeTiled enc = encode_fn();
   if (enc == nullptr) { set_error("cuTensorMapEncodeTiled is not available from the driver"); return EQF_ERR_CUDA; }
+  static thread_local bool ctx_current = false;
+  if (!ctx_current) {
+    int dev = 0;
+    cudaGetDevice(&dev);
+    if (cudaSetDevice(dev) != cudaSuccess) { set_error("cudaSetDevice failed before cuTensorMapEncodeTiled"); return EQF_ERR_CUDA; }
+    ctx_current = true;
+  }
   cuuint64_t dims[2] = {(cuuint64_t)cols, (cuuint64_t)rows};
   cuuint64_t strides[1] = {(cuuint64_t)ld * sizeof(float)};
   cuuint32_t box[2] = {(cuuint32_t)box_cols, (cuuint32_t)box_rows};
diff --git a/equiformer_b200/nets/graph_attention_transformer.py b/equiformer_b200/nets/graph_attention_transformer.py
--- a/equiformer_b200/nets/graph_attention_transformer.py
+++ b/equiformer_b200/nets/graph_attention_transformer.py
@@ -321,7 +321,7 @@
             sa = self.sep_act
             weight = sa.dtp_rad(edge_scalars, add_offset=False)
             plan1 = sa.dtp.tp.plan
-            fuse1 = self._fuse_act and ops.dtp_linear_ok(plan1, edge_attr, weight)
+            fuse1 = self._fuse_act and ops.dtp_linear_carries(plan1, edge_attr, weight)
             f = None
             if not fuse1:
                 f = sa.dtp.tp.planar_depthwise_gathered(graph, m_src, m_dst, edge_attr, weight,
@@ -396,7 +396,7 @@
         sv = self.sep_value
         plan2 = sv.dtp.tp.plan
         w2 = sv.dtp.tp.weight
-        if self._fuse_value and ops.dtp_linear_ok(plan2, edge_attr, w2):
+        if self._fuse_value and ops.dtp_linear_carries(plan2, edge_attr, w2):
             Ws = _group_weight_matrices(sv.lin, len(plan2.out_groups))
             return sv.lin._planar_bias(ops.dtp_linear(plan2, None, [v.contiguous() for v in value], None, edge_attr, w2,
                                                       None, Ws))
@@ -591,7 +591,7 @@
         node_feats = self.exp.planar([ones])
         weight = self.rad(edge_scalars, add_offset=False)
         plan = self.dw.tp.plan
-        if self._fuse_proj and ops.dtp_linear_ok(plan, edge_attr, weight):
+        if self._fuse_proj and ops.dtp_linear_carries(plan, edge_attr, weight):
             Ws = _group_weight_matrices(self.proj, len(plan.out_groups))
             edge_feats = self.proj._planar_bias(ops.dtp_linear(plan, graph, node_feats, None, edge_attr, weight,
                                                                self.rad.offset, Ws))
diff --git a/equiformer_b200/ops.py b/equiformer_b200/ops.py
--- a/equiformer_b200/ops.py
+++ b/equiformer_b200/ops.py
@@ -259,6 +259,49 @@
         rc = _lib.load().eqf_dtp_grad_xw(plan.handle, ctypes.byref(op), E, _ptr_array(gxs),
                                          ctypes.c_void_p(gw.data_ptr()), _stream())
     _lib.check(rc, "eqf_dtp_grad_xw")
+    return gxs, (_colsum(gw) if shared else gw)
+
+
+def dtp_linear_bwd_raw(plan: DtpPlan, xs, y, w, gs, Ws, gather=None, w_offset=None) -> Tuple[List[torch.Tensor], torch.Tensor]:
+    y, w, E, shared = _check_yw(plan, y, w)
+    xs, gather = _check_gather(plan, xs, gather, E, "dtp_linear_bwd x")
+    if len(gs) != len(plan.out_groups) or len(Ws) != len(plan.out_groups):
+        raise ValueError(f"dtp_linear_bwd: expected {len(plan.out_groups)} output groups")
+    group_n = (ctypes.c_int32 * _lib.EQF_MAX_BLOCKS)()
+    wts = (ctypes.c_void_p * _lib.EQF_MAX_BLOCKS)()
+    gs2, Ws2 = [], []
+    split_floats = 0
+    for g, ((l, _p, K), t, W) in enumerate(zip(plan.out_groups, gs, Ws)):
+        t = _require_cuda(t, "dtp_linear_bwd g").contiguous()
+        n = K if W is None else W.shape[1]
+        if tuple(t.shape) != (E, 2 * l + 1, n):
+            raise ValueError(f"dtp_linear_bwd: group {g} gradient {tuple(t.shape)} != {(E, 2 * l + 1, n)}")
+        if W is not None:
+            W = _require_cuda(W, "dtp_linear_bwd weight").contiguous()
+            if W.shape[0] != K:
+                raise ValueError(f"dtp_linear_bwd: weight {g} must be [{K}, N], got {tuple(W.shape)}")
+            group_n[g] = n
+            wts[g] = W.data_ptr()
+            split_floats += 2 * K * n
+        gs2.append(t)
+        Ws2.append(W)
+    gxs = [torch.empty((E, 2 * l + 1, mul), device=y.device, dtype=torch.float32) for l, mul in plan.in1_blocks]
+    if E == 0:
+        return gxs, torch.zeros_like(w)
+    gw = _gw_buffer(plan, E, shared, y.device)
+    split = _FUSED_SPLIT.get(("bwd", y.device))
+    if split is None or split.numel() < split_floats:
+        split = torch.empty(max(split_floats, 1 << 16), device=y.device, dtype=torch.float32)
+        _FUSED_SPLIT[("bwd", y.device)] = split
+    op = _operands(plan, xs, y, w, gs2, shared, gather, w_offset)
+    d_in = sum((2 * l + 1) * m for l, m in plan.in1_blocks)
+    d_g = sum(t.shape[1] * t.shape[2] for t in gs2)
+    nbytes = 4 * E * (d_g + 2 * d_in + plan.d_y + (0 if shared else 2 * plan.weight_numel))
+    flops = 2 * E * sum(t.shape[1] * t.shape[2] * W.shape[0] for t, W in zip(gs2, Ws2) if W is not None)
+    with torch.cuda.device(y.device), _kernel("dtp_linear_bwd", nbytes, flops):
+        rc = _lib.load().eqf_dtp_linear_bwd(plan.handle, ctypes.byref(op), E, group_n, wts, _ptr_array(gxs),
+                                            ctypes.c_void_p(gw.data_ptr()), ctypes.c_void_p(split.data_ptr()), _stream())
+    _lib.check(rc, "eqf_dtp_linear_bwd")
     return gxs, (_colsum(gw) if shared else gw)
 
 
@@ -518,6 +561,16 @@
 _FUSED = _FUSED_MODE != "0"
 _FUSED_MIN_EDGES = int(os.environ.get("EQF_FUSED_MIN_EDGES", "200000"))
 _FUSED_SPLIT = {}
+_FUSED_BWD = os.environ.get("EQF_FUSED_BWD", "0") == "1"
+
+
+def _fused_bwd_ok(t: torch.Tensor) -> bool:
+    return t.is_cuda and t.dtype == torch.float32
+
+
+def dtp_linear_bwd_supported(plan: DtpPlan) -> bool:
+    return (dtp_linear_supported(plan) and all(l <= 2 and m % 32 == 0 for l, m in plan.in1_blocks)
+            and all(l <= 2 for l, _p, _k in plan.out_groups))
 
 
 def dtp_linear_supported(plan: DtpPlan) -> bool:
@@ -529,11 +582,15 @@
     return ok
 
 
+def dtp_linear_carries(plan: DtpPlan, y: torch.Tensor, w: torch.Tensor) -> bool:
+    return (fused_ok(y) and not (torch.is_grad_enabled() and y.requires_grad)
+            and y.shape[0] > 0 and dtp_linear_supported(plan))
+
+
 def dtp_linear_ok(plan: DtpPlan, y: torch.Tensor, w: torch.Tensor) -> bool:
     if not _FUSED or (_FUSED_MODE == "auto" and y.shape[0] < _FUSED_MIN_EDGES and not FUSED_ON_ANY_DEVICE):
         return False
-    return (fused_ok(y) and not (torch.is_grad_enabled() and y.requires_grad)
-            and y.shape[0] > 0 and dtp_linear_supported(plan))
+    return dtp_linear_carries(plan, y, w)
 
 
 def dtp_linear_fwd_raw(plan: DtpPlan, group: int, xs, y, w, Wt: torch.Tensor, gather=None, w_offset=None) -> torch.Tensor:
@@ -600,16 +657,25 @@
             raise ValueError(f"DtpLinear: expected {ng} weight matrices, got {len(Ws)}")
         As, Bs = AB[:nb], (AB[nb:] if n_b else None)
         gather = (graph.src, graph.dst, Bs) if graph is not None else None
+        E = y.shape[0]
         outs = []
-        for g in range(ng):
-            if Ws[g].shape[1] <= _FUSED_MAX_N:
-                outs.append(dtp_linear_fwd_raw(plan, g, As, y, w, Ws[g], gather=gather, w_offset=offset))
-            else:
-                fg = dtp_group_forward_raw(plan, g, As, y, w, gather=gather, w_offset=offset)
-                E, d = fg.shape[0], fg.shape[1]
-                outs.append(gemm_raw(0, fg.reshape(E * d, fg.shape[2]), Ws[g].contiguous()).view(E, d, -1))
+        f = None
+        if dtp_linear_ok(plan, y, w):
+            for g in range(ng):
+                if Ws[g].shape[1] <= _FUSED_MAX_N:
+                    outs.append(dtp_linear_fwd_raw(plan, g, As, y, w, Ws[g], gather=gather, w_offset=offset))
+                else:
+                    fg = dtp_group_forward_raw(plan, g, As, y, w, gather=gather, w_offset=offset)
+                    d = fg.shape[1]
+                    outs.append(gemm_raw(0, fg.reshape(E * d, fg.shape[2]), Ws[g].contiguous()).view(E, d, -1))
+        else:
+            f = dtp_forward_raw(plan, As, y, w, gather=gather, w_offset=offset)
+            for fg, W in zip(f, Ws):
+                d = fg.shape[1]
+                outs.append(gemm_raw(0, fg.reshape(E * d, fg.shape[2]), W.contiguous()).view(E, d, -1))
         ctx.plan, ctx.graph, ctx.n_b, ctx.n_ab, ctx.has_off = plan, graph, n_b, n_ab, offset is not None
-        ctx.save_for_backward(y, w, *([offset] if offset is not None else []), *rest)
+        ctx.n_f = 0 if f is None else len(f)
+        ctx.save_for_backward(y, w, *([offset] if offset is not None else []), *rest, *(f if f is not None else ()))
         return tuple(outs)
 
     @staticmethod
@@ -617,6 +683,8 @@
         plan, graph, n_b, n_ab = ctx.plan, ctx.graph, ctx.n_b, ctx.n_ab
         y, w, *saved = ctx.saved_tensors
         offset = saved.pop(0) if ctx.has_off else None
+        f = saved[len(saved) - ctx.n_f:] if ctx.n_f else None
+        saved = saved[:len(saved) - ctx.n_f]
         AB, Ws = saved[:n_ab], saved[n_ab:]
         nb, ng = len(plan.in1_blocks), len(plan.out_groups)
         As, Bs = AB[:nb], (AB[nb:] if n_b else None)
@@ -632,20 +700,30 @@
             grads = _higher_order_grads(fn, (y, w, offset, *AB, *Ws), dCs)
             return (None, None, None, *grads)
         gather = (graph.src, graph.dst, Bs) if graph is not None else None
-        shared = w.dim() == 1
-        f = dtp_forward_raw(plan, As, y, w, gather=gather, w_offset=offset)
+        if f is None:
+            f = dtp_forward_raw(plan, As, y, w, gather=gather, w_offset=offset)
+        need_xw = need_x or need_w or need_off
+        narrow = [_FUSED_BWD and _fused_bwd_ok(y) and W.shape[1] <= _FUSED_MAX_N and W.shape[1] % 32 == 0 for W in Ws]
+        fuse_bwd = need_xw and any(narrow) and dtp_linear_bwd_supported(plan)
         gWs, dfs = [], []
         for g in range(ng):
             d, K = f[g].shape[1], f[g].shape[2]
             dC2 = dCs[g].contiguous().reshape(E * d, -1)
             gWs.append(gemm_raw(2, f[g].reshape(E * d, K), dC2) if need_W[g] else None)
-            dfs.append(gemm_raw(1, dC2, Ws[g]).view(E, d, K) if (need_x or need_w or need_off) else None)
+            if fuse_bwd and narrow[g]:
+                dfs.append(dC2.view(E, d, -1))
+            else:
+                dfs.append(gemm_raw(1, dC2, Ws[g]).view(E, d, K) if need_xw else None)
         del f
         gw = goff = None
         gA = [None] * nb
         gB = [None] * nb
-        if need_x or need_w or need_off:
-            gxs, gw_full = dtp_grad_xw_raw(plan, As, y, w, dfs, gather=gather, w_offset=offset)
+        if need_xw:
+            if fuse_bwd:
+                gxs, gw_full = dtp_linear_bwd_raw(plan, As, y, w, dfs, [W if n else None for W, n in zip(Ws, narrow)],
+                                                  gather=gather, w_offset=offset)
+            else:
+                gxs, gw_full = dtp_grad_xw_raw(plan, As, y, w, dfs, gather=gather, w_offset=offset)
             gw = gw_full if need_w else None
             if need_off:
                 goff = colsum_raw(gw_full)
diff --git a/include/eqf_b200.h b/include/eqf_b200.h
--- a/include/eqf_b200.h
+++ b/include/eqf_b200.h
@@ -111,6 +111,8 @@
                           void* stream);
 int eqf_dtp_linear_fwd(const EqfPlan* plan, const EqfEdgeOperands* op, int64_t n_edges, int32_t group,
                        const float* Wt, int64_t N, int64_t ldw, float* C, int64_t ldc, float* split, void* stream);
+int eqf_dtp_linear_bwd(const EqfPlan* plan, const EqfEdgeOperands* op, int64_t n_edges, const int32_t* group_n,
+                       const float* const* Wts, float* const* gx_blocks, float* gw, float* split, void* stream);
 
 int eqf_edge_geom_fwd(const float* pos, const int64_t* src, const int64_t* dst, const float* offsets, const float* a1,
                       const float* a2, int64_t E, int32_t lmax, float* vec, float* len, float* sh, void* stream);
```

Result: no change. 1.378 million (median of 6 runs) (-0.3%).
